# daniilidis-group/msckf_mono

Hardware: AMD Instinct MI355X
Metric: filter updates/sec (30-cam window, 200 feats) (higher is better)
Workload: dtype f32; 1 GPU; BASELINE.json configs[2]: synthetic 30-cam window / 200 feats, float, 64 batched trajectories per GPU; cam_window=30, tracks_per_update=200, trajectories_per_gpu=64, imu_per_update=10, parallelism=replicated trajectories, 64 per rank, noise=isotropic (f_u = f_v), sequences=1, gate_early_accept=False, streams=4

## Files before the change

include/msckf_hip.h:

```cpp
#ifndef MSCKF_HIP_H
#define MSCKF_HIP_H

#include <stdint.h>

#ifdef __cplusplus
extern "C" {
#endif

typedef struct msckf_hip_batch* msckf_hip_handle;

enum { MSCKF_HIP_F32 = 0, MSCKF_HIP_F64 = 1, MSCKF_HIP_F16H_F32P = 2 };

int msckf_hip_create(int B, int n_cap, int f_cap, int m_cap, int dtype, int device, msckf_hip_handle* out);
int msckf_hip_destroy(msckf_hip_handle h);
int msckf_hip_copy_state(msckf_hip_handle dst, msckf_hip_handle src);
const char* msckf_hip_last_error(void);

int msckf_hip_initialize(msckf_hip_handle h, int b, const double* cam12, const double* noise29,
                         const double* params8, const double* imu29);
int msckf_hip_initialize_full(msckf_hip_handle h, int b, const double* cam12, const double* uv2, const double* Q144,
                              const double* P0_225, const double* params8, const double* imu29);
int msckf_hip_propagate(msckf_hip_handle h, int b, const double* readings7, int K);
int msckf_hip_augment_state(msckf_hip_handle h, int b, int state_id, double time);
int msckf_hip_update(msckf_hip_handle h, int b, const double* meas2, const uint64_t* ids, int n);
// ... 10 lines not shown
int msckf_hip_get_pruned_states(msckf_hip_handle h, int b, double* cam7, double* time, int* state_ids,
                                int* last_correlated_ids, int cap);
int msckf_hip_get_cam_meta(msckf_hip_handle h, int b, double* time, int* n_tracked, int* last_correlated_ids, int cap);
int msckf_hip_get_tracked_feature_ids(msckf_hip_handle h, int b, int cam_index, uint64_t* ids, int cap);

int msckf_hip_get_covariance(msckf_hip_handle h, int b, double* P, int ld);
int msckf_hip_set_covariance(msckf_hip_handle h, int b, const double* P, int D);
int msckf_hip_set_imu_state(msckf_hip_handle h, int b, const double* imu29);
int msckf_hip_set_cam_pose(msckf_hip_handle h, int b, int slot, const double* cam7);
int msckf_hip_get_num_residualized(msckf_hip_handle h, int b, long long* n);
int msckf_hip_set_num_residualized(msckf_hip_handle h, int b, long long n);
int msckf_hip_last_stats(msckf_hip_handle h, int b, int* out7);
int msckf_hip_clear_error_flags(msckf_hip_handle h, int b);
int msckf_hip_get_error_flags(msckf_hip_handle h, int b, int* flags);
int msckf_hip_last_tracks(msckf_hip_handle h, int b, double* out8, int cap);
int msckf_hip_last_deltax(msckf_hip_handle h, int b, double* dx, int cap);
int msckf_hip_last_track_blocks(msckf_hip_handle h, int b, int* first, double* Hx, double* rw, double* Bh, int cap);

int msckf_hip_set_tracks(msckf_hip_handle h, int b, int F, const int* M, const int* slots, const double* obs2);
int msckf_hip_propagate_range(msckf_hip_handle h, int b0, int nb, const double* readings7, int K);
int msckf_hip_propagate_range_counts(msckf_hip_handle h, int b0, int nb, const double* readings7, const int* K);
int msckf_hip_augment_range(msckf_hip_handle h, int b0, int nb);
int msckf_hip_marginalize_range(msckf_hip_handle h, int b0, int nb);
int msckf_hip_drop_oldest_range(msckf_hip_handle h, int b0, int nb, int n_drop);
int msckf_hip_image_cycle_range(msckf_hip_handle h, int b0, int nb, const int* state_ids, const double* times,
                                const double* upd_meas2, const uint64_t* upd_ids, const int* upd_n,
                                const double* new_meas2, const uint64_t* new_ids, const int* new_n, int flags);

int msckf_hip_scenario_alloc(msckf_hip_handle h, int n_frames, int K);
int msckf_hip_scenario_set(msckf_hip_handle h, int frame, int b, const double* readings7 , int F,
                           const int* M, const int* slots, const double* obs2, int n_drop);
enum { MSCKF_HIP_CELL_SKIP = 1 };
int msckf_hip_scenario_set_cell(msckf_hip_handle h, int frame, int b, const double* readings7 , int k, int F,
                                const int* M, const int* slots, const double* obs2, int n_drop, int flags);
int msckf_hip_scenario_commit(msckf_hip_handle h);
int msckf_hip_run_frames(msckf_hip_handle h, int f0, int f1);
int msckf_hip_run_frames_streamed(msckf_hip_handle h, int f0, int f1);
int msckf_hip_scenario_pin(msckf_hip_handle h, int f0, int f1);
int msckf_hip_set_upload_ring(msckf_hip_handle h, int depth, int mode);
int msckf_hip_replay_alloc(msckf_hip_handle h, int n_seq, int n_frames, int K);
int msckf_hip_replay_set_cell(msckf_hip_handle h, int frame, int seq, const double* readings7 , int k, int F,
                              const int* M, const int* slots, const double* obs2, int n_drop, int flags);
int msckf_hip_replay_assign(msckf_hip_handle h, const int* seq_of, const uint64_t* seed, const double* sigma4);
int msckf_hip_replay_assign_q(msckf_hip_handle h, const int* seq_of, const uint64_t* seed, const double* Q144 ,
                              const double* scale , const double* sigma_uv );
int msckf_hip_replay_walk(msckf_hip_handle h, int f0, int f1, int b0, int nb, double* out);
int msckf_hip_replay_commit(msckf_hip_handle h);
int msckf_hip_run_frames_replay(msckf_hip_handle h, int f0, int f1);
int msckf_hip_replay_expand(msckf_hip_handle h, int frame, int b, double* rd , double* obs2, int cap_entries);
int msckf_hip_replay_expand_ints(msckf_hip_handle h, int frame, int b, int* ints, int* slots, int cap_entries);
int msckf_hip_sync(msckf_hip_handle h);
int msckf_hip_frame_log_enable(msckf_hip_handle h, int capacity_frames);
int msckf_hip_frame_log_reset(msckf_hip_handle h);
int msckf_hip_frame_log_count(msckf_hip_handle h);
int msckf_hip_frame_log_read(msckf_hip_handle h, int r0, int n, int b0, int nb, double* out);
int msckf_hip_frame_log_metrics(msckf_hip_handle h, int r0, int r1, const double* gt_p, double* out);
int msckf_hip_frame_log_metrics_ranges(msckf_hip_handle h, const int* r0, const int* r1, const double* gt_p, double* out);
int msckf_hip_map_log_enable(msckf_hip_handle h, int capacity_per_trajectory);
int msckf_hip_map_log_reset(msckf_hip_handle h);
int msckf_hip_map_log_frames(msckf_hip_handle h);
int msckf_hip_map_log_counts(msckf_hip_handle h, int b0, int nb, int* stored, int* found);
int msckf_hip_map_log_read(msckf_hip_handle h, int b, int r0, int n, double* out);
int msckf_hip_map_log_metrics(msckf_hip_handle h, int q0, int q1, const double* gt_xyz, const int* gt_off, double* out);
int msckf_hip_pruned_log_enable(msckf_hip_handle h, int capacity_per_trajectory);
int msckf_hip_pruned_log_reset(msckf_hip_handle h);
int msckf_hip_pruned_log_frames(msckf_hip_handle h);
int msckf_hip_pruned_log_counts(msckf_hip_handle h, int b0, int nb, int* stored, int* found);
int msckf_hip_pruned_log_read(msckf_hip_handle h, int b, int r0, int n, double* out, int* aug_ord);
int msckf_hip_pruned_log_metrics(msckf_hip_handle h, int q0, int q1, const double* gt_pose, int n_ord, double* out);
int msckf_hip_profile_enable(msckf_hip_handle h, int on);
int msckf_hip_profile_read(msckf_hip_handle h, double* ms8, int* count8);
int msckf_hip_profile_read_ex(msckf_hip_handle h, double* ms, int* count, int cap);
int msckf_hip_profile_event_overhead(msckf_hip_handle h, double* ms);
int msckf_hip_set_streams(msckf_hip_handle h, int n);
int msckf_hip_set_hw_queues(msckf_hip_handle h, int n);
int msckf_hip_parse_hw_queues(const char* text);
int msckf_hip_set_slices_exact(msckf_hip_handle h, int on);
int msckf_hip_get_effective_streams(msckf_hip_handle h, int streamed, int* out);
int msckf_hip_set_host_affinity(msckf_hip_handle h, const int* cpus, int n);
int msckf_hip_set_gate_early_accept(msckf_hip_handle h, int on);
int msckf_hip_set_compression(msckf_hip_handle h, int route);
int msckf_hip_set_covariance_update(msckf_hip_handle h, int form);
int msckf_hip_set_feature_overlap(msckf_hip_handle h, int on);
int msckf_hip_set_anisotropic_noise(msckf_hip_handle h, int mode, double tail_tol);
int msckf_hip_literal_info(msckf_hip_handle h, int b, int* out8);

#ifdef __cplusplus
}
#endif
#endif
```

msckf_mono_amd/capi.py:

```python
import ctypes as C
import os
import subprocess

import numpy as np

_HERE = os.path.dirname(os.path.abspath(__file__))
LIB_PATH = os.environ.get("MSCKF_HIP_LIB", os.path.join(_HERE, "libmsckf_hip.so"))
_LIB = None

F32, F64, F16H = 0, 1, 2
_dp = C.POINTER(C.c_double)
_ip = C.POINTER(C.c_int)
_up = C.POINTER(C.c_uint64)

SYMBOLS = [
    "msckf_hip_create", "msckf_hip_destroy", "msckf_hip_last_error", "msckf_hip_initialize", "msckf_hip_initialize_full", "msckf_hip_propagate",
    "msckf_hip_augment_state", "msckf_hip_update", "msckf_hip_add_features", "msckf_hip_marginalize",
    "msckf_hip_prune_empty_states", "msckf_hip_prune_redundant_states", "msckf_hip_finish",
    "msckf_hip_get_num_cam_states", "msckf_hip_get_imu_state", "msckf_hip_get_cam_states", "msckf_hip_get_map",
    "msckf_hip_get_pruned_state_ids", "msckf_hip_get_covariance", "msckf_hip_set_covariance", "msckf_hip_set_imu_state",
    "msckf_hip_set_cam_pose", "msckf_hip_get_num_residualized", "msckf_hip_set_num_residualized", "msckf_hip_last_stats",
    "msckf_hip_last_tracks", "msckf_hip_last_deltax", "msckf_hip_set_tracks", "msckf_hip_propagate_range",
    "msckf_hip_augment_range", "msckf_hip_marginalize_range", "msckf_hip_drop_oldest_range", "msckf_hip_scenario_alloc",
    "msckf_hip_scenario_set", "msckf_hip_scenario_commit", "msckf_hip_run_frames", "msckf_hip_run_frames_streamed", "msckf_hip_sync",
    "msckf_hip_profile_enable", "msckf_hip_profile_read", "msckf_hip_profile_read_ex", "msckf_hip_profile_event_overhead", "msckf_hip_set_streams", "msckf_hip_set_gate_early_accept",
    "msckf_hip_scenario_pin", "msckf_hip_set_upload_ring", "msckf_hip_clear_error_flags",
    "msckf_hip_set_compression", "msckf_hip_set_covariance_update", "msckf_hip_set_feature_overlap", "msckf_hip_get_pruned_states", "msckf_hip_get_cam_meta", "msckf_hip_get_tracked_feature_ids",
    "msckf_hip_set_anisotropic_noise", "msckf_hip_literal_info", "msckf_hip_get_error_flags", "msckf_hip_copy_state", "msckf_hip_set_host_affinity",
    "msckf_hip_image_cycle_range", "msckf_hip_get_effective_streams", "msckf_hip_set_hw_queues", "msckf_hip_parse_hw_queues", "msckf_hip_set_slices_exact",
    "msckf_hip_frame_log_enable", "msckf_hip_frame_log_reset", "msckf_hip_frame_log_count", "msckf_hip_frame_log_read", "msckf_hip_frame_log_metrics",
    "msckf_hip_scenario_set_cell", "msckf_hip_propagate_range_counts", "msckf_hip_frame_log_metrics_ranges",
    "msckf_hip_map_log_enable", "msckf_hip_map_log_reset", "msckf_hip_map_log_frames", "msckf_hip_map_log_counts", "msckf_hip_map_log_read", "msckf_hip_map_log_metrics",
    "msckf_hip_pruned_log_enable", "msckf_hip_pruned_log_reset", "msckf_hip_pruned_log_frames", "msckf_hip_pruned_log_counts", "msckf_hip_pruned_log_read", "msckf_hip_pruned_log_metrics",
    "msckf_hip_replay_alloc", "msckf_hip_replay_set_cell", "msckf_hip_replay_assign", "msckf_hip_replay_commit", "msckf_hip_run_frames_replay", "msckf_hip_replay_expand",
    "msckf_hip_replay_expand_ints", "msckf_hip_replay_assign_q", "msckf_hip_replay_walk", "msckf_hip_last_track_blocks",
]
CELL_SKIP = 1

FRAME_LOG_STRIDE = 48
FRAME_LOG_FIELDS = {
    "q": slice(0, 4), "b_g": slice(4, 7), "v": slice(7, 10), "b_a": slice(10, 13), "p": slice(13, 16),
    "P_II_diag": slice(16, 31), "P_pp": slice(31, 37),
    "n_cam": slice(37, 38), "n_tracks": slice(38, 39), "n_passed": slice(39, 40), "error_flags": slice(40, 41),
    "cam0": slice(41, 48),
}
FRAME_LOG_METRICS = ("n", "sum_sq_err", "max_err", "final_err", "sum_nees", "n_flagged")
MAP_LOG_STRIDE = 8
MAP_LOG_FIELDS = {"p": slice(0, 3), "gamma": slice(3, 4), "frame": slice(4, 5), "track": slice(5, 6), "flags": slice(6, 7), "M": slice(7, 8)}
MAP_FLAG_PASS, MAP_FLAG_INCLUDED, MAP_FLAG_BOUND = 1, 2, 4
MAP_LOG_METRICS = ("n", "n_matched", "sum_sq_err", "max_err", "n_gated", "sum_gamma", "sum_dof", "n_unmatched")
PRUNED_LOG_STRIDE = 32
PRUNED_LOG_FIELDS = {"q": slice(0, 4), "p": slice(4, 7), "frame": slice(7, 8), "cov": slice(8, 29),
                     "n_cam": slice(29, 30), "k": slice(30, 31), "pad": slice(31, 32)}
PRUNED_LOG_METRICS = ("n", "n_matched", "sum_sq_pos_err", "max_pos_err", "sum_sq_ang_err", "max_ang_err", "sum_nees", "n_nees", "n_bad_pivot", "n_unmatched")


def build():
    subprocess.check_call(["make", "-s", "-j8", "-C", os.path.join(_HERE, "csrc")])


def lib():
    global _LIB
    if _LIB is None:
        if not os.path.exists(LIB_PATH):
            raise RuntimeError("libmsckf_hip.so is not built (run __graft_entry__.build()); there is no CPU fallback")
        try:
            import torch
        except Exception:
            pass
        L = C.CDLL(LIB_PATH)
        L.msckf_hip_last_error.restype = C.c_char_p
        _LIB = L
    return _LIB


class HipError(RuntimeError):
    pass


def _chk(rc):
    if rc < 0:
        raise HipError("msckf_hip call failed (%d): %s" % (rc, lib().msckf_hip_last_error().decode()))
    return rc


def _d(a):
    a = np.ascontiguousarray(a, dtype=np.float64)
    return a, a.ctypes.data_as(_dp)


def _i(a):
    a = np.ascontiguousarray(a, dtype=np.int32)
    return a, a.ctypes.data_as(_ip)


def pack_config(cfg):
    cam = np.array([cfg["c_u"], cfg["c_v"], cfg["f_u"], cfg["f_v"], cfg.get("b", 0.0)] + list(cfg["q_CI"]) + list(cfg["p_C_I"]), dtype=np.float64)
    noise = np.array([cfg["u_var_prime"], cfg["v_var_prime"]] + list(cfg["Q_imu_diag"]) + list(cfg["P0_diag"]), dtype=np.float64)
    params = np.array([cfg["max_gn_cost_norm"], cfg.get("min_rcond", 3e-12), cfg["translation_threshold"],
                       cfg.get("redundancy_angle_thresh", 0.005), cfg.get("redundancy_distance_thresh", 0.05),
                       cfg["min_track_length"], cfg["max_track_length"], cfg["max_cam_states"]], dtype=np.float64)
    return cam, noise, params


def full_noise(cfg):
    if "Q_imu" not in cfg and "P0" not in cfg:
        return None
    Q = np.asarray(cfg["Q_imu"], dtype=np.float64) if "Q_imu" in cfg else np.diag(np.asarray(cfg["Q_imu_diag"], dtype=np.float64))
    P0 = np.asarray(cfg["P0"], dtype=np.float64) if "P0" in cfg else np.diag(np.asarray(cfg["P0_diag"], dtype=np.float64))
    if Q.shape != (12, 12) or P0.shape != (15, 15):
        raise ValueError("Q_imu must be 12 x 12 and P0 15 x 15")
    return Q, P0


class Batch:
    _replay_K = 0
    _replay_frames = 0

# ... 211 lines not shown
    def replay_set_cell(self, frame, seq, readings, M, slots, obs, n_drop, skip=False):
        r, pr = _d(np.asarray(readings, dtype=np.float64).reshape(-1, 7)); Ma, pM = _i(M); s, ps = _i(slots); o, po = _d(obs)
        _chk(self.L.msckf_hip_replay_set_cell(self.h, int(frame), int(seq), pr, r.shape[0], len(Ma), pM, ps, po, int(n_drop), CELL_SKIP if skip else 0))

    def replay_assign(self, seq_of, seeds, sigma4):
        q, pq = _i(seq_of)
        sd = np.ascontiguousarray([int(x) & 0xFFFFFFFFFFFFFFFF for x in seeds], dtype=np.uint64)
        sg = np.ascontiguousarray(np.broadcast_to(np.asarray(sigma4, dtype=np.float64), (self.B, 4)))
        if q.shape != (self.B,) or sd.shape != (self.B,):
            raise ValueError("seq_of and seeds must hold one value per trajectory")
        _chk(self.L.msckf_hip_replay_assign(self.h, pq, sd.ctypes.data_as(_up), sg.ctypes.data_as(_dp)))

    def replay_assign_q(self, seq_of, seeds, Q, scale, sigma_uv):
        q, pq = _i(seq_of)
        sd = np.ascontiguousarray([int(x) & 0xFFFFFFFFFFFFFFFF for x in seeds], dtype=np.uint64)
        if q.shape != (self.B,) or sd.shape != (self.B,):
            raise ValueError("seq_of and seeds must hold one value per trajectory")
        Qa = np.broadcast_to(np.asarray(Q, dtype=np.float64), (self.B, 12, 12))
        Qc = np.ascontiguousarray(np.swapaxes(Qa, 1, 2))
        sc_ = np.ascontiguousarray(np.broadcast_to(np.asarray(scale, dtype=np.float64), (self.B,)))
        uv = np.ascontiguousarray(np.broadcast_to(np.asarray(sigma_uv, dtype=np.float64), (self.B, 2)))
        _chk(self.L.msckf_hip_replay_assign_q(self.h, pq, sd.ctypes.data_as(_up), Qc.ctypes.data_as(_dp), sc_.ctypes.data_as(_dp), uv.ctypes.data_as(_dp)))

    def replay_walk(self, f0=0, f1=None, b0=0, nb=None):
        f1 = self._replay_frames + 1 if f1 is None else int(f1)
        nb = self.B - int(b0) if nb is None else int(nb)
        out = np.zeros((max(f1 - int(f0), 0), max(nb, 0), 6))
        _chk(self.L.msckf_hip_replay_walk(self.h, int(f0), f1, int(b0), nb, out.ctypes.data_as(_dp)))
        return out

    def replay_commit(self):
        _chk(self.L.msckf_hip_replay_commit(self.h))

    def run_frames_replay(self, f0, f1):
        _chk(self.L.msckf_hip_run_frames_replay(self.h, int(f0), int(f1)))

    def replay_expand(self, frame, b):
        cap = self.f_cap * self.m_cap
        rd = np.zeros((self._replay_K, 7)); obs = np.zeros((cap, 2)); ints = np.zeros(3 + 2 * self.f_cap, dtype=np.int32); slots = np.zeros(cap, dtype=np.int32)
        n = _chk(self.L.msckf_hip_replay_expand(self.h, int(frame), int(b), rd.ctypes.data_as(_dp), obs.ctypes.data_as(_dp), cap))
        _chk(self.L.msckf_hip_replay_expand_ints(self.h, int(frame), int(b), ints.ctypes.data_as(_ip), slots.ctypes.data_as(_ip), cap))
        return dict(rd=rd, obs=obs[:n], n=int(ints[0]), drop=int(ints[1]), k=int(ints[2]), M=ints[3:3 + self.f_cap].copy(),
                    off=ints[3 + self.f_cap:].copy(), slots=slots[:n])

    def scenario_pin(self, f0, f1):
        _chk(self.L.msckf_hip_scenario_pin(self.h, int(f0), int(f1)))

    def set_upload_ring(self, depth=6, mode=0):
        _chk(self.L.msckf_hip_set_upload_ring(self.h, int(depth), int(mode)))

    def clear_error_flags(self, b):
        _chk(self.L.msckf_hip_clear_error_flags(self.h, int(b)))

    def sync(self):
        _chk(self.L.msckf_hip_sync(self.h))

    def set_host_affinity(self, cpus):
        a = np.ascontiguousarray(list(cpus), dtype=np.int32)
        _chk(self.L.msckf_hip_set_host_affinity(self.h, a.ctypes.data_as(_ip), int(a.size)))

    def set_streams(self, n):
        _chk(self.L.msckf_hip_set_streams(self.h, int(n)))

    def set_hw_queues(self, n):
        _chk(self.L.msckf_hip_set_hw_queues(self.h, int(n)))

    def set_slices_exact(self, on):
        _chk(self.L.msckf_hip_set_slices_exact(self.h, 1 if on else 0))

    def effective_streams(self, streamed=False):
        n = C.c_int(0)
        _chk(self.L.msckf_hip_get_effective_streams(self.h, 1 if streamed else 0, C.byref(n)))
        return int(n.value)

    def set_compression(self, route):
        _chk(self.L.msckf_hip_set_compression(self.h, int(route)))

    def set_covariance_update(self, form):
        _chk(self.L.msckf_hip_set_covariance_update(self.h, int(form)))

    def set_feature_overlap(self, on):
        _chk(self.L.msckf_hip_set_feature_overlap(self.h, 1 if on else 0))

    def set_gate_early_accept(self, on):
        _chk(self.L.msckf_hip_set_gate_early_accept(self.h, 1 if on else 0))

    def set_anisotropic_noise(self, mode, tail_tol=-1.0):
        _chk(self.L.msckf_hip_set_anisotropic_noise(self.h, int(mode), C.c_double(float(tail_tol))))

    def literal_info(self, b):
        o = np.zeros(8, dtype=np.int32)
        _chk(self.L.msckf_hip_literal_info(self.h, int(b), o.ctypes.data_as(_ip)))
        return dict(zip(["m_rows", "kept_rows", "reflected", "skipped_by_tolerance", "route", "leading_rows_handed_through", "kept_handed_through_rows", "spare"], o.tolist()))

    def frame_log_enable(self, capacity_frames):
        _chk(self.L.msckf_hip_frame_log_enable(self.h, int(capacity_frames)))

    def frame_log_reset(self):
        _chk(self.L.msckf_hip_frame_log_reset(self.h))

    def frame_log_count(self):
        return _chk(self.L.msckf_hip_frame_log_count(self.h))

    def frame_log_read(self, r0=0, n=None, b0=0, nb=None):
        n = self.frame_log_count() - r0 if n is None else int(n)
        nb = self.B - b0 if nb is None else int(nb)
        o = np.zeros((max(n, 0), max(nb, 0), FRAME_LOG_STRIDE))
        _chk(self.L.msckf_hip_frame_log_read(self.h, int(r0), n, int(b0), nb, o.ctypes.data_as(_dp)))
        return o, {k: o[:, :, s] for k, s in FRAME_LOG_FIELDS.items()}

    def frame_log_metrics(self, r0, r1, gt_p):
        g = np.ascontiguousarray(gt_p, dtype=np.float64)
        if g.shape != (int(r1) - int(r0), self.B, 3):
            raise ValueError("gt_p must be [r1 - r0][B][3]")
        o = np.zeros((self.B, 6))
        _chk(self.L.msckf_hip_frame_log_metrics(self.h, int(r0), int(r1), g.ctypes.data_as(_dp), o.ctypes.data_as(_dp)))
        return o

    def frame_log_metrics_ranges(self, r0, r1, gt_p):
        a0, p0 = _i(r0); a1, p1 = _i(r1)
        if a0.shape != (self.B,) or a1.shape != (self.B,):
            raise ValueError("r0 and r1 must hold one record index per trajectory")
        g = np.ascontiguousarray(gt_p, dtype=np.float64)
        if g.shape != (int(a1.max()) - int(a0.min()), self.B, 3):
            raise ValueError("gt_p must be [max(r1) - min(r0)][B][3]")
        o = np.zeros((self.B, 6))
        _chk(self.L.msckf_hip_frame_log_metrics_ranges(self.h, p0, p1, g.ctypes.data_as(_dp), o.ctypes.data_as(_dp)))
        return o

    def _cursor_log_counts(self, prefix, b0, nb):
        nb = self.B - b0 if nb is None else int(nb)
        s = np.zeros(max(nb, 0), dtype=np.int32); f = np.zeros(max(nb, 0), dtype=np.int32)
        _chk(getattr(self.L, "msckf_hip_%s_log_counts" % prefix)(self.h, int(b0), nb, s.ctypes.data_as(_ip), f.ctypes.data_as(_ip)))
        return s, f

    def _cursor_log_read(self, prefix, stride, b, r0, n, aug=False):
        n = int(self._cursor_log_counts(prefix, b, 1)[0][0]) - r0 if n is None else int(n)
        o = np.zeros((max(n, 0), stride)); a = np.full(max(n, 1), -1, dtype=np.int32) if aug else None
        _chk(getattr(self.L, "msckf_hip_%s_log_read" % prefix)(self.h, int(b), int(r0), n, o.ctypes.data_as(_dp), *([a.ctypes.data_as(_ip)] if aug else [])))
        return o, a

    def map_log_enable(self, capacity_per_trajectory):
        _chk(self.L.msckf_hip_map_log_enable(self.h, int(capacity_per_trajectory)))

    def map_log_reset(self):
        _chk(self.L.msckf_hip_map_log_reset(self.h))

    def map_log_frames(self):
        return _chk(self.L.msckf_hip_map_log_frames(self.h))

    def map_log_counts(self, b0=0, nb=None):
        return self._cursor_log_counts("map", b0, nb)

    def map_log_read(self, b, r0=0, n=None):
        o = self._cursor_log_read("map", MAP_LOG_STRIDE, b, r0, n)[0]
        return o, {k: o[:, s] for k, s in MAP_LOG_FIELDS.items()}

    def map_log_metrics(self, q0, q1, gt=None):
        o = np.zeros((self.B, 8))
        if gt is None:
            _chk(self.L.msckf_hip_map_log_metrics(self.h, int(q0), int(q1), None, None, o.ctypes.data_as(_dp)))
            return o
        g = np.ascontiguousarray(gt[0], dtype=np.float64).reshape(-1, 3)
        off, po = _i(gt[1])
        if off.shape != ((int(q1) - int(q0)) * self.B + 1,) or (off.size and int(off[-1]) > len(g)):
            raise ValueError("gt_off must hold (q1 - q0) * B + 1 offsets into gt_xyz")
# ... 110 lines not shown
```

msckf_mono_amd/csrc/dev_common.h:

```cpp
#ifndef MSCKF_DEV_COMMON_H
#define MSCKF_DEV_COMMON_H

#include <hip/hip_runtime.h>
#include <hip/hip_fp16.h>

#include <cstdint>
#include <type_traits>

#include "update_routes.h"

namespace msckf {

constexpr int IMU_STRIDE = 32;
constexpr int CAM_STRIDE = 8;
constexpr int PRM_STRIDE = 48;
constexpr int DG_STRIDE = 28;
constexpr int RD_STRIDE = 7;
constexpr int QF_STRIDE = 80;
constexpr int QF_FLAG = 78;
__host__ __device__ constexpr int qf_index(int i, int j) { return i * (23 - i) / 2 + j; }

enum {
  IQ = 0, IBG = 4, IV = 7, IBA = 10, IP = 13, IG = 16, IQN = 19, IVN = 23, IPN = 26
};
// ... 292 lines not shown
template <class T> __device__ __forceinline__ T half_sum(T v) { return x16_sum(row16_sum(v)); }
__device__ __forceinline__ float half_max(float v) {
  v = row16_max(v);
  const auto r = __builtin_amdgcn_permlane16_swap(__float_as_uint(v), __float_as_uint(v), false, false);
  const float a = __uint_as_float(r[0]), c = __uint_as_float(r[1]);
  return a > c ? a : c;
}
__device__ __forceinline__ int half_min_i(int v) {
  v = row16_min(v);
  const auto r = __builtin_amdgcn_permlane16_swap((unsigned)v, (unsigned)v, false, false);
  return min((int)r[0], (int)r[1]);
}

__device__ __forceinline__ void wave_lds_sync() {
  __builtin_amdgcn_fence(__ATOMIC_RELEASE, "workgroup"); __builtin_amdgcn_wave_barrier(); __builtin_amdgcn_fence(__ATOMIC_ACQUIRE, "workgroup");
}

typedef float f32x4 __attribute__((ext_vector_type(4)));
typedef double f64x4 __attribute__((ext_vector_type(4)));
template <class T> struct Mfma16;
template <> struct Mfma16<double> {
  typedef f64x4 V;
  static __device__ __forceinline__ V mma(double a, double b, V c) { return __builtin_amdgcn_mfma_f64_16x16x4f64(a, b, c, 0, 0, 0); }
  static __device__ __forceinline__ int row(int lane, int r) { return (lane >> 4) + 4 * r; }
  static __device__ __forceinline__ int row_of_group(int g, int r) { return g + 4 * r; }
};
template <> struct Mfma16<float> {
  typedef f32x4 V;
  static __device__ __forceinline__ V mma(float a, float b, V c) { return __builtin_amdgcn_mfma_f32_16x16x4f32(a, b, c, 0, 0, 0); }
  static __device__ __forceinline__ int row(int lane, int r) { return 4 * (lane >> 4) + r; }
  static __device__ __forceinline__ int row_of_group(int g, int r) { return 4 * g + r; }
};

template <class S> __device__ __forceinline__ S fast_rsqrt(S x);
template <> __device__ __forceinline__ float fast_rsqrt<float>(float x) {
  const float r = __builtin_amdgcn_rsqf(x);
  return r * (1.5f - 0.5f * x * r * r);
}
template <> __device__ __forceinline__ double fast_rsqrt<double>(double x) {
  double r = __builtin_amdgcn_rsq(x);
  r = r + 0.5 * r * (1.0 - x * r * r);
  r = r + 0.5 * r * (1.0 - x * r * r);
  return r;
}

template <class S> __device__ __forceinline__ S fast_rcp(S x);
template <> __device__ __forceinline__ float fast_rcp<float>(float x) {
  const float r = __builtin_amdgcn_rcpf(x);
  return __builtin_fmaf(__builtin_fmaf(-x, r, 1.0f), r, r);
}
template <> __device__ __forceinline__ double fast_rcp<double>(double x) {
  double r = __builtin_amdgcn_rcp(x);
  r = __builtin_fma(__builtin_fma(-x, r, 1.0), r, r);
  r = __builtin_fma(__builtin_fma(-x, r, 1.0), r, r);
  return r;
}

template <class S> struct Lim;
template <> struct Lim<float> { static __device__ __forceinline__ float tiny() { return 1.17549435e-38f; } };
template <> struct Lim<double> { static __device__ __forceinline__ double tiny() { return 2.2250738585072014e-308; } };

__device__ __forceinline__ double lam_diag_term(const double* Dg, int n, int n_cap, int I, int J) {
  const int hi = I >= J ? I : J, lo = I >= J ? J : I;
  const bool isy = hi == n && lo < n, isd = hi < n && (hi / 6 == lo / 6);
  const int a6 = lo % 6, c6 = hi % 6;
  const int idx = isy ? 21 + a6 : (isd ? a6 * 6 - a6 * (a6 - 1) / 2 + (c6 - a6) : 0);
  const double dg = Dg[min(lo / 6, n_cap - 1) * DG_STRIDE + idx];
  return (isy || isd) ? dg : 0.0;
}
__device__ __forceinline__ double lam_hat(const double* Lam, const double* , int ldL, int n, int , int I, int J) {
  const int hi = I >= J ? I : J, lo = I >= J ? J : I;
  const bool ok = hi <= n && lo < n;
  const double lv = Lam[(long)min(hi, ldL - 1) * ldL + min(lo, ldL - 1)];
  return ok ? lv : 0.0;
}

constexpr int IMU_SKIP = -1;
template <class S> void launch_propagate(const Dev<S>& d, int b0, int nb, const S* readings, long rd_stride, int K, hipStream_t st, bool then_augment, int qroute, const int* cnt = nullptr);
template <class S> void launch_augment(const Dev<S>& d, int b0, int nb, hipStream_t st, const int* cnt = nullptr);
template <class S> void launch_prune(const Dev<S>& d, int b0, int nb, hipStream_t st, const int* drop = nullptr, int drop_const = -1);
template <class S> void launch_feature(const Dev<S>& d, int b0, int nb, hipStream_t st);
template <class S> void launch_select(const Dev<S>& d, int b0, int nb, hipStream_t st);
template <class S> void launch_select_diag(const Dev<S>& d, int b0, int nb, hipStream_t st);
template <class S> void launch_compress(const Dev<S>& d, int b0, int nb, hipStream_t st, int phase);
template <class S> void launch_gram(const Dev<S>& d, int b0, int nb, hipStream_t st, int phase);
template <class S> void launch_kalman(const Dev<S>& d, int b0, int nb, hipStream_t st);
template <class S> void launch_update_small(const Dev<S>& d, int b0, int nb, hipStream_t st, const routes::SmallRoute& r);
bool update_small_granted();
template <class S> void launch_literal(const Dev<S>& d, int b0, int nb, hipStream_t st, int part = 0);
template <class S> void launch_chol_gram(const Dev<S>& d, int b0, int nb, hipStream_t st, const routes::CompressRoute& r);
void launch_chol_gain(const Dev<float>& d, int b0, int nb, hipStream_t st, const routes::KalmanRoute& r);
template <class S> void launch_chol_gain_large(const Dev<S>& d, int b0, int nb, hipStream_t st, const routes::KalmanRoute& r);
template <class S> void launch_frame_log(const Dev<S>& d, int b0, int nb, hipStream_t st, const S* P, bool pending, S* rec);
template <class S> void launch_log_metrics(const S* log, int B, int r0, int r1, const int* r0b, const int* r1b, const double* gt, double* out, hipStream_t st);
template <class S> void launch_map_log(const Dev<S>& d, int b0, int nb, hipStream_t st, const int* n, const int* M, int ordinal, int cap, S* rec, int* found);
template <class S> void launch_map_metrics(const S* rec, const int* found, int cap, int B, int q0, int q1, const double* gt, const int* off, double* out, hipStream_t st);
template <class S> void launch_pruned_log(const Dev<S>& d, int b0, int nb, hipStream_t st, const int* drop, int ordinal, int cap, S* rec, int* found);
template <class S> void launch_pruned_metrics(const S* rec, const int* found, int cap, int B, int q0, int q1, const int* aug, const double* gt, int n_ord, double* out, hipStream_t st);
struct ReplaySeqIn { const double* rd; const int* n; const int* drop; const int* k; const int* M; const int* off; const int* slots; const double* obs; };
struct ReplayTrajIn { const int* seq_of; const uint64_t* seed; const double* sigma; const int* base; };
template <class S> struct ReplayOut { S* rd; int* n; int* drop; int* k; int* M; int* off; int* slots; S* obs; };
constexpr int REPLAY_CHUNK = 256;
constexpr int REPLAY_SCAN_CHUNK = 64;
struct ReplayModelIn { const double* L; const double* scale; const double* wstart; };
template <class S> void launch_replay_expand(const ReplaySeqIn& q, const ReplayTrajIn& t, const ReplayModelIn& m, const ReplayOut<S>& o, int f, int b0, int nb, int K, int f_cap, int max_entries, hipStream_t st);
void launch_replay_walk_scan(const double* rd, const int* k, const ReplayTrajIn& t, const ReplayModelIn& m, double* wstart, int frames, int S, int K, int B, hipStream_t st);
void feature_device_setup();
void qr_device_setup();
void kalman_device_setup();
void gram_device_setup();
void literal_device_setup();
bool literal_lds_available();
long lit_ws_doubles(int n6, int m_cap, int r_cap);

}
#endif
```

msckf_mono_amd/csrc/kernels_feature.hip:

```cpp
#include "chi2_table.h"
#include "dev_common.h"

namespace msckf {

__constant__ double c_chi2[99];
#ifdef MSCKF_ABLATE
__device__ int g_feat_dbg = 0;
#endif

template <class S> struct Pose { M3<S> R; V3<S> t; };

template <class S> __device__ __forceinline__ S lm_rcp(S x);
template <> __device__ __forceinline__ double lm_rcp<double>(double x) { return 1.0 / x; }
template <> __device__ __forceinline__ float lm_rcp<float>(float x) { const float r = __builtin_amdgcn_rcpf(x); return r * __builtin_fmaf(-x, r, 2.0f); }
template <class S> __device__ __forceinline__ S lm_sqrt(S x);
template <> __device__ __forceinline__ double lm_sqrt<double>(double x) { return sqrt(x); }
template <> __device__ __forceinline__ float lm_sqrt<float>(float x) { return __builtin_amdgcn_sqrtf(x); }

template <class S>
__device__ __forceinline__ S tri_cost(const Pose<S>& T, S a, S b, S rho, S zx, S zy) {
  const V3<S> h = mulv(T.R, mk3(a, b, S(1))) + (rho * T.t);
  if (sizeof(S) == 4) { const S iz = lm_rcp(h.z); const S dx = h.x * iz - zx, dy = h.y * iz - zy; return dx * dx + dy * dy; }
  const S dx = h.x / h.z - zx, dy = h.y / h.z - zy;
  return dx * dx + dy * dy;
}

template <class S>
__device__ __forceinline__ void ldlt3(const S A[6], S lam, const S b[3], S x[3]) {
  const S a00 = A[0] + lam, a01 = A[1], a02 = A[2], a11 = A[3] + lam, a12 = A[4], a22 = A[5] + lam;
  const S d0 = a00;
  S y0, y1, y2, l10, l20, l21;
  if (sizeof(S) == 4) {
    const S i0 = lm_rcp(d0);
    l10 = a01 * i0; l20 = a02 * i0;
    const S d1 = a11 - l10 * l10 * d0, i1 = lm_rcp(d1);
    l21 = (a12 - l20 * l10 * d0) * i1;
    const S d2 = a22 - l20 * l20 * d0 - l21 * l21 * d1;
    y0 = b[0]; y1 = b[1] - l10 * y0; y2 = b[2] - l20 * y0 - l21 * y1;
    y0 *= i0; y1 *= i1; y2 *= lm_rcp(d2);
  } else {
    l10 = a01 / d0; l20 = a02 / d0;
    const S d1 = a11 - l10 * l10 * d0;
    l21 = (a12 - l20 * l10 * d0) / d1;
    const S d2 = a22 - l20 * l20 * d0 - l21 * l21 * d1;
    y0 = b[0]; y1 = b[1] - l10 * y0; y2 = b[2] - l20 * y0 - l21 * y1;
    y0 /= d0; y1 /= d1; y2 /= d2;
  }
  x[2] = y2; x[1] = y1 - l21 * x[2]; x[0] = y0 - l10 * x[1] - l20 * x[2];
}

template <class T>
__device__ __forceinline__ void house3(T hf[2][3], int lane, T v[2][3], T Tm[3][3]) {
  T tau[3];
  const int row0 = 2 * lane;
#pragma unroll
  for (int k = 0; k < 3; ++k) {
    T t2 = 0;
#pragma unroll
    for (int s2 = 0; s2 < 2; ++s2) if (row0 + s2 > k) t2 += hf[s2][k] * hf[s2][k];
    t2 = wave_sum(t2);
    const T c0 = wave_bcast(hf[k & 1][k], k >> 1);
    T inv = 0;
    if (t2 <= Lim<T>::tiny()) { tau[k] = 0; }
    else {
      const T nn = c0 * c0 + t2, rs = fast_rsqrt(nn);
      T beta = nn * rs, ibeta = rs;
      if (c0 >= T(0)) { beta = -beta; ibeta = -ibeta; }
      inv = fast_rcp(c0 - beta);
      tau[k] = (beta - c0) * ibeta;
    }
#pragma unroll
    for (int s2 = 0; s2 < 2; ++s2) {
      const int row = row0 + s2;
      v[s2][k] = row > k ? hf[s2][k] * inv : (row == k ? T(1) : T(0));
    }
#pragma unroll
    for (int j = k + 1; j < 3; ++j) {
      T s = v[0][k] * hf[0][j] + v[1][k] * hf[1][j];
      s = wave_sum(s) * tau[k];
      hf[0][j] -= s * v[0][k];
      hf[1][j] -= s * v[1][k];
    }
  }
  const T d01 = wave_sum(v[0][0] * v[0][1] + v[1][0] * v[1][1]);
// ... 1175 lines not shown
      asm volatile("" : "+v"(lane_f));
      switch (nbr) {
        case 1: ok = gate_chol_dpp<1>(G, sC, lane_f, R2, sig2); break;
        case 2: ok = gate_chol_dpp<2>(G, sC, lane_f, R2, sig2); break;
        case 3: ok = gate_chol_dpp<3>(G, sC, lane_f, R2, sig2); break;
        case 4: ok = gate_chol_dpp<4>(G, sC, lane_f, R2, sig2); break;
        case 5: ok = gate_chol_dpp<5>(G, sC, lane_f, R2, sig2); break;
        case 6: ok = gate_chol_dpp<6>(G, sC, lane_f, R2, sig2); break;
        case 7: ok = gate_chol_dpp<7>(G, sC, lane_f, R2, sig2); break;
        default: ok = gate_chol_dpp<8>(G, sC, lane_f, R2, sig2); break;
      }
      const S gm = ok ? gate_gamma_from_corner<S>(sC) : S(0);
      if (g == s) { spd = ok; gamma = gm; }
      __syncthreads();
    }
  }
  FP_TICK(5);
  if (spd && gamma < thresh) status |= ST_GATE_PASS;

  if (has && gl == 0) {
    d.trk_status[tb] = status;
    d.trk_gamma[tb] = gamma;
    d.trk_first[tb] = slot_lo | (slot_hi << 8);
    S* opf = d.trk_pf + tb * 4;
    opf[0] = pf.x; opf[1] = pf.y; opf[2] = pf.z; opf[3] = 0;
  }

  {
#pragma unroll
    for (int i = 0; i < 2; ++i) {
      asm volatile("" : "+v"(r[i]));
#pragma unroll
      for (int k = 3; k < 6; ++k) asm volatile("" : "+v"(hx[i][k]));
    }
    const Lq q = normal_eq();
    double Bq[3][6];
    const double f0[3] = {-(double)hx[0][3], -(double)hx[0][4], -(double)hx[0][5]}, f1[3] = {-(double)hx[1][3], -(double)hx[1][4], -(double)hx[1][5]};
#pragma unroll
    for (int k = 0; k < 6; ++k) {
      const double h0 = (double)hx[0][k], h1 = (double)hx[1][k];
      const double g0 = f0[0] * h0 + f1[0] * h1, g1 = f0[1] * h0 + f1[1] * h1, g2 = f0[2] * h0 + f1[2] * h1;
      const double b0v = g0 * q.i00, b1v = (g1 - q.l10 * b0v) * q.i11;
      Bq[0][k] = b0v; Bq[1][k] = b1v; Bq[2][k] = (g2 - q.l20 * b0v - q.l21 * b1v) * q.i22;
    }
    int* sInv = reinterpret_cast<int*>(sG) + g * 64;
    sInv[gl] = -1; sInv[gl + GS] = -1;
    wave_lds_sync();
    if (act) sInv[slot] = gl;
    wave_lds_sync();
    double* oB = d.trk_B + tb * 3 * (long)d.ldR;
    signed char* oI = d.trk_inv + tb * d.n_cap;
    if (has) {
      for (int e = gl; e < d.n_cap; e += GS) oI[e] = (signed char)sInv[e];
      if (slot_hi - slot_lo + 1 != M) {
        const int c_n = 6 * (slot_hi - slot_lo + 1);
        for (int e = gl; e < 3 * c_n; e += GS) { const int qr = e / c_n, cc = e - qr * c_n; if (sInv[slot_lo + cc / 6] < 0) oB[(long)qr * d.ldR + 6 * slot_lo + cc] = 0.0; }
      }
    }
    if (act) {
      typedef float f4v __attribute__((ext_vector_type(4)));
      typedef double d2v __attribute__((ext_vector_type(2)));
      typedef float f2v __attribute__((ext_vector_type(2)));
      if (d.h16) { __half* oH = d.trk_Hx16 + (tb * m_cap) * 12; for (int i = 0; i < 2; ++i) for (int k = 0; k < 6; ++k) oH[gl * 12 + i * 6 + k] = __float2half_rn((float)hx[i][k]); }
      else {
        f4v* oHx = reinterpret_cast<f4v*>(d.trk_Hx + (tb * m_cap) * 12 + gl * 12);
        oHx[0] = f4v{hx[0][0], hx[0][1], hx[0][2], hx[0][3]}; oHx[1] = f4v{hx[0][4], hx[0][5], hx[1][0], hx[1][1]}; oHx[2] = f4v{hx[1][2], hx[1][3], hx[1][4], hx[1][5]};
      }
#pragma unroll
      for (int qr = 0; qr < 3; ++qr) {
        d2v* ob = reinterpret_cast<d2v*>(oB + (long)qr * d.ldR + 6 * slot);
        ob[0] = d2v{Bq[qr][0], Bq[qr][1]}; ob[1] = d2v{Bq[qr][2], Bq[qr][3]}; ob[2] = d2v{Bq[qr][4], Bq[qr][5]};
      }
      *reinterpret_cast<f2v*>(d.trk_rw + tb * 2 * m_cap + 2 * gl) = f2v{r[0], r[1]};
    }
    if (has && gl < 3) oB[(long)gl * d.ldR + 6 * ncam_now] = gl == 0 ? q.cq[0] : (gl == 1 ? q.cq[1] : q.cq[2]);
  }
  FP_TICK(6);
#ifdef MSCKF_ABLATE
  if ((fdbg & 0x100000) && lane == 0) atomicAdd(&g_featp_cycles[7], 1ull);
#endif
}

template <class S>
__device__ __forceinline__ void select_body(const Dev<S>& d, const int b0, const int nb, const int i, const int lane) {
  if (i >= nb) return;
  const int b = b0 + i;
  const int F = d.trk_n[(long)i * d.wl_stride_n];
  long long nres = d.n_resid[b];
  int* st = d.stats + (long)b * STAT_STRIDE;
  int mrej = 0, trej = 0, grej = 0, pass = 0;
  int* rs = d.row_start + (long)b * (d.f_cap + 1);
  int* order = d.trk_order + (long)b * d.f_cap;
  __shared__ int sCnt[64], sBase[64], sRows[64];
  sCnt[lane] = 0; sRows[lane] = 0;
  __syncthreads();
  if (!(nres <= 3 && d.mode == 0) && F <= 256) {
    __shared__ short sMrow[256];
    __shared__ short sOrd[256];
    int sv[4], Mv[4], fv[4];
    bool inc[4];
#pragma unroll
    for (int c = 0; c < 4; ++c) {
      const int t = 64 * c + lane, tc = min(t, max(F - 1, 0));
      const long tb = (long)b * d.f_cap + tc;
      sv[c] = d.trk_status[tb]; Mv[c] = d.trk_M[(long)i * d.wl_stride_f + tc]; fv[c] = d.trk_first[tb] & 63;
    }
#pragma unroll
    for (int c = 0; c < 4; ++c) {
      const int t = 64 * c + lane;
      const bool in = t < F;
      int sx = in ? sv[c] : 0;
      const int M = in ? Mv[c] : 0;
      bool m_rej = false, t_rej = false, g_rej = false, valid = false, incl = false;
      if (in) {
        if (M < 2 || !(sx & ST_MOTION_OK)) { m_rej = true; sx = (M < 2) ? 0 : (sx & ~(ST_TRI_VALID | ST_GATE_PASS)); }
        else if (sx & ST_TRI_VALID) valid = true;
        else { t_rej = true; sx &= ~ST_GATE_PASS; }
        if (valid) { if (sx & ST_GATE_PASS) { incl = true; sx |= ST_INCLUDED; } else g_rej = true; }
        d.trk_status[(long)b * d.f_cap + t] = sx;
        sMrow[t] = (short)(2 * M - 3);
      }
      inc[c] = incl;
      if (incl) { atomicAdd(&sCnt[fv[c]], 1); atomicAdd(&sRows[fv[c]], 2 * M - 3); }
      mrej += __popcll(__ballot(m_rej)); trej += __popcll(__ballot(t_rej)); grej += __popcll(__ballot(g_rej));
      pass += __popcll(__ballot(incl)); if (d.mode == 0) nres += __popcll(__ballot(valid));
    }
    __syncthreads();
    {
      const int c0 = sCnt[lane];
      int scan = c0;
#pragma unroll
      for (int o = 1; o < 64; o <<= 1) { const int up = __shfl_up(scan, o, 64); if (lane >= o) scan += up; }
      sBase[lane] = scan - c0;
    }
    __syncthreads();
    const int nbin = min(d.n_cap, 64);
#pragma unroll
    for (int c = 0; c < 4; ++c) {
      const int bin = inc[c] ? fv[c] : -1;
      int rank = 0, cnt = 0;
      for (int sbin = 0; sbin < nbin; ++sbin) {
        const unsigned long long m = __ballot(bin == sbin);
        if (bin == sbin) { rank = __popcll(m & ((1ull << lane) - 1ull)); cnt = __popcll(m); }
      }
      int pos = 0;
      if (inc[c]) { pos = sBase[bin] + rank; sOrd[pos] = (short)(64 * c + lane); order[pos] = 64 * c + lane; }
      __syncthreads();
      if (inc[c] && rank == 0) sBase[bin] += cnt;
      __syncthreads();
    }
    int rows = 0;
    for (int p0 = 0; p0 < pass; p0 += 64) {
      const int p = p0 + lane;
      const int r = p < pass ? (int)sMrow[sOrd[p]] : 0;
      int scan = r;
#pragma unroll
      for (int o = 1; o < 64; o <<= 1) { const int up = __shfl_up(scan, o, 64); if (lane >= o) scan += up; }
      if (p < pass) rs[p] = rows + scan - r;
      rows += __shfl(scan, 63, 64);
    }
    if (lane == 0) {
      rs[pass] = rows;
      d.n_resid[b] = nres;
      st[STAT_NTRACKS] = F; st[STAT_MOTION_REJ] = mrej; st[STAT_TRI_REJ] = trej; st[STAT_GATE_REJ] = grej;
      st[STAT_PASSED] = pass; st[STAT_MROWS] = rows; st[STAT_RROWS] = rows > 0 ? 6 * d.ncam[b] : 0;
    }
    return;
  }
  if (nres <= 3 && d.mode == 0) {
    if (lane == 0) {
      for (int t = 0; t < F; ++t) {
        const long tb = (long)b * d.f_cap + t;
        int s = d.trk_status[tb];
        const int M = d.trk_M[(long)i * d.wl_stride_f + t];
        bool valid = false;
        if (M < 2) { if (nres > 3) mrej++; else trej++; s = 0; }
        else if (nres > 3 && !(s & ST_MOTION_OK)) { mrej++; s &= ~(ST_TRI_VALID | ST_GATE_PASS); }
        else {
          if (nres <= 3) s |= ST_MOTION_SKIPPED;
          if (s & ST_TRI_VALID) { valid = true; nres++; } else { trej++; s &= ~ST_GATE_PASS; }
        }
        if (valid) {
          if (s & ST_GATE_PASS) { s |= ST_INCLUDED; pass++; const int f0 = d.trk_first[tb] & 63; sCnt[f0]++; sRows[f0] += 2 * M - 3; }
          else grej++;
        }
        d.trk_status[tb] = s;
      }
    }
    mrej = __shfl(mrej, 0, 64); trej = __shfl(trej, 0, 64); grej = __shfl(grej, 0, 64); pass = __shfl(pass, 0, 64);
    nres = __shfl((int)nres, 0, 64);
  } else {
    for (int t0 = 0; t0 < F; t0 += 64) {
      const int t = t0 + lane;
      const bool in = t < F;
      const long tb = (long)b * d.f_cap + t;
      int s = in ? d.trk_status[tb] : 0;
      const int M = in ? d.trk_M[(long)i * d.wl_stride_f + t] : 0;
      bool m_rej = false, t_rej = false, g_rej = false, valid = false, incl = false;
      if (in) {
        if (M < 2 || !(s & ST_MOTION_OK)) { m_rej = true; s = (M < 2) ? 0 : (s & ~(ST_TRI_VALID | ST_GATE_PASS)); }
        else if (s & ST_TRI_VALID) valid = true;
        else { t_rej = true; s &= ~ST_GATE_PASS; }
        if (valid) { if (s & ST_GATE_PASS) { incl = true; s |= ST_INCLUDED; } else g_rej = true; }
        d.trk_status[tb] = s;
      }
      if (incl) { const int f0 = d.trk_first[tb] & 63; atomicAdd(&sCnt[f0], 1); atomicAdd(&sRows[f0], 2 * M - 3); }
      mrej += __popcll(__ballot(m_rej)); trej += __popcll(__ballot(t_rej)); grej += __popcll(__ballot(g_rej));
      pass += __popcll(__ballot(incl)); if (d.mode == 0) nres += __popcll(__ballot(valid));
    }
  }
  __syncthreads();
  {
    const int c = sCnt[lane];
    int scan = c;
#pragma unroll
    for (int o = 1; o < 64; o <<= 1) { const int up = __shfl_up(scan, o, 64); if (lane >= o) scan += up; }
    sBase[lane] = scan - c;
  }
  __syncthreads();
  for (int t0 = 0; t0 < F; t0 += 64) {
    const int t = t0 + lane;
    const long tb = (long)b * d.f_cap + t;
    const bool incl = (t < F) && (d.trk_status[tb] & ST_INCLUDED);
    const int bin = incl ? (d.trk_first[tb] & 63) : -1;
    int pos = -1;
    for (int sbin = 0; sbin < d.n_cap && sbin < 64; ++sbin) {
      const unsigned long long m = __ballot(bin == sbin);
      if (bin == sbin) pos = sBase[sbin] + __popcll(m & ((1ull << lane) - 1ull));
      __syncthreads();
      if (lane == 0) sBase[sbin] += __popcll(m);
      __syncthreads();
    }
    if (incl) order[pos] = t;
  }
  __syncthreads();
  int rows = 0;
  for (int p0 = 0; p0 < pass; p0 += 64) {
    const int p = p0 + lane;
    int r = 0;
    if (p < pass) { const int t = order[p]; r = 2 * d.trk_M[(long)i * d.wl_stride_f + t] - 3; }
    int scan = r;
#pragma unroll
    for (int o = 1; o < 64; o <<= 1) { const int up = __shfl_up(scan, o, 64); if (lane >= o) scan += up; }
    if (p < pass) rs[p] = rows + scan - r;
    rows += __shfl(scan, 63, 64);
  }
  if (lane == 0) {
    rs[pass] = rows;
    d.n_resid[b] = nres;
    st[STAT_NTRACKS] = F; st[STAT_MOTION_REJ] = mrej; st[STAT_TRI_REJ] = trej; st[STAT_GATE_REJ] = grej;
    st[STAT_PASSED] = pass; st[STAT_MROWS] = rows; st[STAT_RROWS] = rows > 0 ? 6 * d.ncam[b] : 0;
  }
}

template <class S>
__global__ __launch_bounds__(64) void k_select(Dev<S> d, int b0, int nb) { select_body<S>(d, b0, nb, (int)blockIdx.x, (int)threadIdx.x); }

template <class S>
__global__ __launch_bounds__(256) void k_select_diag(Dev<S> d, int b0, int nb, int ndiag) {
  const int tid = threadIdx.x, lane = tid & 63, w = tid >> 6, i = blockIdx.y;
  if ((int)blockIdx.x == ndiag) { if (tid < 64) select_body<S>(d, b0, nb, i, tid); return; }
  const int b = b0 + i;
  const int N = d.ncam[b], F = d.trk_n[(long)i * d.wl_stride_n];
  const int s = 4 * (int)blockIdx.x + w;
  if (s >= N) return;
  const int f_cap = d.f_cap, m_cap = d.m_cap;
  const int* stt = d.trk_status + (long)b * f_cap;
  const int* Mv = d.trk_M + (long)i * d.wl_stride_f;
  constexpr int ALL = ST_MOTION_OK | ST_TRI_VALID | ST_GATE_PASS;
  int tcut = 0;
  if (d.mode == 0 && F > 0) {
    int need = 4 - d.nres_upd[b];
    if (need > 0) {
      tcut = F;
      for (int t0 = 0; t0 < F && need > 0; t0 += 64) {
        const int t = t0 + lane;
        const bool v = t < F && Mv[t] >= 2 && (stt[t] & ST_TRI_VALID);
        unsigned long long m = __ballot(v);
        const int c = __popcll(m);
        if (c < need) { need -= c; continue; }
        int pos = 0;
        for (int k = 0; k < need; ++k) { pos = __builtin_ctzll(m); m &= m - 1; }
        tcut = t0 + pos + 1; need = 0;
      }
    }
  }
  double acc[27];
#pragma unroll
  for (int e = 0; e < 27; ++e) acc[e] = 0.0;
  for (int t = lane; t < F; t += 64) {
    const long tb = (long)b * f_cap + t;
    const int sx = stt[t], M = Mv[t];
    const int oi = d.trk_inv[tb * d.n_cap + s];
    const int need_bits = t < tcut ? (ST_TRI_VALID | ST_GATE_PASS) : ALL;
    if (M < 2 || (sx & need_bits) != need_bits || oi < 0) continue;
    const long h0i = (tb * m_cap + oi) * 12;
    const S* rw = d.trk_rw + tb * 2 * m_cap + 2 * oi;
    double h0[6], h1[6];
#pragma unroll
    for (int k = 0; k < 6; ++k) { h0[k] = (double)ld_hx(d, h0i + k); h1[k] = (double)ld_hx(d, h0i + 6 + k); }
    const double r0 = (double)rw[0], r1 = (double)rw[1];
    int e = 0;
#pragma unroll
    for (int a = 0; a < 6; ++a)
#pragma unroll
      for (int c = a; c < 6; ++c) acc[e++] += h0[a] * h0[c] + h1[a] * h1[c];
#pragma unroll
    for (int a = 0; a < 6; ++a) acc[21 + a] += h0[a] * r0 + h1[a] * r1;
  }
  double* out = d.Dg + ((long)b * d.n_cap + s) * DG_STRIDE;
#pragma unroll
  for (int e = 0; e < 27; ++e) {
    const double v = wave_sum(acc[e]);
    if (lane == 0) out[e] = v;
  }
}

void feature_device_setup() {
  (void)hipMemcpyToSymbol(HIP_SYMBOL(c_chi2), kChi2Q05, sizeof(double) * 99);
  (void)hipFuncSetAttribute(reinterpret_cast<const void*>(k_feature<float, false>), hipFuncAttributeMaxDynamicSharedMemorySize, 160 * 1024);
  (void)hipFuncSetAttribute(reinterpret_cast<const void*>(k_feature<double, false>), hipFuncAttributeMaxDynamicSharedMemorySize, 160 * 1024);
  (void)hipFuncSetAttribute(reinterpret_cast<const void*>(k_feature<float, true>), hipFuncAttributeMaxDynamicSharedMemorySize, 160 * 1024);
  (void)hipFuncSetAttribute(reinterpret_cast<const void*>(k_feature<double, true>), hipFuncAttributeMaxDynamicSharedMemorySize, 160 * 1024);
  (void)hipFuncSetAttribute(reinterpret_cast<const void*>(k_feature_pair), hipFuncAttributeMaxDynamicSharedMemorySize, 160 * 1024);
}

template <class S>
void launch_feature(const Dev<S>& d, int b0, int nb, hipStream_t st) {
  if (nb <= 0) return;
  const dim3 grid(xcd_grid(nb, d.f_cap));
  const routes::FeatureRoute r = routes::feature_route(sizeof(S), d.f_cap, d.m_cap, nb, d.feat_pair, d.compress);
  for (int i = 0; i < r.n; ++i) {
    const routes::FeatureLaunch& l = r.l[i];
    if (l.pair) {
      if constexpr (sizeof(S) == 4) {
        const routes::PairResidency res = routes::feature_pair_residency(l.lm);
        hipLaunchKernelGGL(k_feature_pair, dim3(xcd_grid(nb, l.items)), dim3(64), res.lds_bytes, st, d, b0, nb, l.lm, l.m_lo, l.m_hi, res.s_cap, l.items, l.single);
      }
      continue;
    }
    const size_t lds = routes::feature_lds_bytes(l.lm, sizeof(S), l.staged != 0);
    if (l.long_form) hipLaunchKernelGGL((k_feature<S, true>), grid, dim3(64), lds, st, d, b0, nb, l.lm, l.m_lo, l.m_hi, l.staged);
    else hipLaunchKernelGGL((k_feature<S, false>), grid, dim3(64), lds, st, d, b0, nb, l.lm, l.m_lo, l.m_hi, l.staged);
  }
}
#ifdef MSCKF_ABLATE
void feat_debug_set(int val) { (void)hipMemcpyToSymbol(HIP_SYMBOL(g_feat_dbg), &val, sizeof(int)); }
void featp_cycles_read(unsigned long long* out8, int reset) {
  (void)hipMemcpyFromSymbol(out8, HIP_SYMBOL(g_featp_cycles), sizeof(unsigned long long) * 8);
  if (reset) { unsigned long long z[8] = {0}; (void)hipMemcpyToSymbol(HIP_SYMBOL(g_featp_cycles), z, sizeof(z)); }
}
#endif

template <class S>
void launch_select(const Dev<S>& d, int b0, int nb, hipStream_t st) {
  if (nb <= 0) return;
  hipLaunchKernelGGL(k_select<S>, dim3(nb), dim3(64), 0, st, d, b0, nb);
}
template <class S>
void launch_select_diag(const Dev<S>& d, int b0, int nb, hipStream_t st) {
  if (nb <= 0) return;
  const int ndiag = (d.n_cap + 3) / 4;
  hipLaunchKernelGGL(k_select_diag<S>, dim3(ndiag + 1, nb), dim3(256), 0, st, d, b0, nb, ndiag);
}

template void launch_feature<float>(const Dev<float>&, int, int, hipStream_t);
template void launch_feature<double>(const Dev<double>&, int, int, hipStream_t);
template void launch_select<float>(const Dev<float>&, int, int, hipStream_t);
template void launch_select<double>(const Dev<double>&, int, int, hipStream_t);
template void launch_select_diag<float>(const Dev<float>&, int, int, hipStream_t);
template void launch_select_diag<double>(const Dev<double>&, int, int, hipStream_t);

}
```

msckf_mono_amd/csrc/kernels_state.hip:

```cpp
#include "dev_common.h"

namespace msckf {

template <class S>
__device__ __forceinline__ void mm15(S* C, const S* A, const S* B, int lane) {
  for (int e = lane; e < 225; e += 64) {
    const int i = e / 15, j = e % 15;
    S s = 0;
#pragma unroll
    for (int k = 0; k < 15; ++k) s += A[i * 15 + k] * B[k * 15 + j];
    C[e] = s;
  }
}
template <class S>
__device__ __forceinline__ void mm15_abt(S* C, const S* A, const S* B, int lane) {
  for (int e = lane; e < 225; e += 64) {
    const int i = e / 15, j = e % 15;
    S s = 0;
#pragma unroll
    for (int k = 0; k < 15; ++k) s += A[i * 15 + k] * B[j * 15 + k];
    C[e] = s;
  }
}

constexpr int PG = 16;
constexpr int SST = 20;

template <class S>
__device__ __forceinline__ void imu_rk(const S* st, V3<S> g, V3<S> om, V3<S> ac, S dT, S* out) {
  const Q4<S> q = ldq(st);
  const V3<S> bg = ld3(st + 4), v = ld3(st + 7), ba = ld3(st + 10), p = ld3(st + 13);
  const V3<S> wh = om - bg, ah = ac - ba;
  const M3<S> C = q2rot(q);
  S y0[4] = {-q.x, -q.y, -q.z, q.w};
  auto omul = [&](const S* y, S* o) {
    o[0] = S(0.5) * (wh.z * y[1] - wh.y * y[2] + wh.x * y[3]);
    o[1] = S(0.5) * (-wh.z * y[0] + wh.x * y[2] + wh.y * y[3]);
    o[2] = S(0.5) * (wh.y * y[0] - wh.x * y[1] + wh.z * y[3]);
    o[3] = S(0.5) * (-wh.x * y[0] - wh.y * y[1] - wh.z * y[2]);
  };
  S k0[4], k1[4], k2[4], k3[4], k4[4], k5[4], t[4];
  omul(y0, k0);
  for (int i = 0; i < 4; ++i) t[i] = y0[i] + (k0[i] / S(4)) * dT;
  omul(t, k1);
  for (int i = 0; i < 4; ++i) t[i] = y0[i] + (k0[i] / S(8) + k1[i] / S(8)) * dT;
  omul(t, k2);
  for (int i = 0; i < 4; ++i) t[i] = y0[i] + (-k1[i] / S(2) + k2[i]) * dT;
  omul(t, k3);
  for (int i = 0; i < 4; ++i) t[i] = y0[i] + (k0[i] * S(3) / S(16) + k3[i] * S(9) / S(16)) * dT;
  omul(t, k4);
  for (int i = 0; i < 4; ++i)
    t[i] = y0[i] + (-k0[i] * S(3) / S(7) + k1[i] * S(2) / S(7) + k2[i] * S(12) / S(7) - k3[i] * S(12) / S(7) + k4[i] * S(8) / S(7)) * dT;
  omul(t, k5);
  S yt[4];
  for (int i = 0; i < 4; ++i) yt[i] = y0[i] + (S(7) * k0[i] + S(32) * k2[i] + S(12) * k3[i] + S(32) * k4[i] + S(7) * k5[i]) * dT / S(90);
  Q4<S> qn; qn.w = yt[3]; qn.x = -yt[0]; qn.y = -yt[1]; qn.z = -yt[2];
  qn = qnormalized(qn);
  stq(out, qn);
  st3(out + 4, bg);
  st3(out + 7, v + (dT * (multv(C, ah) + g)));
  st3(out + 10, ba);
  st3(out + 13, p + (dT * v));
}

#ifdef MSCKF_ABLATE
__device__ unsigned long long g_prop_cycles[8];
#define PR_TICK(slot) do { if (tid == 0) { const long long t_ = clock64(); pcyc[slot] += t_ - ptl; ptl = t_; } } while (0)
void prop_cycles_read(unsigned long long* out8, int reset) {
  (void)hipMemcpyFromSymbol(out8, HIP_SYMBOL(g_prop_cycles), sizeof(unsigned long long) * 8);
  if (reset) { unsigned long long z[8] = {0}; (void)hipMemcpyToSymbol(HIP_SYMBOL(g_prop_cycles), z, sizeof(z)); }
}
#else
#define PR_TICK(slot) do {} while (0)
#endif

template <class S>
__device__ __forceinline__ void augment_body(const Dev<S>& d, int b, int tid, S* sJP) {
  const int n = d.ncam[b];
  if (n >= d.n_cap) { if (tid == 0) atomicOr(&d.stats[(long)b * STAT_STRIDE + STAT_ERR], STAT_ERR_NCAP); return; }
  const int D = 15 + 6 * n, ld = d.ld;
  const S* imu = d.imu + (long)b * IMU_STRIDE;
  const S* prm = d.prm + (long)b * PRM_STRIDE;
  S* P = d.P + (long)b * ld * ld;
  const Q4<S> q = ldq(imu + IQ), qci = ldq(prm + PRM_QCI);
  const V3<S> pci = ld3(prm + PRM_PCI);
  const V3<S> lever = qrotate(qinverse(q), pci);
  const M3<S> Jtt = q2rot(qci), Jpt = skew3(lever);
  if (tid == 0) {
    S* cs = d.cam + ((long)b * d.n_cap + n) * CAM_STRIDE;
    stq(cs, qnormalized(qmul(qci, q)));
    st3(cs + 4, ld3(imu + IP) + lever);
  }
  for (int c = tid; c < D; c += 256) {
    const S* pc = P + (long)c * ld;
    const V3<S> th = mk3(pc[0], pc[1], pc[2]);
    const V3<S> a = mulv(Jtt, th), bb = mulv(Jpt, th);
    const S jp[6] = {a.x, a.y, a.z, bb.x + pc[12], bb.y + pc[13], bb.z + pc[14]};
#pragma unroll
    for (int i = 0; i < 6; ++i) { sJP[i * ld + c] = jp[i]; P[(long)c * ld + D + i] = jp[i]; P[(long)(D + i) * ld + c] = jp[i]; }
  }
  __syncthreads();
  if (tid < 36) {
    const int i = tid / 6, j = tid % 6;
    auto corner = [&](int r, int cc) {
      const S* jp = sJP + r * ld;
      if (cc < 3) return jp[0] * Jtt.m[cc][0] + jp[1] * Jtt.m[cc][1] + jp[2] * Jtt.m[cc][2];
      const int c3 = cc - 3;
      return jp[0] * Jpt.m[c3][0] + jp[1] * Jpt.m[c3][1] + jp[2] * Jpt.m[c3][2] + jp[12 + c3];
    };
    P[(long)(D + j) * ld + D + i] = (corner(i, j) + corner(j, i)) / S(2);
  }
  if (tid == 0) d.ncam[b] = n + 1;
}

template <class S>
__global__ __launch_bounds__(256) void k_augment(Dev<S> d, int b0, const int* cnt) {
  const int b = b0 + blockIdx.x, tid = threadIdx.x;
  if (cnt && cnt[blockIdx.x] < 0) return;
  __builtin_amdgcn_s_setprio(3);
  extern __shared__ __attribute__((aligned(16))) unsigned char smem_raw[];
  augment_body<S>(d, b, tid, reinterpret_cast<S*>(smem_raw));
}

template <class S, bool AUGMENT, int QM>
__global__ __launch_bounds__(256) void k_propagate(Dev<S> d, int b0, const S* readings, long rd_stride, int K, const int* cnt) {
  const int b = b0 + blockIdx.x, tid = threadIdx.x, lane = tid & 63, w = tid >> 6;
  if (cnt) K = cnt[blockIdx.x];
  constexpr bool FULLQ = QM == 2;
  if (QM != 0 && (d.qf[(long)b * QF_STRIDE + QF_FLAG] != S(0)) != FULLQ) return;
  __builtin_amdgcn_s_setprio(3);
#ifdef MSCKF_ABLATE
  long long pcyc[8] = {0, 0, 0, 0, 0, 0, 0, 0}, ptl = clock64();
#endif
  __shared__ S sState[(PG + 1) * SST];
  __shared__ S sPhi[PG * 225];
  constexpr int QT = FULLQ ? 145 : 32;
  __shared__ S sQt[PG * QT];
  __shared__ S sTot[225];
  __shared__ S sPii[225];
  __shared__ S sNull[12];
  __shared__ S sG[4];
  __shared__ S sRd[PG * RD_STRIDE];
  __shared__ S sQ[FULLQ ? 144 : 12];
  __shared__ S sRk[PG * 16];
  __shared__ S sDv[PG * 3];
  S* imu = d.imu + (long)b * IMU_STRIDE;
  const S* prm = d.prm + (long)b * PRM_STRIDE;
  S* P = d.P + (long)b * d.ld * d.ld;
  const int ld = d.ld;
  const int ncams = d.ncam_defer ? d.ncam_upd[b] - 1 : d.ncam[b];
  if (d.ncam_defer && tid == 0) d.ncam[b] = ncams;
  const int n = 6 * ncams;
  const S* rd = readings + (long)(b - b0) * rd_stride;
  constexpr int PIC_T = 6;
  S pic[PIC_T][4];
  {
    const int g = lane >> 4, c = lane & 15;
#pragma unroll
    for (int t = 0; t < PIC_T; ++t) {
      const int col = (w + 4 * t) * 16 + c;
#pragma unroll
      for (int kk = 0; kk < 4; ++kk) { const int k = Mfma16<S>::row_of_group(g, kk); pic[t][kk] = P[(long)(15 + min(col, d.n6cap - 1)) * ld + min(k, 14)]; }
    }
  }
  if (K <= 0) {
    if (AUGMENT && K == 0) {
      __syncthreads();
      extern __shared__ __attribute__((aligned(16))) unsigned char smem_aug0[];
      augment_body<S>(d, b, tid, reinterpret_cast<S*>(smem_aug0));
    }
    return;
  }
  if (tid < 16) sState[tid] = imu[tid];
  if (tid < 3) sG[tid] = imu[IG + tid];
  if (!FULLQ) { if (tid >= 64 && tid < 64 + 12) sQ[tid - 64] = prm[PRM_Q + tid - 64]; }
  else if (tid >= 64 && tid < 64 + 144) {
    const int i = (tid - 64) / 12, j = (tid - 64) % 12;
    sQ[tid - 64] = d.qf[(long)b * QF_STRIDE + (i <= j ? qf_index(i, j) : qf_index(j, i))];
  }
  if (tid >= 32 && tid < 32 + 10) sNull[tid - 32] = imu[IQN + (tid - 32)];
  for (int e = tid; e < 225; e += 256) {
    const int i = e / 15, j = e % 15;
    sPii[e] = P[(long)j * ld + i];
  }
  for (int e = tid; e < min(PG, K) * RD_STRIDE; e += 256) sRd[e] = rd[e];
  __syncthreads();
  typename Mfma16<S>::V Mreg = {0, 0, 0, 0};
  {
    const int g = lane >> 4, c = lane & 15;
#pragma unroll
    for (int r = 0; r < 4; ++r) {
      const int i = Mfma16<S>::row_of_group(g, r);
      if (i < 15 && c < 15) Mreg[r] = w == 0 ? sPii[i * 15 + c] : (i == c ? S(1) : S(0));
    }
  }
  for (int k0 = 0; k0 < K; k0 += PG) {
    const int G = min(PG, K - k0);
    if (k0 > 0) { for (int e = tid; e < G * RD_STRIDE; e += 256) sRd[e] = rd[(long)k0 * RD_STRIDE + e]; __syncthreads(); }
    PR_TICK(0);
    const V3<S> g = mk3(sG[0], sG[1], sG[2]);
    if (tid < 4 * G) {
      const int s = tid >> 2, c = tid & 3;
      const S* r = sRd + s * RD_STRIDE;
      const S dT = r[6];
      const V3<S> wh = ld3(r) - mk3(sState[4], sState[5], sState[6]);
      auto omul = [&](const S* y, S* o) {
        o[0] = S(0.5) * (wh.z * y[1] - wh.y * y[2] + wh.x * y[3]);
        o[1] = S(0.5) * (-wh.z * y[0] + wh.x * y[2] + wh.y * y[3]);
        o[2] = S(0.5) * (wh.y * y[0] - wh.x * y[1] + wh.z * y[3]);
        o[3] = S(0.5) * (-wh.x * y[0] - wh.y * y[1] - wh.z * y[2]);
// ... 164 lines not shown
    __syncthreads();
    PR_TICK(2);
    {
      typedef Mfma16<S> MF;
      const int g = lane >> 4, c = lane & 15;
      if (w < 2) {
        const S* qt = sQt;
        int qidx[4];
#pragma unroll
        for (int r = 0; r < 4; ++r) {
          const int i = MF::row_of_group(g, r), bi = i / 3;
          if (FULLQ) qidx[r] = (i < 12 && c < 12) ? i * 12 + c : 144;
          else qidx[r] = (bi != c / 3 || bi >= 4) ? 31 : (bi == 2 ? 15 + (i - 6) * 3 + (c - 6) : (i == c ? i : 31));
        }
        if (w == 0) {
#pragma unroll
          for (int r = 0; r < 4; ++r) Mreg[r] += qt[qidx[r]];
        }
        for (int s = 0; s < G; ++s) {
          const S* Ph = sPhi + s * 225;
          S aPhi[4];
#pragma unroll
          for (int kk = 0; kk < 4; ++kk) { const int k = MF::row_of_group(g, kk); aPhi[kk] = (k < 15 && c < 15) ? Ph[c * 15 + k] : S(0); }
          typename MF::V zero = {0, 0, 0, 0};
          if (w == 0) {
            typename MF::V Y = zero, Pn = zero, Pt = zero;
#pragma unroll
            for (int kk = 0; kk < 4; ++kk) Y = MF::mma(Mreg[kk], aPhi[kk], Y);
#pragma unroll
            for (int kk = 0; kk < 4; ++kk) { Pn = MF::mma(aPhi[kk], Y[kk], Pn); Pt = MF::mma(Y[kk], aPhi[kk], Pt); }
            qt += QT;
#pragma unroll
            for (int r = 0; r < 4; ++r) Mreg[r] = (Pn[r] + Pt[r]) / S(2) + (s + 1 < G ? qt[qidx[r]] : S(0));
          } else {
            typename MF::V Tn = zero;
#pragma unroll
            for (int kk = 0; kk < 4; ++kk) Tn = MF::mma(aPhi[kk], Mreg[kk], Tn);
            Mreg = Tn;
          }
        }
      }
    }
    __syncthreads();
    if (tid < 16) sState[tid] = sState[G * SST + tid];
    __syncthreads();
    PR_TICK(3);
  }
  if (w < 2) {
    const int g = lane >> 4, c = lane & 15;
    S* dst = w == 0 ? sPii : sTot;
#pragma unroll
    for (int r = 0; r < 4; ++r) { const int i = Mfma16<S>::row_of_group(g, r); if (i < 15 && c < 15) dst[i * 15 + c] = Mreg[r]; }
  }
  __syncthreads();
  if (tid < 16) imu[tid] = sState[tid];
  if (tid < 4) imu[IQN + tid] = sState[tid];
  if (tid >= 4 && tid < 7) imu[IVN + tid - 4] = sState[7 + tid - 4];
  if (tid >= 8 && tid < 11) imu[IPN + tid - 8] = sState[13 + tid - 8];
  for (int e = tid; e < 225; e += 256) { const int i = e / 15, j = e % 15; P[(long)j * ld + i] = sPii[e]; }
  {
    const int g = lane >> 4, c = lane & 15;
    S aT[4];
#pragma unroll
    for (int kk = 0; kk < 4; ++kk) { const int k = Mfma16<S>::row_of_group(g, kk); aT[kk] = (k < 15 && c < 15) ? sTot[c * 15 + k] : S(0); }
#pragma unroll
    for (int t = 0; t < PIC_T; ++t) {
      const int col = (w + 4 * t) * 16 + c;
      if ((w + 4 * t) * 16 >= n) break;
      typename Mfma16<S>::V o = {0, 0, 0, 0};
#pragma unroll
      for (int kk = 0; kk < 4; ++kk) o = Mfma16<S>::mma(aT[kk], (col < n && Mfma16<S>::row_of_group(g, kk) < 15) ? pic[t][kk] : S(0), o);
      if (col < n) {
#pragma unroll
        for (int r = 0; r < 4; ++r) {
          const int i = Mfma16<S>::row_of_group(g, r);
          if (i < 15) { P[(long)(15 + col) * ld + i] = o[r]; P[(long)i * ld + 15 + col] = o[r]; }
        }
      }
    }
  }
#ifdef MSCKF_ABLATE
  __syncthreads();
  PR_TICK(4);
  if (tid == 0 && blockIdx.x == 0) { for (int q = 0; q < 5; ++q) atomicAdd(&g_prop_cycles[q], (unsigned long long)pcyc[q]); atomicAdd(&g_prop_cycles[5], 1ull); }
#endif
  if (AUGMENT) {
    __syncthreads();
    extern __shared__ __attribute__((aligned(16))) unsigned char smem_aug[];
    augment_body<S>(d, b, tid, reinterpret_cast<S*>(smem_aug));
  }
}

template <class S, int RMAX, int CMAX>
__global__ __launch_bounds__(1024) void k_prune_inplace(Dev<S> d, int b0, const int* drop, int drop_const, int use_keep) {
  const int b = b0 + blockIdx.y, tid = threadIdx.x;
  const int n = d.ncam[b];
  int nk, nd = 0;
  if (use_keep) nk = d.nkeep[b];
  else { nd = drop ? drop[blockIdx.y] : drop_const; nd = nd < 0 ? 0 : (nd > n ? n : nd); nk = n - nd; }
  const int* keep = d.keep + (long)b * d.n_cap;
  prune_bookkeeping<S>(d, b, tid, n, nk, nd, use_keep);
  if (nk >= n) return;
  const int Dn = 15 + 6 * nk, ld = d.ld;
  S* P = d.P + (long)b * ld * ld;
  __shared__ int sSrc[256 * RMAX];
  for (int i = tid; i < Dn; i += 1024) sSrc[i] = i < 15 ? i : 15 + 6 * (use_keep ? keep[(i - 15) / 6] : nd + (i - 15) / 6) + (i - 15) % 6;
  __syncthreads();
  const int ri = tid & 255, cg = tid >> 8;
  for (int j0 = 0; j0 < Dn; j0 += 4 * CMAX) {
    S v[CMAX][RMAX];
#pragma unroll
    for (int c = 0; c < CMAX; ++c) {
      const int j = j0 + cg + 4 * c;
      if (j < Dn) {
        const S* src = P + (long)sSrc[j] * ld;
#pragma unroll
        for (int r = 0; r < RMAX; ++r) { const int i = ri + r * 256; v[c][r] = i < Dn ? src[sSrc[i]] : S(0); }
      }
    }
    asm volatile("s_waitcnt vmcnt(0)" ::: "memory");
    __syncthreads();
#pragma unroll
    for (int c = 0; c < CMAX; ++c) {
      const int j = j0 + cg + 4 * c;
      if (j < Dn) {
        S* dst = P + (long)j * ld;
#pragma unroll
        for (int r = 0; r < RMAX; ++r) { const int i = ri + r * 256; if (i < Dn) dst[i] = v[c][r]; }
      }
    }
  }
  if (tid == 0) d.ncam[b] = nk;
}

template <class S, int QM>
static void launch_propagate_q(const Dev<S>& d, int b0, int nb, const S* readings, long rd_stride, int K, hipStream_t st, bool then_augment, const int* cnt) {
  if (then_augment) hipLaunchKernelGGL((k_propagate<S, true, QM>), dim3(nb), dim3(256), (size_t)6 * d.ld * sizeof(S), st, d, b0, readings, rd_stride, K, cnt);
  else hipLaunchKernelGGL((k_propagate<S, false, QM>), dim3(nb), dim3(256), 0, st, d, b0, readings, rd_stride, K, cnt);
}
template <class S>
void launch_propagate(const Dev<S>& d, int b0, int nb, const S* readings, long rd_stride, int K, hipStream_t st, bool then_augment, int qroute, const int* cnt) {
  if (nb <= 0) return;
  if (K <= 0 && !cnt) { if (then_augment) launch_augment<S>(d, b0, nb, st); return; }
  if (qroute == 0) { launch_propagate_q<S, 0>(d, b0, nb, readings, rd_stride, K, st, then_augment, cnt); return; }
  if (qroute == 1) launch_propagate_q<S, 1>(d, b0, nb, readings, rd_stride, K, st, then_augment, cnt);
  launch_propagate_q<S, 2>(d, b0, nb, readings, rd_stride, K, st, then_augment, cnt);
}
template <class S>
void launch_augment(const Dev<S>& d, int b0, int nb, hipStream_t st, const int* cnt) {
  if (nb <= 0) return;
  hipLaunchKernelGGL(k_augment<S>, dim3(nb), dim3(256), (size_t)6 * d.ld * sizeof(S), st, d, b0, cnt);
}
template <class S>
void launch_prune(const Dev<S>& d, int b0, int nb, hipStream_t st, const int* drop, int drop_const) {
  if (nb <= 0) return;
  const int use_keep = (!drop && drop_const < 0) ? 1 : 0;
  const dim3 grid(1, nb);
  if (d.ld <= 256) hipLaunchKernelGGL((k_prune_inplace<S, 1, 16>), grid, dim3(1024), 0, st, d, b0, drop, drop_const, use_keep);
  else hipLaunchKernelGGL((k_prune_inplace<S, 2, 12>), grid, dim3(1024), 0, st, d, b0, drop, drop_const, use_keep);
}

template void launch_propagate<float>(const Dev<float>&, int, int, const float*, long, int, hipStream_t, bool, int, const int*);
template void launch_propagate<double>(const Dev<double>&, int, int, const double*, long, int, hipStream_t, bool, int, const int*);
template void launch_augment<float>(const Dev<float>&, int, int, hipStream_t, const int*);
template void launch_augment<double>(const Dev<double>&, int, int, hipStream_t, const int*);
template void launch_prune<float>(const Dev<float>&, int, int, hipStream_t, const int*, int);
template void launch_prune<double>(const Dev<double>&, int, int, hipStream_t, const int*, int);

}
```

msckf_mono_amd/csrc/msckf_hip.hip:

```cpp
#include <hip/hip_runtime.h>

#include <algorithm>
#include <atomic>
#include <cerrno>
#include <chrono>
#include <cmath>
#include <condition_variable>
#include <cstdint>
#include <cstdio>
#include <cstdlib>
#include <cstring>
#include <dlfcn.h>
#include <functional>
#include <mutex>
#include <string>
#include <thread>
#include <utility>
#include <vector>
#include <pthread.h>
#include <sched.h>

#include "../../include/msckf_hip.h"
#include "dev_common.h"
#include "host_lists.h"
#include "input_layouts.h"
#include "replay_plan.h"
#include "settings.h"
#include "slice_policy.h"

namespace {
using namespace msckf;
using namespace msckf_lists;
using msckf_settings::Settings;
namespace inputs = msckf_inputs;
static_assert(inputs::RD_ROW == RD_STRIDE && inputs::NO_IMAGE == IMU_SKIP, "input_layouts.h restates the reading's stride and the skipped cell's count");
static_assert(TRK_MOTION_OK == ST_MOTION_OK && TRK_TRI_VALID == ST_TRI_VALID && TRK_MOTION_SKIPPED == ST_MOTION_SKIPPED, "host_lists.h reads the feature kernel's status bits");

struct Roctx {
  int (*push)(const char*) = nullptr; int (*pop)() = nullptr;
  Roctx() {
    const char* e = getenv("MSCKF_HIP_ROCTX");
    if (!e || !atoi(e)) return;
    void* h = dlopen("librocprofiler-sdk-roctx.so", RTLD_NOW | RTLD_GLOBAL);
    if (!h) h = dlopen("libroctx64.so", RTLD_NOW | RTLD_GLOBAL);
    if (!h) return;
    push = reinterpret_cast<int (*)(const char*)>(dlsym(h, "roctxRangePushA"));
    pop = reinterpret_cast<int (*)()>(dlsym(h, "roctxRangePop"));
    if (!push || !pop) { push = nullptr; pop = nullptr; }
  }
};
const Roctx& roctx() { static Roctx r; return r; }
struct StageRange {
  bool on;
  explicit StageRange(const char* name) : on(roctx().push != nullptr) { if (on) roctx().push(name); }
  ~StageRange() { if (on) roctx().pop(); }
};

thread_local std::string g_err;
int fail(int code, const std::string& msg) { g_err = msg; return code; }

#define HIPCHK(expr)                                                                         \
  do {                                                                                       \
    hipError_t e_ = (expr);                                                                  \
    if (e_ != hipSuccess) return fail(-EIO, std::string(#expr) + ": " + hipGetErrorString(e_)); \
  } while (0)

constexpr int NSTAGE = 13;

struct Workers {
  std::vector<std::thread> th;
  std::mutex m;
  std::condition_variable cv, cv_done;
  std::function<void(int)> job;
  unsigned long gen = 0;
  int active = 0, pending = 0;
  bool stop = false;
  std::vector<int> cpus;
  static void pin_self(int cpu, cpu_set_t* orig, bool* have_orig) {
    if (cpu < 0) {
      if (*have_orig) (void)pthread_setaffinity_np(pthread_self(), sizeof(*orig), orig);
      return;
    }
    if (!*have_orig) { if (pthread_getaffinity_np(pthread_self(), sizeof(*orig), orig) == 0) *have_orig = true; }
    cpu_set_t set; CPU_ZERO(&set); CPU_SET(cpu, &set);
    (void)pthread_setaffinity_np(pthread_self(), sizeof(set), &set);
  }
  void loop(int idx) {
    unsigned long seen = 0;
    int pinned = -2;
    cpu_set_t orig; bool have_orig = false;
    for (;;) {
      std::function<void(int)> f;
      {
        std::unique_lock<std::mutex> lk(m);
        cv.wait(lk, [&] { return stop || gen != seen; });
        if (stop) return;
        seen = gen;
        if (idx >= active) continue;
        f = job;
        const int want = idx + 1 < (int)cpus.size() ? cpus[idx + 1] : -1;
        if (want != pinned) { pin_self(want, &orig, &have_orig); pinned = want; }
      }
      f(idx);
      { std::lock_guard<std::mutex> lk(m); if (--pending == 0) cv_done.notify_all(); }
    }
  }
  void start(int n, std::function<void(int)> f) {
    while ((int)th.size() < n) { const int idx = (int)th.size(); th.emplace_back([this, idx] { loop(idx); }); }
    { std::lock_guard<std::mutex> lk(m); job = std::move(f); active = n; pending = n; ++gen; }
    cv.notify_all();
  }
  void wait() { std::unique_lock<std::mutex> lk(m); cv_done.wait(lk, [&] { return pending == 0; }); }
  ~Workers() {
    { std::lock_guard<std::mutex> lk(m); stop = true; }
    cv.notify_all();
    for (auto& t : th) t.join();
  }
};

struct BatchCore {
  int B = 0, n_cap = 0, f_cap = 0, m_cap = 0, dtype = 0, device = 0;
  bool h16 = false;
  size_t esz = 0;
  std::vector<HostTraj> traj;
  hipStream_t st = nullptr;
  static constexpr int MAXS = 8;
  hipStream_t stx[MAXS] = {nullptr};
  hipEvent_t ev_fork = nullptr, ev_join[MAXS] = {nullptr};
  std::vector<void*> allocs;
  static constexpr int NSTG = 8;
  unsigned char* h_stage[NSTG] = {nullptr}; size_t h_stage_bytes[NSTG] = {0}; hipEvent_t ev_stage[NSTG] = {nullptr}; bool stage_busy[NSTG] = {false};
  int stage_cur = 0;
  std::vector<int> h_ncam;
  hipStream_t sty[MAXS] = {nullptr}; hipEvent_t ev_fa[MAXS] = {nullptr}, ev_fb[MAXS] = {nullptr};
  Settings settings;
  int small_limit = 0;
  bool info_form = false;
  std::vector<double> h_uv;
  std::vector<char> h_imu_ok;
  std::vector<char> h_lit;
  std::vector<char> h_qfull;
  int qroute(int b0, int nb) const {
    int n = 0;
    for (int b = b0; b < b0 + nb; ++b) n += h_qfull[b] ? 1 : 0;
    return n == 0 ? 0 : (n == nb ? 2 : 1);
  }
  int n_lit = 0;
  int* dv_ncam = nullptr; long long* dv_nres = nullptr; int* dv_stats = nullptr;
  int rd_cap = 0;
  void* h_rb = nullptr;
  inputs::SingleBlock wl_blk; int* wl_i = nullptr;
  inputs::ScenarioStore sc;
  bool committed = false;
  unsigned char* sc_dev[inputs::N_SECTIONS] = {nullptr}; size_t sc_total = 0;
  std::vector<void*> sc_allocs;
  static constexpr int RING_MAX = 8;
  hipStream_t stc = nullptr; hipEvent_t ev_up[RING_MAX] = {nullptr}; hipEvent_t ev_use[RING_MAX][MAXS] = {{nullptr}};
  unsigned char* sg_blk[RING_MAX] = {nullptr}; size_t sg_bytes = 0;
  struct PinFrame { unsigned char* p = nullptr; size_t bytes = 0; int chunk = -1; };
  struct PinChunk { void* p = nullptr; int live = 0; };
  std::vector<PinFrame> pinf; std::vector<PinChunk> pin_chunks;
  void unpin_frame(int f) {
    const int c = pinf[f].chunk;
    if (c >= 0 && c < (int)pin_chunks.size() && pin_chunks[c].p && --pin_chunks[c].live == 0) {
      if (stc) (void)hipStreamSynchronize(stc);
      (void)hipHostFree(pin_chunks[c].p);
      pin_chunks[c].p = nullptr;
    }
    pinf[f] = PinFrame();
  }
  void unpin_host() {
    for (auto& q : pin_chunks) if (q.p) hipHostFree(q.p);
    pin_chunks.clear();
    for (auto& pf : pinf) pf = PinFrame();
  }
  msckf_replay::Plan rp;
  unsigned char* rp_dev[inputs::N_SECTIONS] = {nullptr}; std::vector<int> rp_maxcell;
  int* rp_seq_of = nullptr; uint64_t* rp_seed = nullptr; double* rp_sigma = nullptr; int* rp_base = nullptr; size_t rp_base_count = 0;
  bool rp_uploaded = false;
  double* rp_L = nullptr; double* rp_scale = nullptr; double* rp_wstart = nullptr; size_t rp_wstart_count = 0;
  unsigned char* rp_blk[MAXS] = {nullptr}; size_t rp_blk_bytes = 0;
  unsigned char* rp_scratch = nullptr; size_t rp_scratch_bytes = 0;
  std::vector<int> rp_cells[MAXS];
  Workers workers;
  void* log_buf = nullptr; int log_cap = 0, log_n = 0, log_base = 0;
  struct CursorLog {
    int stride; const char* name; const char* api;
    void* buf = nullptr; int* found = nullptr; int cap = 0, ord = 0, base = 0;
    int ordinal(int f, int f0) const { return base + (f - f0); }
  };
  CursorLog map{MAP_STRIDE, "map log", "msckf_hip_map_log"};
  CursorLog prn{PRN_STRIDE, "pruned-state log", "msckf_hip_pruned_log"};
  PrunedFifo prn_list;
  bool prof = false;
  std::vector<std::pair<hipEvent_t, hipEvent_t>> ev_pool[NSTAGE];
  size_t ev_used[NSTAGE] = {0};
  double prof_ms[NSTAGE] = {0}; int prof_cnt[NSTAGE] = {0};

  template <class T> int dalloc(T** p, size_t count, size_t elem = sizeof(T)) {
    void* q = nullptr;
    HIPCHK(hipMalloc(&q, std::max<size_t>(count, 1) * elem));
    HIPCHK(hipMemsetAsync(q, 0, std::max<size_t>(count, 1) * elem, st));
    allocs.push_back(q);
    *p = (T*)q;
    return 0;
  }
  int create() {
    { std::string err; if (!msckf_settings::settings_from_env(settings, err)) return fail(-EINVAL, err); }
    HIPCHK(hipSetDevice(device));
    feature_device_setup(); qr_device_setup(); kalman_device_setup(); gram_device_setup(); literal_device_setup();
    HIPCHK(hipGetLastError());
    HIPCHK(hipStreamCreateWithFlags(&st, hipStreamNonBlocking));
    for (int i = 0; i < NSTG; ++i) HIPCHK(hipEventCreateWithFlags(&ev_stage[i], hipEventDisableTiming));
    stx[0] = st;
    for (int i = 1; i < MAXS; ++i) HIPCHK(hipStreamCreateWithFlags(&stx[i], hipStreamNonBlocking));
    HIPCHK(hipEventCreateWithFlags(&ev_fork, hipEventDisableTiming));
    for (int i = 1; i < MAXS; ++i) HIPCHK(hipEventCreateWithFlags(&ev_join[i], hipEventDisableTiming));
    for (int i = 0; i < MAXS; ++i) {
// ... 641 lines not shown
    stage_begin(12, st);
    launch_replay_walk_scan(reinterpret_cast<const double*>(rp_dev[SEC_RD]), reinterpret_cast<const int*>(rp_dev[SEC_K]), ReplayTrajIn{rp_seq_of, rp_seed, rp_sigma, rp_base},
                            replay_model(0), rp_wstart, rp.frames(), rp.S, rp.K(), B, st);
    stage_end(12, st);
    HIPCHK(hipGetLastError());
    rp.walk_planned = true;
    return 0;
  }
  ReplayModelIn replay_model(int f) const {
    if (rp.model != msckf_replay::MODEL_Q) return ReplayModelIn{nullptr, nullptr, nullptr};
    return ReplayModelIn{rp_L, rp_scale, rp_wstart + (size_t)f * B * msckf_replay::WALK_ROW};
  }
  int replay_walk(int f0, int f1, int b0, int nb, double* out) {
    if (int rc = guard()) return rc;
    if (int rc = refuse(rp.walk_refusal(f0, f1, b0, nb))) return rc;
    if (int rc = enter()) return rc;
    if (int rc = replay_upload_plan()) return rc;
    if (int rc = replay_walk_table()) return rc;
    constexpr int W = msckf_replay::WALK_ROW;
    std::vector<double> rows((size_t)(f1 - f0) * B * W);
    if (!rows.empty()) HIPCHK(hipMemcpyAsync(rows.data(), rp_wstart + (size_t)f0 * B * W, rows.size() * sizeof(double), hipMemcpyDeviceToHost, st));
    HIPCHK(hipStreamSynchronize(st));
    for (int f = 0; f < f1 - f0; ++f) std::copy(rows.begin() + ((size_t)f * B + b0) * W, rows.begin() + ((size_t)f * B + b0 + nb) * W, out + (size_t)f * nb * W);
    return 0;
  }
  int replay_blocks(int nh) {
    const size_t need = rp.block_bytes(esz);
    if (need > rp_blk_bytes) {
      HIPCHK(hipStreamSynchronize(st));
      for (auto& p : rp_blk) dfree(p);
      rp_blk_bytes = need;
    }
    for (int i = 0; i < nh; ++i) if (!rp_blk[i]) HIPCHK(hipMalloc((void**)&rp_blk[i], rp_blk_bytes));
    return 0;
  }
  int run_frames_replay(int f0, int f1) {
    if (int rc = guard()) return rc;
    if (int rc = refuse(rp.run_refusal(f0, f1))) return rc;
    if (int rc = enter()) return rc;
    if (int rc = replay_upload_plan()) return rc;
    if (int rc = replay_walk_table()) return rc;
    const int nh = n_slices(false);
    if (int rc = replay_blocks(nh)) return rc;
    if (int rc = reserve_logs(f0, f1)) return rc;
    for (int i = 0; i < nh; ++i) rp_cells[i].assign((size_t)3 * B, 0);
    const int rc = fork_slices(nh);
    if (rc) return rc;
    int slice_rc[MAXS] = {0};
    auto enqueue = [&](int hh) {
      Slice s = begin_slice(hh, nh);
      for (int f = f0; f < f1; ++f) enqueue_frame(s, f, f0, f1, IN_REPLAY);
      slice_rc[hh] = (int)hipGetLastError();
    };
    if (nh == 1) enqueue(0);
    else {
      workers.start(nh - 1, [&](int idx) { enqueue(idx + 1); });
      enqueue(0);
      workers.wait();
    }
    return finish_slices(nh, slice_rc, f0, f1);
  }
  static constexpr int IN_RESIDENT = -1, IN_REPLAY = -2;
  struct FrameCells { const int* k; const int* drop; const int* maxslot; };
  FrameCells frame_cells(int f, int staged, int hh, int b0, int nb) {
    using namespace inputs;
    if (staged != IN_REPLAY) {
      const size_t cell0 = (size_t)f * B;
      return FrameCells{sc.ints(SEC_K) + cell0, sc.ints(SEC_DROP) + cell0, sc.maxslot.data() + cell0};
    }
    int* c = rp_cells[hh].data();
    for (int b = b0; b < b0 + nb; ++b) {
      const size_t cell = rp.cell_of(f, b);
      c[b] = rp.seq.ints(SEC_K)[cell]; c[B + b] = rp.seq.ints(SEC_DROP)[cell]; c[2 * B + b] = rp.seq.maxslot[cell];
    }
    return FrameCells{c, c + B, c + 2 * B};
  }
  int sync() {
    if (int rc = enter()) return rc;
    HIPCHK(hipStreamSynchronize(st));
    return 0;
  }
  int store(int Settings::* field, int v) { settings.*field = v; apply_settings(); return 0; }
  int set_feature_overlap(int on) { return store(&Settings::overlap_feature, on ? 1 : 0); }
  int set_compression(int route) {
    if (route < -1 || route > 3) return fail(-EINVAL, "route: -1 default, 0 Householder TSQR, 1..3 information form (blocked matrix-core Cholesky; 1 and 2 named retired factorizations)");
    if (route >= 1 && !info_form) return fail(-ENOTSUP, "information form not available for this window size (6 n_cap + 1 > 384 or f_cap > 1024)");
    return store(&Settings::compress_route, route);
  }
  int set_gate_early(int on) { return store(&Settings::gate_early, on ? 1 : 0); }
  int set_cov_update(int form) {
    if (form < 0 || form > 2) return fail(-EINVAL, "form: 0 square-root gain (P - W W^T), 1 Joseph, 2 square-root gain with the register-resident solve");
    return store(&Settings::cov_update, form);
  }
  int set_host_affinity(const int* cpus, int n) {
    std::lock_guard<std::mutex> lk(workers.m);
    workers.cpus.assign(cpus, cpus + std::max(n, 0));
    return 0;
  }
  int set_streams(int n) {
    if (n < 1 || n > MAXS) return fail(-EINVAL, "1 to 8 streams");
    return store(&Settings::nstreams, n);
  }
  int prof_enable(int on) {
    prof = on != 0;
    for (int s = 0; s < NSTAGE; ++s) { ev_used[s] = 0; prof_ms[s] = 0; prof_cnt[s] = 0; }
    return 0;
  }
  int prof_event_overhead(double* ms) {
    if (int rc = enter()) return rc;
    hipEvent_t a, b2;
    HIPCHK(hipEventCreate(&a)); HIPCHK(hipEventCreate(&b2));
    HIPCHK(hipStreamSynchronize(st));
    double tot = 0; const int reps = 64;
    for (int i = 0; i < reps; ++i) {
      HIPCHK(hipEventRecord(a, st)); HIPCHK(hipEventRecord(b2, st));
      HIPCHK(hipEventSynchronize(b2));
      float t = 0; HIPCHK(hipEventElapsedTime(&t, a, b2));
      tot += t;
    }
    hipEventDestroy(a); hipEventDestroy(b2);
    *ms = tot / reps;
    return 0;
  }
  int prof_read(double* ms, int* cnt, int cap) {
    if (int rc = enter()) return rc;
    HIPCHK(hipStreamSynchronize(st));
    for (int s = 0; s < NSTAGE; ++s) {
      for (size_t i = 0; i < ev_used[s]; ++i) {
        float t = 0;
        HIPCHK(hipEventElapsedTime(&t, ev_pool[s][i].first, ev_pool[s][i].second));
        prof_ms[s] += t; prof_cnt[s]++;
      }
      ev_used[s] = 0;
      if (s < cap) { ms[s] = prof_ms[s]; cnt[s] = prof_cnt[s]; }
    }
    return 0;
  }

  virtual int alloc() = 0;
  virtual int init_core(int b, const double* cam, const double* noise, const double* q78, const double* P0, const double* params, const double* imu) = 0;
  virtual int init_full(int b, const double* cam, const double* uv2, const double* Q144, const double* P0_225, const double* params, const double* imu) = 0;
  virtual void mirror_advance(int b, const double* rd, int K) = 0;
  virtual int propagate_device(const inputs::Readings& in, int b0, bool then_augment = false) = 0;
  virtual int augment(int b0, int nb) = 0;
  virtual int set_tracks(int b, int F, const int* M, const int* slots, const double* obs) = 0;
  virtual int marginalize(int b0, int nb, int mode = 0) = 0;
  virtual int set_tracks_range(int b0, int nb, const std::vector<WorkList>& wl) = 0;
  virtual int cams_range(int b0, int nb, double* poses7) = 0;
  virtual int feature_only_range(int b0, int nb, int* status, double* pf3, bool launch) = 0;
  virtual int set_given_range(int b0, int nb, const double* pf3) = 0;
  virtual int prune_keep_range(int b0, int nb, const std::vector<std::vector<int>>& keep) = 0;
  virtual int drop_oldest(int b0, int nb, int n) = 0;
  virtual int get_imu(int b, double* o) = 0;
  virtual int set_imu(int b, const double* in) = 0;
  virtual int get_cams(int b, double* o, int cap, int* n) = 0;
  virtual int get_cams_known(int b, double* o, int n) = 0;
  virtual int set_cam(int b, int slot, const double* in) = 0;
  virtual int get_cov(int b, double* P, int ldo) = 0;
  virtual int set_cov(int b, const double* P, int D) = 0;
  virtual int track_info(int b, double* out, int cap) = 0;
  virtual int track_blocks(int b, int* first, double* Hx, double* rw, double* Bh, int cap) = 0;
  virtual int deltax(int b, double* out, int cap) = 0;
  virtual int scen_set(int f, int b, const double* rd, int k, int F, const int* M, const int* slots, const double* obs, int n_drop, int flags) = 0;
  virtual void enqueue_frame(Slice& s, int f, int f0, int f1, int staged) = 0;
  virtual int replay_expand(int f, int b, double* rd, double* obs, int* ints, int* slots, int cap_entries) = 0;
  virtual void commit_buffer_parity(int f0, int f1) = 0;
// ... 260 lines not shown
  }
  void mirror_advance(int b, const double* rd, int K) override {
    for (int k = 0; k < K; ++k) host_rk(h_imu.data() + (size_t)b * IMU_STRIDE, rd + (size_t)k * RD_STRIDE);
  }
  int propagate_device(const inputs::Readings& in, int b0, bool then_augment) override {
    const int nb = in.nb;
    for (int k0 = 0; k0 < in.kmax; k0 += rd_cap) {
      const int kk = in.rows(k0, rd_cap);
      unsigned char* raw = nullptr;
      int rc = stage_acquire(in.staged_bytes(kk, sizeof(S)), &raw);
      if (rc) return rc;
      S* tmp = reinterpret_cast<S*>(raw); int* hc = reinterpret_cast<int*>(raw + in.counts_at(kk, sizeof(S)));
      in.pack(tmp, hc, k0, kk, rd_cap);
      HIPCHK(hipMemcpyAsync(d_rd, tmp, in.scalars(kk) * sizeof(S), hipMemcpyHostToDevice, st));
      if (in.Kb) HIPCHK(hipMemcpyAsync(d_cnt, hc, nb * sizeof(int), hipMemcpyHostToDevice, st));
      rc = stage_release();
      if (rc) return rc;
      if (in.Kb) launch_propagate<S>(d, b0, nb, d_rd, (long)kk * RD_STRIDE, kk, st, false, qroute(b0, nb), d_cnt);
      else launch_propagate<S>(d, b0, nb, d_rd, (long)kk * RD_STRIDE, kk, st, then_augment && k0 + kk >= in.K, qroute(b0, nb));
      HIPCHK(hipGetLastError());
    }
    return 0;
  }
  int augment(int b0, int nb) override {
    if (int rc = guard()) return rc;
    if (chk_range(b0, nb)) return fail(-EINVAL, "trajectory range out of bounds");
    HIPCHK(hipSetDevice(device));
    if (pend_b >= 0 && pend_b == b0 && nb == 1 && !pend_rd.empty()) {
      const int rc = flush_pending(true);
      if (rc) return rc;
    } else {
      if (int rc = enter()) return rc;
      launch_augment<S>(d, b0, nb, st);
    }
    for (int b = b0; b < b0 + nb; ++b) if (h_ncam[b] < n_cap) h_ncam[b]++;
    HIPCHK(hipGetLastError());
    return 0;
  }
  int set_tracks(int b, int F, const int* M, const int* slots, const double* obs) override {
    if (chk(b)) return fail(-EINVAL, "trajectory index out of range");
    int rc = check_worklist(F, M, slots);
    if (rc) return rc;
    if (int rc = enter()) return rc;
    const size_t nI = wl_blk.ints(F), nO = wl_blk.scalars(F);
    unsigned char* raw = nullptr;
    rc = stage_acquire(wl_blk.staged_bytes(nI, nO, sizeof(S)), &raw);
    if (rc) return rc;
    int* hI = reinterpret_cast<int*>(raw); S* hO = reinterpret_cast<S*>(raw + wl_blk.coords_at(nI));
    wl_blk.pack(hI, hO, F, M, slots, obs);
    HIPCHK(hipMemcpyAsync(wl_i + (size_t)b * wl_blk.ib, hI, (F ? nI : (size_t)wl_blk.M_AT) * sizeof(int), hipMemcpyHostToDevice, st));
    if (F) HIPCHK(hipMemcpyAsync(wl_obs + (size_t)b * wl_blk.ib * 2, hO, nO * sizeof(S), hipMemcpyHostToDevice, st));
    rc = stage_release();
    if (rc) return rc;
    traj[b].wl_F = F;
    return 0;
  }
  int set_tracks_range(int b0, int nb, const std::vector<WorkList>& wl) override {
    if (chk_range(b0, nb) || (int)wl.size() != nb) return fail(-EINVAL, "trajectory range out of bounds");
    for (int i = 0; i < nb; ++i) { const int rc = check_worklist((int)wl[i].M.size(), wl[i].M.data(), wl[i].slots.data()); if (rc) return rc; }
    if (int rc = enter()) return rc;
    const size_t nI = (size_t)nb * wl_blk.ib, nO = (size_t)nb * wl_blk.ib * 2;
    unsigned char* raw = nullptr;
    int rc = stage_acquire(wl_blk.staged_bytes(nI, nO, sizeof(S)), &raw);
    if (rc) return rc;
    int* hI = reinterpret_cast<int*>(raw); S* hO = reinterpret_cast<S*>(raw + wl_blk.coords_at(nI));
    parallel_for(nb, [&](int i) {
      wl_blk.pack(hI + (size_t)i * wl_blk.ib, hO + (size_t)i * wl_blk.ib * 2, (int)wl[i].M.size(), wl[i].M.data(), wl[i].slots.data(), wl[i].obs.data());
      return 0;
    });
    HIPCHK(hipMemcpyAsync(wl_i + (size_t)b0 * wl_blk.ib, hI, nI * sizeof(int), hipMemcpyHostToDevice, st));
    HIPCHK(hipMemcpyAsync(wl_obs + (size_t)b0 * wl_blk.ib * 2, hO, nO * sizeof(S), hipMemcpyHostToDevice, st));
    rc = stage_release();
    if (rc) return rc;
    for (int i = 0; i < nb; ++i) traj[b0 + i].wl_F = (int)wl[i].M.size();
    return 0;
  }
  bool fuse_frame(int f, int f1) const { return settings.fuse_prune && !prof && !settings.overlap_feature && d.joseph == 0 && f + 1 < f1 && !prn.buf; }
  void commit_buffer_parity(int f0, int f1) override {
    int flips = 0;
    for (int f = f0; f < f1; ++f) flips += fuse_frame(f, f1) ? 1 : 0;
    if (flips & 1) std::swap(d.P, P_spare);
  }
  int update_compress() const { return routes::effective_compress(d.compress, settings.compress_route, n_lit); }
  void launch_update(const Dev<S>& vin, int b0, int nb, hipStream_t q, bool feature_done = false, int ncam_ahead = 0, const int* cell_k = nullptr) {
    invalidate_imu(b0, nb);
    Dev<S> v = vin;
    v.compress = update_compress();
    if (!feature_done) { stage_begin(2, q); launch_feature<S>(v, b0, nb, q); stage_end(2, q); }
    const routes::CompressRoute cr = routes::compress_route(v.compress, d.ldR, d.Mp != nullptr, d.lam_part > 0, d.gram_parts);
    stage_begin(7, q); if (cr.select_diag) launch_select_diag<S>(v, b0, nb, q); else launch_select<S>(v, b0, nb, q); stage_end(7, q);
    const routes::SmallRoute sr = routes::small_route(nb, [&](int i) { return routes::window_cols(h_ncam[b0 + i], ncam_ahead, cell_k && cell_k[i] == IMU_SKIP, n_cap); },
                                                      small_limit, v.compress, n_lit, d.joseph, f_cap, sizeof(S), update_small_granted());
    if (sr.kind != routes::CHAIN_ONLY) {
      v.small_split = sr.small_split;
      stage_begin(5, q); launch_update_small<S>(v, b0, nb, q, sr); stage_end(5, q);
      if (sr.kind == routes::SMALL_ONLY) return;
    }
    if (cr.info) {
      stage_begin(3, q);
      launch_gram<S>(v, b0, nb, q, 3);
      stage_end(3, q);
      if (n_lit > 0) {
        if (prof) for (int part = 1; part <= 3; ++part) { stage_begin(7 + part, q); launch_literal<S>(v, b0, nb, q, part); stage_end(7 + part, q); }
        else launch_literal<S>(v, b0, nb, q);
      }
      stage_begin(4, q); launch_gram<S>(v, b0, nb, q, 2); stage_end(4, q);
    } else {
      stage_begin(3, q); launch_compress<S>(v, b0, nb, q, 1); stage_end(3, q);
      stage_begin(4, q); launch_compress<S>(v, b0, nb, q, 2); stage_end(4, q);
    }
    stage_begin(5, q); launch_kalman<S>(v, b0, nb, q); stage_end(5, q);
  }
  int marginalize(int b0, int nb, int mode) override {
    if (int rc = guard()) return rc;
    if (int rc = enter_range(b0, nb)) return rc;
    use_single_worklists();
    Dev<S> v = view(b0);
    v.mode = mode;
    launch_update(v, b0, nb, st);
    HIPCHK(hipGetLastError());
    return 0;
  }
  int cams_range(int b0, int nb, double* poses7) override {
    if (int rc = guard()) return rc;
    if (int rc = enter_range(b0, nb)) return rc;
    const size_t per = (size_t)n_cap * CAM_STRIDE;
    std::vector<S> tmp(per * nb);
    if (const int rc = read_back(tmp.data(), d.cam + (size_t)b0 * per, tmp.size() * sizeof(S))) return rc;
    for (int i = 0; i < nb; ++i)
      for (int c = 0; c < n_cap; ++c)
        for (int k = 0; k < 7; ++k) poses7[((size_t)i * n_cap + c) * 7 + k] = (double)tmp[(size_t)i * per + (size_t)c * CAM_STRIDE + k];
    return 0;
  }
  int feature_only_range(int b0, int nb, int* status, double* pf3, bool launch) override {
    if (int rc = guard()) return rc;
    if (int rc = enter_range(b0, nb)) return rc;
    if (launch) { use_single_worklists(); launch_feature<S>(view(b0), b0, nb, st); HIPCHK(hipGetLastError()); }
    std::vector<int> stt((size_t)nb * f_cap); std::vector<S> pf((size_t)nb * f_cap * 4);
    HIPCHK(hipMemcpyAsync(stt.data(), d.trk_status + (size_t)b0 * f_cap, stt.size() * sizeof(int), hipMemcpyDeviceToHost, st));
    HIPCHK(hipMemcpyAsync(pf.data(), d.trk_pf + (size_t)b0 * f_cap * 4, pf.size() * sizeof(S), hipMemcpyDeviceToHost, st));
    HIPCHK(hipStreamSynchronize(st));
    for (size_t t = 0; t < stt.size(); ++t) { status[t] = stt[t]; for (int k = 0; k < 3; ++k) pf3[3 * t + k] = (double)pf[4 * t + k]; }
    return 0;
  }
  int set_given_range(int b0, int nb, const double* pf3) override {
    if (int rc = enter_range(b0, nb)) return rc;
    const size_t cnt = (size_t)nb * f_cap * 4;
    unsigned char* raw = nullptr;
    int rc = stage_acquire(cnt * sizeof(S), &raw);
    if (rc) return rc;
    S* tmp = reinterpret_cast<S*>(raw);
    for (size_t t = 0; t < (size_t)nb * f_cap; ++t) { for (int k = 0; k < 3; ++k) tmp[4 * t + k] = (S)pf3[3 * t + k]; tmp[4 * t + 3] = S(0); }
    HIPCHK(hipMemcpyAsync(d_pfin + (size_t)b0 * f_cap * 4, tmp, cnt * sizeof(S), hipMemcpyHostToDevice, st));
    return stage_release();
  }
  int prune_keep_range(int b0, int nb, const std::vector<std::vector<int>>& keep) override {
    if (int rc = guard()) return rc;
    if (chk_range(b0, nb) || (int)keep.size() != nb) return fail(-EINVAL, "trajectory range out of bounds");
    if (int rc = enter()) return rc;
    const size_t nI = (size_t)nb * n_cap + nb;
    unsigned char* raw = nullptr;
    int rc = stage_acquire(nI * sizeof(int), &raw);
    if (rc) return rc;
    int* hk = reinterpret_cast<int*>(raw); int* hn = hk + (size_t)nb * n_cap;
    std::memset(hk, 0, nI * sizeof(int));
    for (int i = 0; i < nb; ++i) {
      const int nk = (int)keep[i].size();
      if (nk > n_cap) return fail(-EINVAL, "keep list longer than n_cap");
      hn[i] = nk;
      for (int k = 0; k < nk; ++k) hk[(size_t)i * n_cap + k] = keep[i][k];
    }
    HIPCHK(hipMemcpyAsync(d.keep + (size_t)b0 * n_cap, hk, (size_t)nb * n_cap * sizeof(int), hipMemcpyHostToDevice, st));
    HIPCHK(hipMemcpyAsync(d.nkeep + b0, hn, nb * sizeof(int), hipMemcpyHostToDevice, st));
// ... 28 lines not shown
    if (int rc = enter_traj(b)) return rc;
    S tmp[IMU_STRIDE] = {0};
    for (int i = 0; i < 29; ++i) tmp[i] = (S)in[i];
    if (const int rc = write_dev(d.imu + (size_t)b * IMU_STRIDE, tmp, sizeof(tmp))) return rc;
    std::copy(tmp, tmp + IMU_STRIDE, h_imu.begin() + (size_t)b * IMU_STRIDE); h_imu_ok[b] = 1;
    return 0;
  }
  int get_cams(int b, double* o, int cap, int* nout) override {
    if (int rc = guard()) return rc;
    int n = 0;
    int rc = get_ncam(b, &n);
    if (rc) return rc;
    *nout = n;
    if (n > cap) return fail(-E2BIG, "output buffer too small");
    std::vector<S> tmp((size_t)std::max(n, 1) * CAM_STRIDE);
    if (n) HIPCHK(hipMemcpyAsync(tmp.data(), d.cam + (size_t)b * n_cap * CAM_STRIDE, (size_t)n * CAM_STRIDE * sizeof(S), hipMemcpyDeviceToHost, st));
    HIPCHK(hipStreamSynchronize(st));
    for (int i = 0; i < n; ++i) for (int k = 0; k < 7; ++k) o[7 * i + k] = (double)tmp[(size_t)i * CAM_STRIDE + k];
    return 0;
  }
  int get_cams_known(int b, double* o, int n) override {
    if (int rc = guard()) return rc;
    if (chk(b) || n < 0 || n > n_cap) return fail(-EINVAL, "index out of range");
    if (int rc = enter()) return rc;
    S* tmp = static_cast<S*>(h_rb); S* tim = tmp + (size_t)n_cap * CAM_STRIDE;
    if (n) HIPCHK(hipMemcpyAsync(tmp, d.cam + (size_t)b * n_cap * CAM_STRIDE, (size_t)n * CAM_STRIDE * sizeof(S), hipMemcpyDeviceToHost, st));
    const bool want_imu = !h_imu_ok[b];
    if (want_imu) HIPCHK(hipMemcpyAsync(tim, d.imu + (size_t)b * IMU_STRIDE, IMU_STRIDE * sizeof(S), hipMemcpyDeviceToHost, st));
    HIPCHK(hipStreamSynchronize(st));
    if (want_imu) { std::copy(tim, tim + IMU_STRIDE, h_imu.begin() + (size_t)b * IMU_STRIDE); h_imu_ok[b] = 1; }
    for (int i = 0; i < n; ++i) for (int k = 0; k < 7; ++k) o[7 * i + k] = (double)tmp[(size_t)i * CAM_STRIDE + k];
    return 0;
  }
  int set_cam(int b, int slot, const double* in) override {
    if (chk(b) || slot < 0 || slot >= n_cap) return fail(-EINVAL, "index out of range");
    if (int rc = enter()) return rc;
    S tmp[CAM_STRIDE] = {0};
    for (int k = 0; k < 7; ++k) tmp[k] = (S)in[k];
    return write_dev(d.cam + ((size_t)b * n_cap + slot) * CAM_STRIDE, tmp, sizeof(tmp));
  }
  int get_cov(int b, double* P, int ldo) override {
    if (int rc = guard()) return rc;
    int n = 0;
    int rc = get_ncam(b, &n);
    if (rc) return rc;
    const int D = 15 + 6 * n;
    if (ldo < D) return fail(-EINVAL, "ld smaller than D");
    std::vector<S> tmp((size_t)d.ld * d.ld);
    if (const int rc = read_back(tmp.data(), d.P + (size_t)b * d.ld * d.ld, tmp.size() * sizeof(S))) return rc;
    for (int j = 0; j < D; ++j) for (int i = 0; i < D; ++i) P[(size_t)j * ldo + i] = (double)tmp[(size_t)j * d.ld + i];
    return 0;
  }
  int set_cov(int b, const double* P, int D) override {
    if (chk(b)) return fail(-EINVAL, "trajectory index out of range");
    if (D < 15 || (D - 15) % 6 || (D - 15) / 6 > n_cap) return fail(-EINVAL, "bad covariance dimension");
    if (int rc = enter()) return rc;
    std::vector<S> tmp((size_t)d.ld * d.ld, S(0));
    for (int j = 0; j < D; ++j) for (int i = 0; i < D; ++i) tmp[(size_t)j * d.ld + i] = (S)P[(size_t)j * D + i];
    const int n = (D - 15) / 6;
    HIPCHK(hipMemcpyAsync(d.P + (size_t)b * d.ld * d.ld, tmp.data(), tmp.size() * sizeof(S), hipMemcpyHostToDevice, st));
    HIPCHK(hipMemcpyAsync(d.ncam + b, &n, sizeof(int), hipMemcpyHostToDevice, st));
    HIPCHK(hipStreamSynchronize(st));
    h_ncam[b] = n;
    return 0;
  }
  int copy_from(BatchCore* src) override {
    if (int rc = guard()) return rc;
    Batch<S>* o = dynamic_cast<Batch<S>*>(src);
    if (!o || o->B != B || o->n_cap != n_cap || o->f_cap != f_cap || o->m_cap != m_cap || o->h16 != h16 || (d.lit.W2 && !d.lit.X && o->settings.lit_route == 1))
      return fail(-EINVAL, "copy_state: handles differ in shape or dtype");
    if (o->poisoned) return fail(-EIO, "copy_state: the source handle is unusable after a failed run_frames call (its filter states are undefined)");
    { const int rcf = o->flush_pending(); if (rcf) return rcf; }
    for (int b = 0; b < o->B; ++b) { const int rcm = resolve_map(o, b); if (rcm) return rcm; }
    if (int rc = enter()) return rc;
    HIPCHK(hipStreamSynchronize(o->st));
    const size_t Bz = B, pl = (size_t)d.ld * d.ld;
    auto cp = [&](void* dst, const void* sp, size_t bytes) { return hipMemcpyAsync(dst, sp, bytes, hipMemcpyDeviceToDevice, st); };
    HIPCHK(cp(d.imu, o->d.imu, Bz * IMU_STRIDE * sizeof(S))); HIPCHK(cp(d.cam, o->d.cam, Bz * n_cap * CAM_STRIDE * sizeof(S)));
    HIPCHK(cp(d.prm, o->d.prm, Bz * PRM_STRIDE * sizeof(S))); HIPCHK(cp(d.P, o->d.P, Bz * pl * sizeof(S)));
    HIPCHK(cp(d.qf, o->d.qf, Bz * QF_STRIDE * sizeof(S)));
    HIPCHK(cp(d.ncam, o->d.ncam, Bz * sizeof(int))); HIPCHK(cp(d.n_resid, o->d.n_resid, Bz * sizeof(long long)));
    HIPCHK(cp(d.stats, o->d.stats, Bz * STAT_STRIDE * sizeof(int))); HIPCHK(cp(d.ncam_upd, o->d.ncam_upd, Bz * sizeof(int)));
    traj = o->traj; h_ncam = o->h_ncam; h_uv = o->h_uv; h_imu = o->h_imu; h_imu_ok = o->h_imu_ok; h_qfull = o->h_qfull;
    settings.take_over(o->settings);
    prn_list.forget(h_ncam);
    HIPCHK(hipStreamSynchronize(st));
    std::fill(h_lit.begin(), h_lit.end(), 0); n_lit = 0;
    return set_aniso(settings.aniso_mode, settings.lit_tol);
  }
  int track_info(int b, double* out, int cap) override {
    if (int rc = enter_traj(b)) return rc;
    int tmp[STAT_STRIDE];
    if (const int rc = read_back(tmp, d.stats + (size_t)b * STAT_STRIDE, sizeof(tmp))) return rc;
    const int F = tmp[STAT_NTRACKS];
    if (F > cap) return fail(-E2BIG, "output buffer too small");
    std::vector<int> stt(std::max(F, 1)); std::vector<S> gm(std::max(F, 1)), pf((size_t)std::max(F, 1) * 4);
    if (F) {
      HIPCHK(hipMemcpyAsync(stt.data(), d.trk_status + (size_t)b * f_cap, F * sizeof(int), hipMemcpyDeviceToHost, st));
      HIPCHK(hipMemcpyAsync(gm.data(), d.trk_gamma + (size_t)b * f_cap, F * sizeof(S), hipMemcpyDeviceToHost, st));
      HIPCHK(hipMemcpyAsync(pf.data(), d.trk_pf + (size_t)b * f_cap * 4, (size_t)F * 4 * sizeof(S), hipMemcpyDeviceToHost, st));
      HIPCHK(hipStreamSynchronize(st));
    }
    for (int t = 0; t < F; ++t) {
      double* o = out + 8 * t;
      const bool skipped = stt[t] & ST_MOTION_SKIPPED;
      o[0] = (skipped || (stt[t] & ST_MOTION_OK)) ? 1 : 0;
      o[1] = (stt[t] & ST_TRI_VALID) ? 1 : 0; o[2] = (stt[t] & ST_GATE_PASS) ? 1 : 0; o[3] = (stt[t] & ST_INCLUDED) ? 1 : 0;
      o[4] = (double)gm[t]; o[5] = (double)pf[4 * t]; o[6] = (double)pf[4 * t + 1]; o[7] = (double)pf[4 * t + 2];
    }
    return F;
  }
  int track_blocks(int b, int* first, double* Hx, double* rw, double* Bh, int cap) override {
    if (int rc = enter_traj(b)) return rc;
    if (!d.trk_B || !d.trk_Hx || !d.trk_rw) return fail(-ENOTSUP, "the per-track blocks exist on the information-form route with an f32 / f64 Jacobian only");
    int tmp[STAT_STRIDE];
    if (const int rc = read_back(tmp, d.stats + (size_t)b * STAT_STRIDE, sizeof(tmp))) return rc;
    const int F = tmp[STAT_NTRACKS];
    if (F > cap) return fail(-E2BIG, "output buffer too small");
    if (!F) return 0;
    const size_t tb = (size_t)b * f_cap, nh = (size_t)F * m_cap * 12, nr = (size_t)F * 2 * m_cap, ldR = (size_t)d.ldR, nB = (size_t)F * 3 * ldR, nc = 6 * (size_t)n_cap + 1;
    std::vector<S> hx(nh), r(nr); std::vector<double> bb(nB);
    HIPCHK(hipMemcpyAsync(first, d.trk_first + tb, F * sizeof(int), hipMemcpyDeviceToHost, st));
    HIPCHK(hipMemcpyAsync(hx.data(), d.trk_Hx + tb * m_cap * 12, nh * sizeof(S), hipMemcpyDeviceToHost, st));
    HIPCHK(hipMemcpyAsync(r.data(), d.trk_rw + tb * 2 * m_cap, nr * sizeof(S), hipMemcpyDeviceToHost, st));
    HIPCHK(hipMemcpyAsync(bb.data(), d.trk_B + tb * 3 * ldR, nB * sizeof(double), hipMemcpyDeviceToHost, st));
    HIPCHK(hipStreamSynchronize(st));
    for (size_t i = 0; i < nh; ++i) Hx[i] = (double)hx[i];
    for (size_t i = 0; i < nr; ++i) rw[i] = (double)r[i];
    for (size_t q = 0; q < (size_t)F * 3; ++q) for (size_t c = 0; c < nc; ++c) Bh[q * nc + c] = bb[q * ldR + c];
    return F;
  }
  int deltax(int b, double* out, int cap) override {
    int n = 0;
    int rc = get_ncam(b, &n);
    if (rc) return rc;
    const int D = 15 + 6 * n;
    if (D > cap) return fail(-E2BIG, "output buffer too small");
    std::vector<S> tmp(D);
    if (const int rc = read_back(tmp.data(), d.dx + (size_t)b * d.ld, D * sizeof(S))) return rc;
    for (int i = 0; i < D; ++i) out[i] = (double)tmp[i];
    return D;
  }
  int scen_set(int f, int b, const double* rd, int k, int F, const int* M, const int* slots, const double* obs, int n_drop, int flags) override {
    if (f < 0 || f >= sc.frames || chk(b)) return fail(-EINVAL, "scenario cell out of range");
    { const int rc = check_worklist(F, M, slots); if (rc) return rc; }
    if (n_drop < 0) return fail(-EINVAL, "negative n_drop");
    if (const char* why = cell_refusal(k, sc.lay.K, F, n_drop, flags)) return fail(-EINVAL, why);
    if (k > 0 && !rd) return fail(-EINVAL, "null readings for a cell with samples");
    sc.set_cell<S>(f, b, rd, k, (flags & CELL_SKIP) != 0, F, M, slots, obs, n_drop);
    committed = false;
    unpin_frame(f);
    return 0;
  }
  using FrameIn = inputs::FrameIn<S>;
  FrameIn resident_frame(int f, int b0) const {
    return inputs::frame_in<S>(sc.lay, b0, [&](int s) { return sc_dev[s] + sc.lay.resident_at(s, f, sc.fr_base[f]); });
  }
  FrameIn staged_frame(int f, int k, int b0) const {
    return inputs::frame_in<S>(sc.lay, b0, [&](int s) { return sg_blk[k] + sc.lay.block_at(s, sc.entries(f)); });
  }
  ReplaySeqIn replay_seq(int f) const {
    using namespace inputs;
    const ScenarioStore& q = rp.seq;
    auto at = [&](int s) { return rp_dev[s] + q.lay.resident_at(s, f, q.fr_base[f]); };
    auto i = [&](int s) { return reinterpret_cast<const int*>(at(s)); };
    return ReplaySeqIn{reinterpret_cast<const double*>(at(SEC_RD)), i(SEC_N), i(SEC_DROP), i(SEC_K), i(SEC_M), i(SEC_OFF), i(SEC_SLOTS), reinterpret_cast<const double*>(at(SEC_OBS))};
  }
  ReplayTrajIn replay_traj(int f) const { return ReplayTrajIn{rp_seq_of, rp_seed, rp_sigma, rp_base + (size_t)f * B}; }
  ReplayOut<S> replay_out(unsigned char* blk, int f) const {
    using namespace inputs;
    const FrameLayout L = rp.out_layout(sizeof(S));
    auto at = [&](int s) { return blk + L.block_at(s, rp.nf[f]); };
    auto i = [&](int s) { return reinterpret_cast<int*>(at(s)); };
    return ReplayOut<S>{reinterpret_cast<S*>(at(SEC_RD)), i(SEC_N), i(SEC_DROP), i(SEC_K), i(SEC_M), i(SEC_OFF), i(SEC_SLOTS), reinterpret_cast<S*>(at(SEC_OBS))};
  }
  FrameIn replay_frame(int f, int hh, int b0) const {
    const inputs::FrameLayout L = rp.out_layout(sizeof(S));
    return inputs::frame_in<S>(L, b0, [&](int s) { return rp_blk[hh] + L.block_at(s, rp.nf[f]); });
  }
  int replay_expand(int f, int b, double* rd, double* obs, int* ints, int* slots, int cap_entries) override {
    using namespace inputs;
    if (int rc = guard()) return rc;
    if (int rc = refuse(rp.expand_refusal(f, b))) return rc;
    if (int rc = enter()) return rc;
    if (int rc = replay_upload_plan()) return rc;
    if (int rc = replay_walk_table()) return rc;
    const int K = rp.K(), E = (int)rp.entries(rp.seq_of[b], f);
    if (E > cap_entries) return fail(-E2BIG, "output buffer too small for the cell's entries");
    const size_t need = rp.block_bytes(sizeof(S));
    if (need > rp_scratch_bytes) {
      HIPCHK(hipStreamSynchronize(st));
      dfree(rp_scratch); rp_scratch_bytes = 0;
      HIPCHK(hipMalloc((void**)&rp_scratch, need));
      rp_scratch_bytes = need;
    }
    const ReplayOut<S> o = replay_out(rp_scratch, f);
    launch_replay_expand<S>(replay_seq(f), replay_traj(f), replay_model(f), o, f, b, 1, K, f_cap, rp_maxcell[f], st);
    HIPCHK(hipGetLastError());
    const size_t base = (size_t)rp.base[(size_t)f * B + b];
    std::vector<S> hr((size_t)K * RD_STRIDE), ho((size_t)2 * std::max(E, 1));
    std::vector<int> hi((size_t)3 + 2 * f_cap), hs(std::max(E, 1));
    HIPCHK(hipMemcpyAsync(hr.data(), o.rd + (size_t)b * K * RD_STRIDE, hr.size() * sizeof(S), hipMemcpyDeviceToHost, st));
    if (E) HIPCHK(hipMemcpyAsync(ho.data(), o.obs + 2 * base, (size_t)2 * E * sizeof(S), hipMemcpyDeviceToHost, st));
    if (E) HIPCHK(hipMemcpyAsync(hs.data(), o.slots + base, (size_t)E * sizeof(int), hipMemcpyDeviceToHost, st));
    HIPCHK(hipMemcpyAsync(&hi[0], o.n + b, sizeof(int), hipMemcpyDeviceToHost, st));
    HIPCHK(hipMemcpyAsync(&hi[1], o.drop + b, sizeof(int), hipMemcpyDeviceToHost, st));
    HIPCHK(hipMemcpyAsync(&hi[2], o.k + b, sizeof(int), hipMemcpyDeviceToHost, st));
    HIPCHK(hipMemcpyAsync(&hi[3], o.M + (size_t)b * f_cap, (size_t)f_cap * sizeof(int), hipMemcpyDeviceToHost, st));
    HIPCHK(hipMemcpyAsync(&hi[3 + f_cap], o.off + (size_t)b * f_cap, (size_t)f_cap * sizeof(int), hipMemcpyDeviceToHost, st));
    HIPCHK(hipStreamSynchronize(st));
    if (rd) for (size_t i = 0; i < hr.size(); ++i) rd[i] = (double)hr[i];
    if (obs) for (int i = 0; i < 2 * E; ++i) obs[i] = (double)ho[i];
    if (ints) std::copy(hi.begin(), hi.end(), ints);
    if (slots) std::copy(hs.begin(), hs.begin() + E, slots);
    return E;
  }
  void enqueue_frame(Slice& s, int f, int f0, int f1, int staged) override {
    const int b0 = s.b0, nb = s.nb, hh = s.hh;
    const bool replay = staged == IN_REPLAY;
    const FrameIn in = replay ? replay_frame(f, hh, b0) : staged == IN_RESIDENT ? resident_frame(f, b0) : staged_frame(f, staged, b0);
    const bool may_overlap = staged == IN_RESIDENT;
    hipStream_t q = s.q;
    const FrameCells cells = frame_cells(f, staged, hh, b0, nb);
    const int* cell_k = cells.k; const int* cell_drop = cells.drop;
    const int K = replay ? rp.K() : sc.lay.K;
    if (replay) { stage_begin(11, q); launch_replay_expand<S>(replay_seq(f), replay_traj(f), replay_model(f), replay_out(rp_blk[hh], f), f, b0, nb, K, f_cap, rp_maxcell[f], q); stage_end(11, q); }
    Dev<S> v = d;
    v.P = s.flipped ? P_spare : d.P; v.ncam_defer = s.pending ? 1 : 0;
    const bool fuse = fuse_frame(f, f1);
    v.trk_n = in.n; v.trk_M = in.M; v.trk_off = in.off; v.trk_slots = in.slots; v.trk_obs = in.obs;
    v.wl_stride_n = 1; v.wl_stride_f = f_cap; v.wl_stride_o = 0;
    bool early = may_overlap && settings.overlap_feature && !prof && f > f0;
    for (int b = b0; b < b0 + nb && early; ++b) {
      const int n_after = std::min(h_ncam[b] + 1, n_cap);
      early = h_ncam[b] < n_cap && cells.maxslot[b] <= n_after - 2 && cell_k[b] != IMU_SKIP;
    }
    if (early) {
      (void)hipEventRecord(ev_fa[hh], q);
      (void)hipStreamWaitEvent(sty[hh], ev_fa[hh], 0);
      Dev<S> v2 = v; v2.ncam_bias = 1;
      v2.compress = update_compress();
      launch_feature<S>(v2, b0, nb, sty[hh]);
      (void)hipEventRecord(ev_fb[hh], sty[hh]);
    }
    {
      StageRange r("imu_prop+msckf_augment_state");
      stage_begin(0, q); launch_propagate<S>(v, b0, nb, in.rd, (long)K * RD_STRIDE, K, q, !prof, qroute(b0, nb), in.k); stage_end(0, q);
      if (prof) { stage_begin(1, q); launch_augment<S>(v, b0, nb, q, in.k); stage_end(1, q); }
    }
    if (early) (void)hipStreamWaitEvent(q, ev_fb[hh], 0);
    v.ncam_defer = 0;
    if (fuse) { v.Pout = s.flipped ? d.P : P_spare; v.fuse_drop = in.drop; }
    { StageRange r(fuse ? "msckf_marginalize+msckf_prune_empty_states" : "msckf_marginalize"); launch_update(v, b0, nb, q, early, 1, cell_k + b0); }
    if (fuse) s.flipped = !s.flipped;
    else {
      if (prn.buf) launch_pruned_log<S>(v, b0, nb, q, in.drop, prn.ordinal(f, f0), prn.cap, static_cast<S*>(prn.buf), prn.found);
      StageRange r("msckf_prune_empty_states");
      stage_begin(6, q);
      launch_prune<S>(v, b0, nb, q, in.drop, 0);
      stage_end(6, q);
    }
    s.pending = fuse;
    if (log_buf) launch_frame_log<S>(d, b0, nb, q, s.flipped ? P_spare : d.P, s.pending, static_cast<S*>(log_buf) + (size_t)(log_base + (f - f0)) * B * LOG_STRIDE);
    if (map.buf) launch_map_log<S>(d, b0, nb, q, in.n, in.M, map.ordinal(f, f0), map.cap, static_cast<S*>(map.buf), map.found);
    for (int b = b0; b < b0 + nb; ++b) {
      const bool augmented = h_ncam[b] < n_cap && cell_k[b] != IMU_SKIP;
      if (augmented) h_ncam[b]++;
      const int nd = std::max(0, std::min(cell_drop[b], h_ncam[b]));
      h_ncam[b] -= nd;
      if (prn.buf) prn_list.mirror(b, augmented, nd, prn.ordinal(f, f0), prn.cap);
    }
  }
  int frame_log_read(int r0, int n, int b0, int nb, double* out) override {
    if (int rc = guard()) return rc;
    if (r0 < 0 || n < 0 || (long)r0 + n > log_n) return fail(-EINVAL, "record range beyond the records written (msckf_hip_frame_log_count)");
    if (int rc = enter_range(b0, nb)) return rc;
    const size_t row = (size_t)nb * LOG_STRIDE;
    std::vector<S> tmp(std::max<size_t>(row * n, 1));
    if (n && nb)
      HIPCHK(hipMemcpy2DAsync(tmp.data(), row * sizeof(S), static_cast<const S*>(log_buf) + ((size_t)r0 * B + b0) * LOG_STRIDE, (size_t)B * LOG_STRIDE * sizeof(S),
                              row * sizeof(S), (size_t)n, hipMemcpyDeviceToHost, st));
    HIPCHK(hipStreamSynchronize(st));
    for (size_t i = 0; i < row * n; ++i) out[i] = (double)tmp[i];
    return 0;
  }
  int frame_log_metrics(int r0, int r1, const double* gt_p, double* out, const int* r0b, const int* r1b) override {
    if (int rc = guard()) return rc;
    if (r0 < 0 || r1 < r0 || r1 > log_n) return fail(-EINVAL, "record range beyond the records written (msckf_hip_frame_log_count)");
    if (int rc = enter()) return rc;
    std::vector<int> rb;
    if (r0b) { rb.assign(r0b, r0b + B); rb.insert(rb.end(), r1b, r1b + B); }
    return log_metrics_call("frame_log_metrics", gt_p, (size_t)(r1 - r0) * B * 3, rb.data(), rb.size(), out, (size_t)B * 6, [&](const double* dg, double* dout, const int* dr) {
      launch_log_metrics<S>(static_cast<const S*>(log_buf), B, r0, r1, r0b ? dr : nullptr, r0b ? dr + B : nullptr, dg, dout, st);
    });
  }
  int cursor_log_copy(const CursorLog& g, int b, int r0, int n, double* out) {
    if (!n) return 0;
    std::vector<S> tmp((size_t)n * g.stride);
    if (const int rc = read_back(tmp.data(), static_cast<const S*>(g.buf) + ((size_t)b * g.cap + r0) * g.stride, tmp.size() * sizeof(S))) return rc;
    for (size_t i = 0; i < tmp.size(); ++i) out[i] = (double)tmp[i];
    return 0;
  }
  int cursor_log_read(CursorLog& g, int b, int r0, int n, double* out) {
    if (int rc = cursor_log_check_range(g, b, r0, n)) return rc;
    return cursor_log_copy(g, b, r0, n, out);
  }
  int map_log_read(int b, int r0, int n, double* out) override { return cursor_log_read(map, b, r0, n, out); }
  int map_log_metrics(int q0, int q1, const double* gt_xyz, const int* gt_off, double* out) override {
    if (int rc = guard()) return rc;
    if (int rc = map_log_check_gt(q0, q1, gt_xyz, gt_off)) return rc;
    if (int rc = enter()) return rc;
    const size_t cells = (size_t)(q1 - q0) * B, noff = gt_off ? cells + 1 : 0, ng = gt_off ? (size_t)gt_off[cells] * 3 : 0;
    return log_metrics_call("map_log_metrics", gt_xyz, ng, gt_off, noff, out, (size_t)B * 8, [&](const double* dg, double* dout, const int* doff) {
      launch_map_metrics<S>(static_cast<const S*>(map.buf), map.found, map.cap, B, q0, q1, gt_off ? dg : nullptr, gt_off ? doff : nullptr, dout, st);
    });
  }
  int pruned_log_read(int b, int r0, int n, double* out, int* aug_ord) override {
    if (int rc = cursor_log_check_range(prn, b, r0, n)) return rc;
    if (!n) return 0;
    const std::vector<int>& aug = prn_list.aug[b];
    if ((int)aug.size() < r0 + n) return fail(-EIO, "pruned-state log: fewer augment ordinals on the host than records on the device");
    if (int rc = cursor_log_copy(prn, b, r0, n, out)) return rc;
    if (aug_ord) std::copy(aug.begin() + r0, aug.begin() + r0 + n, aug_ord);
    return 0;
  }
  int pruned_log_metrics(int q0, int q1, const double* gt_pose, int n_ord, double* out) override {
    if (int rc = guard()) return rc;
    if (int rc = cursor_log_check_ordinals(prn, q0, q1)) return rc;
    if (n_ord < 0 || (n_ord > 0 && !gt_pose)) return fail(-EINVAL, "gt_pose: n_ord poses per trajectory, n_ord >= 0, null only with n_ord == 0");
    if (int rc = enter()) return rc;
    std::vector<int> aug((size_t)B * prn.cap, -1);
    for (int b = 0; b < B; ++b) std::copy(prn_list.aug[b].begin(), prn_list.aug[b].end(), aug.begin() + (size_t)b * prn.cap);
    return log_metrics_call("pruned_log_metrics", gt_pose, (size_t)n_ord * B * 7, aug.data(), aug.size(), out, (size_t)B * 10, [&](const double* dg, double* dout, const int* daug) {
      launch_pruned_metrics<S>(static_cast<const S*>(prn.buf), prn.found, prn.cap, B, q0, q1, daug, dg, n_ord, dout, st);
    });
  }
// ... 439 lines not shown
  if (b < 0 || b >= H(h)->B) return fail(-EINVAL, "trajectory index out of range");
  const auto& cams = H(h)->traj[b].cams;
  if ((int)cams.size() > cap) return fail(-E2BIG, "output buffer too small");
  for (size_t i = 0; i < cams.size(); ++i) {
    if (time) time[i] = cams[i].time;
    if (n_tracked) n_tracked[i] = (int)cams[i].tracked.size();
    if (last_correlated_ids) last_correlated_ids[i] = cams[i].last_correlated_id;
  }
  return (int)cams.size();
}
int msckf_hip_get_tracked_feature_ids(msckf_hip_handle h, int b, int cam_index, uint64_t* ids, int cap) {
  if (b < 0 || b >= H(h)->B) return fail(-EINVAL, "trajectory index out of range");
  const auto& cams = H(h)->traj[b].cams;
  if (cam_index < 0 || cam_index >= (int)cams.size()) return fail(-EINVAL, "camera index out of range");
  const auto& tr = cams[(size_t)cam_index].tracked;
  if ((int)tr.size() > cap) return fail(-E2BIG, "output buffer too small");
  std::copy(tr.begin(), tr.end(), ids);
  return (int)tr.size();
}
int msckf_hip_get_covariance(msckf_hip_handle h, int b, double* P, int ld) { return H(h)->get_cov(b, P, ld); }
int msckf_hip_set_covariance(msckf_hip_handle h, int b, const double* P, int D) { return H(h)->set_cov(b, P, D); }
int msckf_hip_set_imu_state(msckf_hip_handle h, int b, const double* imu29) { return H(h)->set_imu(b, imu29); }
int msckf_hip_set_cam_pose(msckf_hip_handle h, int b, int slot, const double* cam7) { return H(h)->set_cam(b, slot, cam7); }
int msckf_hip_get_num_residualized(msckf_hip_handle h, int b, long long* n) { return H(h)->get_nres(b, n); }
int msckf_hip_set_num_residualized(msckf_hip_handle h, int b, long long n) { return H(h)->set_nres(b, n); }
int msckf_hip_last_stats(msckf_hip_handle h, int b, int* out7) { return H(h)->stats(b, out7); }
int msckf_hip_clear_error_flags(msckf_hip_handle h, int b) { if (!h) return fail(-EINVAL, "null handle"); return H(h)->clear_errors(b); }
int msckf_hip_last_tracks(msckf_hip_handle h, int b, double* out8, int cap) { return H(h)->track_info(b, out8, cap); }
int msckf_hip_last_deltax(msckf_hip_handle h, int b, double* dx, int cap) { return H(h)->deltax(b, dx, cap); }
int msckf_hip_last_track_blocks(msckf_hip_handle h, int b, int* first, double* Hx, double* rw, double* Bh, int cap) { return H(h)->track_blocks(b, first, Hx, rw, Bh, cap); }

int msckf_hip_set_tracks(msckf_hip_handle h, int b, int F, const int* M, const int* slots, const double* obs2) { return H(h)->set_tracks(b, F, M, slots, obs2); }
int msckf_hip_propagate_range(msckf_hip_handle h, int b0, int nb, const double* readings7, int K) { return H(h)->propagate(b0, nb, readings7, K); }
int msckf_hip_propagate_range_counts(msckf_hip_handle h, int b0, int nb, const double* readings7, const int* K) {
  if (!h || (nb > 0 && !K)) return fail(-EINVAL, "null argument");
  return H(h)->propagate_counts(b0, nb, readings7, K);
}
int msckf_hip_augment_range(msckf_hip_handle h, int b0, int nb) { return H(h)->augment(b0, nb); }
int msckf_hip_marginalize_range(msckf_hip_handle h, int b0, int nb) { return H(h)->marginalize(b0, nb, 0); }
int msckf_hip_drop_oldest_range(msckf_hip_handle h, int b0, int nb, int n_drop) { return H(h)->drop_oldest(b0, nb, n_drop); }

int msckf_hip_scenario_alloc(msckf_hip_handle h, int n_frames, int K) { return H(h)->scen_alloc(n_frames, K); }
int msckf_hip_scenario_set(msckf_hip_handle h, int frame, int b, const double* readings7, int F, const int* M, const int* slots, const double* obs2, int n_drop) {
  if (!h) return fail(-EINVAL, "null handle");
  return H(h)->scen_set(frame, b, readings7, H(h)->sc.lay.K, F, M, slots, obs2, n_drop, 0);
}
static_assert(MSCKF_HIP_CELL_SKIP == CELL_SKIP, "host_lists.h states the cell rule with the header's flag bit");
int msckf_hip_scenario_set_cell(msckf_hip_handle h, int frame, int b, const double* readings7, int k, int F, const int* M, const int* slots, const double* obs2, int n_drop, int flags) {
  if (!h) return fail(-EINVAL, "null handle");
  return H(h)->scen_set(frame, b, readings7, k, F, M, slots, obs2, n_drop, flags);
}
int msckf_hip_scenario_commit(msckf_hip_handle h) { return H(h)->scen_commit(); }
int msckf_hip_run_frames(msckf_hip_handle h, int f0, int f1) { return H(h)->run_frames(f0, f1); }
int msckf_hip_run_frames_streamed(msckf_hip_handle h, int f0, int f1) { return H(h)->run_frames_streamed(f0, f1); }
int msckf_hip_replay_alloc(msckf_hip_handle h, int n_seq, int n_frames, int K) { if (!h) return fail(-EINVAL, "null handle"); return H(h)->replay_alloc(n_seq, n_frames, K); }
int msckf_hip_replay_set_cell(msckf_hip_handle h, int frame, int seq, const double* readings7, int k, int F, const int* M, const int* slots, const double* obs2, int n_drop, int flags) {
  if (!h) return fail(-EINVAL, "null handle");
  return H(h)->replay_set_cell(frame, seq, readings7, k, F, M, slots, obs2, n_drop, flags);
}
int msckf_hip_replay_assign(msckf_hip_handle h, const int* seq_of, const uint64_t* seed, const double* sigma4) { if (!h || !seq_of || !seed || !sigma4) return fail(-EINVAL, "null argument"); return H(h)->replay_assign(seq_of, seed, sigma4); }
int msckf_hip_replay_assign_q(msckf_hip_handle h, const int* seq_of, const uint64_t* seed, const double* Q144, const double* scale, const double* sigma_uv) {
  if (!h || !seq_of || !seed || !Q144 || !scale || !sigma_uv) return fail(-EINVAL, "null argument");
  return H(h)->replay_assign_q(seq_of, seed, Q144, scale, sigma_uv);
}
int msckf_hip_replay_walk(msckf_hip_handle h, int f0, int f1, int b0, int nb, double* out) { if (!h || !out) return fail(-EINVAL, "null argument"); return H(h)->replay_walk(f0, f1, b0, nb, out); }
int msckf_hip_replay_commit(msckf_hip_handle h) { if (!h) return fail(-EINVAL, "null handle"); return H(h)->replay_commit(); }
int msckf_hip_run_frames_replay(msckf_hip_handle h, int f0, int f1) { if (!h) return fail(-EINVAL, "null handle"); return H(h)->run_frames_replay(f0, f1); }
int msckf_hip_replay_expand(msckf_hip_handle h, int frame, int b, double* rd, double* obs2, int cap_entries) { if (!h || !rd || !obs2) return fail(-EINVAL, "null argument"); return H(h)->replay_expand(frame, b, rd, obs2, nullptr, nullptr, cap_entries); }
int msckf_hip_replay_expand_ints(msckf_hip_handle h, int frame, int b, int* ints, int* slots, int cap_entries) { if (!h || !ints || !slots) return fail(-EINVAL, "null argument"); return H(h)->replay_expand(frame, b, nullptr, nullptr, ints, slots, cap_entries); }
int msckf_hip_sync(msckf_hip_handle h) { return H(h)->sync(); }
int msckf_hip_profile_enable(msckf_hip_handle h, int on) { return H(h)->prof_enable(on); }
int msckf_hip_profile_read(msckf_hip_handle h, double* ms7, int* count7) { return H(h)->prof_read(ms7, count7, 8); }
int msckf_hip_profile_read_ex(msckf_hip_handle h, double* ms, int* count, int cap) { if (!h || !ms || !count || cap < 8) return fail(-EINVAL, "bad arguments"); for (int s = NSTAGE; s < cap; ++s) { ms[s] = 0; count[s] = 0; } return H(h)->prof_read(ms, count, cap); }
int msckf_hip_profile_event_overhead(msckf_hip_handle h, double* ms) { if (!h || !ms) return fail(-EINVAL, "null argument"); return H(h)->prof_event_overhead(ms); }
int msckf_hip_set_host_affinity(msckf_hip_handle h, const int* cpus, int n) { if (!h || (n > 0 && !cpus)) return fail(-EINVAL, "null argument"); return H(h)->set_host_affinity(cpus, n); }
int msckf_hip_set_streams(msckf_hip_handle h, int n) { return H(h)->set_streams(n); }
int msckf_hip_get_effective_streams(msckf_hip_handle h, int streamed, int* out) { if (!h || !out) return fail(-EINVAL, "null argument"); *out = H(h)->n_slices(streamed != 0); return 0; }
int msckf_hip_parse_hw_queues(const char* text) { return msckf::slices::parse_hw_queue_budget(text); }
int msckf_hip_set_hw_queues(msckf_hip_handle h, int n) { if (!h) return fail(-EINVAL, "null handle"); return H(h)->set_hw_queues(n); }
int msckf_hip_set_slices_exact(msckf_hip_handle h, int on) { if (!h) return fail(-EINVAL, "null handle"); H(h)->slices_exact = on != 0; return 0; }
int msckf_hip_scenario_pin(msckf_hip_handle h, int f0, int f1) { if (!h) return fail(-EINVAL, "null handle"); return H(h)->scen_pin(f0, f1); }
int msckf_hip_set_upload_ring(msckf_hip_handle h, int depth, int mode) { if (!h) return fail(-EINVAL, "null handle"); return H(h)->set_upload_ring(depth, mode); }
int msckf_hip_set_feature_overlap(msckf_hip_handle h, int on) { if (!h) return fail(-EINVAL, "null handle"); return H(h)->set_feature_overlap(on); }
int msckf_hip_set_covariance_update(msckf_hip_handle h, int form) { if (!h) return fail(-EINVAL, "null handle"); return H(h)->set_cov_update(form); }
int msckf_hip_set_compression(msckf_hip_handle h, int route) { if (!h) return fail(-EINVAL, "null handle"); return H(h)->set_compression(route); }
int msckf_hip_set_gate_early_accept(msckf_hip_handle h, int on) { if (!h) return fail(-EINVAL, "null handle"); return H(h)->set_gate_early(on); }
int msckf_hip_set_anisotropic_noise(msckf_hip_handle h, int mode, double tail_tol) { if (!h) return fail(-EINVAL, "null handle"); return H(h)->set_aniso(mode, tail_tol); }
int msckf_hip_copy_state(msckf_hip_handle dst, msckf_hip_handle src) { if (!dst || !src) return fail(-EINVAL, "null handle"); return H(dst)->copy_from(H(src)); }
int msckf_hip_get_error_flags(msckf_hip_handle h, int b, int* flags) { if (!h || !flags) return fail(-EINVAL, "null argument"); return H(h)->error_flags(b, flags); }
int msckf_hip_frame_log_enable(msckf_hip_handle h, int capacity_frames) { if (!h) return fail(-EINVAL, "null handle"); return H(h)->frame_log_enable(capacity_frames); }
int msckf_hip_frame_log_reset(msckf_hip_handle h) { if (!h) return fail(-EINVAL, "null handle"); return H(h)->frame_log_reset(); }
int msckf_hip_frame_log_count(msckf_hip_handle h) { if (!h) return fail(-EINVAL, "null handle"); return H(h)->frame_log_count(); }
int msckf_hip_frame_log_read(msckf_hip_handle h, int r0, int n, int b0, int nb, double* out) { if (!h || !out) return fail(-EINVAL, "null argument"); return H(h)->frame_log_read(r0, n, b0, nb, out); }
int msckf_hip_frame_log_metrics(msckf_hip_handle h, int r0, int r1, const double* gt_p, double* out) { if (!h || !gt_p || !out) return fail(-EINVAL, "null argument"); return H(h)->frame_log_metrics(r0, r1, gt_p, out); }
int msckf_hip_frame_log_metrics_ranges(msckf_hip_handle h, const int* r0, const int* r1, const double* gt_p, double* out) { if (!h || !r0 || !r1 || !gt_p || !out) return fail(-EINVAL, "null argument"); return H(h)->frame_log_metrics_ranges(r0, r1, gt_p, out); }
int msckf_hip_map_log_enable(msckf_hip_handle h, int capacity_per_trajectory) { if (!h) return fail(-EINVAL, "null handle"); return H(h)->map_log_enable(capacity_per_trajectory); }
int msckf_hip_map_log_reset(msckf_hip_handle h) { if (!h) return fail(-EINVAL, "null handle"); return H(h)->map_log_reset(); }
int msckf_hip_map_log_frames(msckf_hip_handle h) { if (!h) return fail(-EINVAL, "null handle"); return H(h)->map_log_frames(); }
int msckf_hip_map_log_counts(msckf_hip_handle h, int b0, int nb, int* stored, int* found) { if (!h || !stored || !found) return fail(-EINVAL, "null argument"); return H(h)->map_log_counts(b0, nb, stored, found); }
int msckf_hip_map_log_read(msckf_hip_handle h, int b, int r0, int n, double* out) { if (!h || !out) return fail(-EINVAL, "null argument"); return H(h)->map_log_read(b, r0, n, out); }
int msckf_hip_map_log_metrics(msckf_hip_handle h, int q0, int q1, const double* gt_xyz, const int* gt_off, double* out) { if (!h || !out) return fail(-EINVAL, "null argument"); return H(h)->map_log_metrics(q0, q1, gt_xyz, gt_off, out); }
int msckf_hip_pruned_log_enable(msckf_hip_handle h, int capacity_per_trajectory) { if (!h) return fail(-EINVAL, "null handle"); return H(h)->pruned_log_enable(capacity_per_trajectory); }
int msckf_hip_pruned_log_reset(msckf_hip_handle h) { if (!h) return fail(-EINVAL, "null handle"); return H(h)->pruned_log_reset(); }
int msckf_hip_pruned_log_frames(msckf_hip_handle h) { if (!h) return fail(-EINVAL, "null handle"); return H(h)->pruned_log_frames(); }
int msckf_hip_pruned_log_counts(msckf_hip_handle h, int b0, int nb, int* stored, int* found) { if (!h || !stored || !found) return fail(-EINVAL, "null argument"); return H(h)->pruned_log_counts(b0, nb, stored, found); }
int msckf_hip_pruned_log_read(msckf_hip_handle h, int b, int r0, int n, double* out, int* aug_ord) { if (!h || !out || !aug_ord) return fail(-EINVAL, "null argument"); return H(h)->pruned_log_read(b, r0, n, out, aug_ord); }
int msckf_hip_pruned_log_metrics(msckf_hip_handle h, int q0, int q1, const double* gt_pose, int n_ord, double* out) { if (!h || !out) return fail(-EINVAL, "null argument"); return H(h)->pruned_log_metrics(q0, q1, gt_pose, n_ord, out); }
int msckf_hip_literal_info(msckf_hip_handle h, int b, int* out8) { if (!h || !out8) return fail(-EINVAL, "null argument"); return H(h)->lit_info(b, out8); }

}
```

msckf_mono_amd/csrc/settings.h:

```cpp
#ifndef MSCKF_SETTINGS_H
#define MSCKF_SETTINGS_H

#include <cstdlib>
#include <string>

namespace msckf_settings {

struct Settings {
  int nstreams = 1;
  int fuse_prune = 1;
  int overlap_feature = 0;
  int compress_route = -1;
  int small_update = 84;
  int gain_parts = 0;
  int fused_s = 2;
  int feat_pair = 1;
  int cov_update = 0;
  int gate_early = 0;
  int aniso_mode = 0;
  double lit_tol = -1;
  int lit_route = 0;
  int lit_serial = 0;
  int lit_timers = 0;
  int ring = 6, up_mode = 0;
  int test_fail_upload = -1;
  inline void take_over(const Settings& o);
};

enum { KEPT = 0, COPIED = 1 };
enum { NUMBER = 0, FLAG = 1 };
struct SettingRow {
  const char* env;
  int Settings::* field = nullptr;
  double Settings::* dfield = nullptr;
  int copied = KEPT, flag = NUMBER;
  const int* allowed = nullptr; int n_allowed = 0; const char* refusal = nullptr;
};
inline constexpr int GAIN_PARTS_ALLOWED[] = {0, 2, 4};
inline constexpr SettingRow SETTINGS_TABLE[] = {
    {nullptr, &Settings::nstreams, nullptr, COPIED},
    {"MSCKF_HIP_FUSE_PRUNE", &Settings::fuse_prune, nullptr, COPIED, FLAG},
    {nullptr, &Settings::overlap_feature, nullptr, COPIED},
    {nullptr, &Settings::compress_route, nullptr, COPIED},
    {"MSCKF_HIP_SMALL_UPDATE", &Settings::small_update, nullptr, COPIED},
    {"MSCKF_HIP_GAIN_PARTS", &Settings::gain_parts, nullptr, COPIED, NUMBER, GAIN_PARTS_ALLOWED, 3, "MSCKF_HIP_GAIN_PARTS must be 0, 2 or 4"},
    {"MSCKF_HIP_FUSED_S", &Settings::fused_s, nullptr, COPIED},
    {"MSCKF_HIP_FEATURE_PAIR", &Settings::feat_pair, nullptr, COPIED},
    {nullptr, &Settings::cov_update, nullptr, COPIED},
    {nullptr, &Settings::gate_early, nullptr, COPIED},
    {nullptr, &Settings::aniso_mode, nullptr, COPIED},
    {nullptr, nullptr, &Settings::lit_tol, COPIED},
    {"MSCKF_HIP_LITERAL_ROUTE", &Settings::lit_route, nullptr, COPIED},
    {"MSCKF_HIP_LITERAL_SERIAL", &Settings::lit_serial, nullptr, COPIED},
    {"MSCKF_HIP_LITERAL_TIMERS", &Settings::lit_timers, nullptr, KEPT, FLAG},
    {nullptr, &Settings::ring, nullptr, KEPT},
    {nullptr, &Settings::up_mode, nullptr, KEPT},
    {"MSCKF_HIP_TEST_FAIL_UPLOAD", &Settings::test_fail_upload, nullptr, KEPT},
    {"MSCKF_HIP_ROCTX"},
    {"MSCKF_HIP_HOST_THREADS"},
    {"MSCKF_HIP_CYCLE_TIMERS"},
};

inline void Settings::take_over(const Settings& o) {
  for (const SettingRow& r : SETTINGS_TABLE) {
    if (r.copied != COPIED) continue;
    if (r.field) this->*r.field = o.*r.field;
    if (r.dfield) this->*r.dfield = o.*r.dfield;
  }
}

inline bool settings_from_env(Settings& s, std::string& err) {
  for (const SettingRow& r : SETTINGS_TABLE) {
    const char* e = (r.env && r.field) ? getenv(r.env) : nullptr;
    if (!e) continue;
    const int v = r.flag == FLAG ? atoi(e) != 0 : atoi(e);
    bool ok = r.n_allowed == 0;
    for (int i = 0; i < r.n_allowed; ++i) ok = ok || v == r.allowed[i];
    if (!ok) { err = r.refusal; return false; }
    s.*r.field = v;
  }
  return true;
}

}
#endif
```

Measured before the change: 218,300 updates/s.

## Fuse feature selection/diagonal Gram into propagate kernel via feature-first frame order

Adds a feature-first frame order in which the select/diag-Gram work for the update runs as extra blocks inside the propagate kernel (a HEAD variant with a 2D grid), so it is no longer a separate launch after propagation. The select and diag bodies move into a shared header so both kernels can call them, and they use an update_ncam helper to read the camera count valid before augmentation. A host-side gate refuses the route for doubles, non-diag routes, the first frame, profiling, a full window, skipped frames, or when tracks already reference the newest slot. This cuts launch count and serialization per frame, at the cost of extra complexity and a larger grid for the propagate kernel.

```diff
diff --git a/include/msckf_hip.h b/include/msckf_hip.h
--- a/include/msckf_hip.h
+++ b/include/msckf_hip.h
@@ -116,6 +116,8 @@
 int msckf_hip_set_compression(msckf_hip_handle h, int route);
 int msckf_hip_set_covariance_update(msckf_hip_handle h, int form);
 int msckf_hip_set_feature_overlap(msckf_hip_handle h, int on);
+int msckf_hip_set_frame_order(msckf_hip_handle h, int order);
+int msckf_hip_get_frame_order_count(msckf_hip_handle h, long long* count);
 int msckf_hip_set_anisotropic_noise(msckf_hip_handle h, int mode, double tail_tol);
 int msckf_hip_literal_info(msckf_hip_handle h, int b, int* out8);
 
diff --git a/msckf_mono_amd/capi.py b/msckf_mono_amd/capi.py
--- a/msckf_mono_amd/capi.py
+++ b/msckf_mono_amd/capi.py
@@ -34,6 +34,7 @@
     "msckf_hip_pruned_log_enable", "msckf_hip_pruned_log_reset", "msckf_hip_pruned_log_frames", "msckf_hip_pruned_log_counts", "msckf_hip_pruned_log_read", "msckf_hip_pruned_log_metrics",
     "msckf_hip_replay_alloc", "msckf_hip_replay_set_cell", "msckf_hip_replay_assign", "msckf_hip_replay_commit", "msckf_hip_run_frames_replay", "msckf_hip_replay_expand",
     "msckf_hip_replay_expand_ints", "msckf_hip_replay_assign_q", "msckf_hip_replay_walk", "msckf_hip_last_track_blocks",
+    "msckf_hip_set_frame_order", "msckf_hip_get_frame_order_count",
 ]
 CELL_SKIP = 1
 
@@ -411,6 +412,14 @@
     def set_feature_overlap(self, on):
         _chk(self.L.msckf_hip_set_feature_overlap(self.h, 1 if on else 0))
 
+    def set_frame_order(self, order):
+        _chk(self.L.msckf_hip_set_frame_order(self.h, int(order)))
+
+    def frame_order_count(self):
+        n = C.c_longlong(0)
+        _chk(self.L.msckf_hip_get_frame_order_count(self.h, C.byref(n)))
+        return n.value
+
     def set_gate_early_accept(self, on):
         _chk(self.L.msckf_hip_set_gate_early_accept(self.h, 1 if on else 0))
 
diff --git a/msckf_mono_amd/csrc/dev_common.h b/msckf_mono_amd/csrc/dev_common.h
--- a/msckf_mono_amd/csrc/dev_common.h
+++ b/msckf_mono_amd/csrc/dev_common.h
@@ -398,6 +398,7 @@
 template <class S> void launch_feature(const Dev<S>& d, int b0, int nb, hipStream_t st);
 template <class S> void launch_select(const Dev<S>& d, int b0, int nb, hipStream_t st);
 template <class S> void launch_select_diag(const Dev<S>& d, int b0, int nb, hipStream_t st);
+template <class S> void launch_frame_head(const Dev<S>& d, int b0, int nb, const S* readings, long rd_stride, int K, hipStream_t st, int qroute, const int* cnt);
 template <class S> void launch_compress(const Dev<S>& d, int b0, int nb, hipStream_t st, int phase);
 template <class S> void launch_gram(const Dev<S>& d, int b0, int nb, hipStream_t st, int phase);
 template <class S> void launch_kalman(const Dev<S>& d, int b0, int nb, hipStream_t st);
diff --git a/msckf_mono_amd/csrc/frame_order.h b/msckf_mono_amd/csrc/frame_order.h
--- /dev/null
+++ b/msckf_mono_amd/csrc/frame_order.h
@@ -0,0 +1,57 @@
+#ifndef MSCKF_FRAME_ORDER_H
+#define MSCKF_FRAME_ORDER_H
+
+#include <cstddef>
+
+namespace msckf {
+namespace routes {
+
+enum FrameOrderRefusal {
+  FO_TAKEN = 0,
+  FO_SETTING,
+  FO_SCALAR,
+  FO_ROUTE,
+  FO_FIRST_FRAME,
+  FO_PROFILE,
+  FO_WINDOW_FULL,
+  FO_SKIPPED,
+  FO_NEWEST_SEEN
+};
+inline const char* frame_order_text(FrameOrderRefusal r) {
+  switch (r) {
+    case FO_TAKEN: return "feature_first";
+    case FO_SETTING: return "setting";
+    case FO_SCALAR: return "double";
+    case FO_ROUTE: return "route";
+    case FO_FIRST_FRAME: return "first_frame";
+    case FO_PROFILE: return "profile";
+    case FO_WINDOW_FULL: return "window_full";
+    case FO_SKIPPED: return "skipped";
+    case FO_NEWEST_SEEN: return "newest_seen";
+  }
+  return "?";
+}
+
+inline FrameOrderRefusal feature_ahead(int nb, const int* ncam, const int* maxslot, const int* k, int skip_mark, int n_cap, bool first_frame, bool prof) {
+  if (first_frame) return FO_FIRST_FRAME;
+  if (prof) return FO_PROFILE;
+  for (int i = 0; i < nb; ++i) {
+    if (ncam[i] >= n_cap) return FO_WINDOW_FULL;
+    if (k[i] == skip_mark) return FO_SKIPPED;
+    const int n_after = ncam[i] + 1;
+    if (maxslot[i] > n_after - 2) return FO_NEWEST_SEEN;
+  }
+  return FO_TAKEN;
+}
+
+inline FrameOrderRefusal frame_order(int setting, int overlap_feature, size_t scalar, bool select_diag, int qroute,
+                                     int nb, const int* ncam, const int* maxslot, const int* k, int skip_mark, int n_cap, bool first_frame, bool prof) {
+  if (!setting || overlap_feature) return FO_SETTING;
+  if (scalar != 4) return FO_SCALAR;
+  if (!select_diag || qroute == 1) return FO_ROUTE;
+  return feature_ahead(nb, ncam, maxslot, k, skip_mark, n_cap, first_frame, prof);
+}
+
+}
+}
+#endif
diff --git a/msckf_mono_amd/csrc/kernels_feature.hip b/msckf_mono_amd/csrc/kernels_feature.hip
--- a/msckf_mono_amd/csrc/kernels_feature.hip
+++ b/msckf_mono_amd/csrc/kernels_feature.hip
@@ -1,5 +1,6 @@
 #include "chi2_table.h"
 #include "dev_common.h"
+#include "select_diag.h"
 
 namespace msckf {
 
@@ -1341,239 +1342,8 @@
 }
 
 template <class S>
-__device__ __forceinline__ void select_body(const Dev<S>& d, const int b0, const int nb, const int i, const int lane) {
-  if (i >= nb) return;
-  const int b = b0 + i;
-  const int F = d.trk_n[(long)i * d.wl_stride_n];
-  long long nres = d.n_resid[b];
-  int* st = d.stats + (long)b * STAT_STRIDE;
-  int mrej = 0, trej = 0, grej = 0, pass = 0;
-  int* rs = d.row_start + (long)b * (d.f_cap + 1);
-  int* order = d.trk_order + (long)b * d.f_cap;
-  __shared__ int sCnt[64], sBase[64], sRows[64];
-  sCnt[lane] = 0; sRows[lane] = 0;
-  __syncthreads();
-  if (!(nres <= 3 && d.mode == 0) && F <= 256) {
-    __shared__ short sMrow[256];
-    __shared__ short sOrd[256];
-    int sv[4], Mv[4], fv[4];
-    bool inc[4];
-#pragma unroll
-    for (int c = 0; c < 4; ++c) {
-      const int t = 64 * c + lane, tc = min(t, max(F - 1, 0));
-      const long tb = (long)b * d.f_cap + tc;
-      sv[c] = d.trk_status[tb]; Mv[c] = d.trk_M[(long)i * d.wl_stride_f + tc]; fv[c] = d.trk_first[tb] & 63;
-    }
-#pragma unroll
-    for (int c = 0; c < 4; ++c) {
-      const int t = 64 * c + lane;
-      const bool in = t < F;
-      int sx = in ? sv[c] : 0;
-      const int M = in ? Mv[c] : 0;
-      bool m_rej = false, t_rej = false, g_rej = false, valid = false, incl = false;
-      if (in) {
-        if (M < 2 || !(sx & ST_MOTION_OK)) { m_rej = true; sx = (M < 2) ? 0 : (sx & ~(ST_TRI_VALID | ST_GATE_PASS)); }
-        else if (sx & ST_TRI_VALID) valid = true;
-        else { t_rej = true; sx &= ~ST_GATE_PASS; }
-        if (valid) { if (sx & ST_GATE_PASS) { incl = true; sx |= ST_INCLUDED; } else g_rej = true; }
-        d.trk_status[(long)b * d.f_cap + t] = sx;
-        sMrow[t] = (short)(2 * M - 3);
-      }
-      inc[c] = incl;
-      if (incl) { atomicAdd(&sCnt[fv[c]], 1); atomicAdd(&sRows[fv[c]], 2 * M - 3); }
-      mrej += __popcll(__ballot(m_rej)); trej += __popcll(__ballot(t_rej)); grej += __popcll(__ballot(g_rej));
-      pass += __popcll(__ballot(incl)); if (d.mode == 0) nres += __popcll(__ballot(valid));
-    }
-    __syncthreads();
-    {
-      const int c0 = sCnt[lane];
-      int scan = c0;
-#pragma unroll
-      for (int o = 1; o < 64; o <<= 1) { const int up = __shfl_up(scan, o, 64); if (lane >= o) scan += up; }
-      sBase[lane] = scan - c0;
-    }
-    __syncthreads();
-    const int nbin = min(d.n_cap, 64);
-#pragma unroll
-    for (int c = 0; c < 4; ++c) {
-      const int bin = inc[c] ? fv[c] : -1;
-      int rank = 0, cnt = 0;
-      for (int sbin = 0; sbin < nbin; ++sbin) {
-        const unsigned long long m = __ballot(bin == sbin);
-        if (bin == sbin) { rank = __popcll(m & ((1ull << lane) - 1ull)); cnt = __popcll(m); }
-      }
-      int pos = 0;
-      if (inc[c]) { pos = sBase[bin] + rank; sOrd[pos] = (short)(64 * c + lane); order[pos] = 64 * c + lane; }
-      __syncthreads();
-      if (inc[c] && rank == 0) sBase[bin] += cnt;
-      __syncthreads();
-    }
-    int rows = 0;
-    for (int p0 = 0; p0 < pass; p0 += 64) {
-      const int p = p0 + lane;
-      const int r = p < pass ? (int)sMrow[sOrd[p]] : 0;
-      int scan = r;
-#pragma unroll
-      for (int o = 1; o < 64; o <<= 1) { const int up = __shfl_up(scan, o, 64); if (lane >= o) scan += up; }
-      if (p < pass) rs[p] = rows + scan - r;
-      rows += __shfl(scan, 63, 64);
-    }
-    if (lane == 0) {
-      rs[pass] = rows;
-      d.n_resid[b] = nres;
-      st[STAT_NTRACKS] = F; st[STAT_MOTION_REJ] = mrej; st[STAT_TRI_REJ] = trej; st[STAT_GATE_REJ] = grej;
-      st[STAT_PASSED] = pass; st[STAT_MROWS] = rows; st[STAT_RROWS] = rows > 0 ? 6 * d.ncam[b] : 0;
-    }
-    return;
-  }
-  if (nres <= 3 && d.mode == 0) {
-    if (lane == 0) {
-      for (int t = 0; t < F; ++t) {
-        const long tb = (long)b * d.f_cap + t;
-        int s = d.trk_status[tb];
-        const int M = d.trk_M[(long)i * d.wl_stride_f + t];
-        bool valid = false;
-        if (M < 2) { if (nres > 3) mrej++; else trej++; s = 0; }
-        else if (nres > 3 && !(s & ST_MOTION_OK)) { mrej++; s &= ~(ST_TRI_VALID | ST_GATE_PASS); }
-        else {
-          if (nres <= 3) s |= ST_MOTION_SKIPPED;
-          if (s & ST_TRI_VALID) { valid = true; nres++; } else { trej++; s &= ~ST_GATE_PASS; }
-        }
-        if (valid) {
-          if (s & ST_GATE_PASS) { s |= ST_INCLUDED; pass++; const int f0 = d.trk_first[tb] & 63; sCnt[f0]++; sRows[f0] += 2 * M - 3; }
-          else grej++;
-        }
-        d.trk_status[tb] = s;
-      }
-    }
-    mrej = __shfl(mrej, 0, 64); trej = __shfl(trej, 0, 64); grej = __shfl(grej, 0, 64); pass = __shfl(pass, 0, 64);
-    nres = __shfl((int)nres, 0, 64);
-  } else {
-    for (int t0 = 0; t0 < F; t0 += 64) {
-      const int t = t0 + lane;
-      const bool in = t < F;
-      const long tb = (long)b * d.f_cap + t;
-      int s = in ? d.trk_status[tb] : 0;
-      const int M = in ? d.trk_M[(long)i * d.wl_stride_f + t] : 0;
-      bool m_rej = false, t_rej = false, g_rej = false, valid = false, incl = false;
-      if (in) {
-        if (M < 2 || !(s & ST_MOTION_OK)) { m_rej = true; s = (M < 2) ? 0 : (s & ~(ST_TRI_VALID | ST_GATE_PASS)); }
-        else if (s & ST_TRI_VALID) valid = true;
-        else { t_rej = true; s &= ~ST_GATE_PASS; }
-        if (valid) { if (s & ST_GATE_PASS) { incl = true; s |= ST_INCLUDED; } else g_rej = true; }
-        d.trk_status[tb] = s;
-      }
-      if (incl) { const int f0 = d.trk_first[tb] & 63; atomicAdd(&sCnt[f0], 1); atomicAdd(&sRows[f0], 2 * M - 3); }
-      mrej += __popcll(__ballot(m_rej)); trej += __popcll(__ballot(t_rej)); grej += __popcll(__ballot(g_rej));
-      pass += __popcll(__ballot(incl)); if (d.mode == 0) nres += __popcll(__ballot(valid));
-    }
-  }
-  __syncthreads();
-  {
-    const int c = sCnt[lane];
-    int scan = c;
-#pragma unroll
-    for (int o = 1; o < 64; o <<= 1) { const int up = __shfl_up(scan, o, 64); if (lane >= o) scan += up; }
-    sBase[lane] = scan - c;
-  }
-  __syncthreads();
-  for (int t0 = 0; t0 < F; t0 += 64) {
-    const int t = t0 + lane;
-    const long tb = (long)b * d.f_cap + t;
-    const bool incl = (t < F) && (d.trk_status[tb] & ST_INCLUDED);
-    const int bin = incl ? (d.trk_first[tb] & 63) : -1;
-    int pos = -1;
-    for (int sbin = 0; sbin < d.n_cap && sbin < 64; ++sbin) {
-      const unsigned long long m = __ballot(bin == sbin);
-      if (bin == sbin) pos = sBase[sbin] + __popcll(m & ((1ull << lane) - 1ull));
-      __syncthreads();
-      if (lane == 0) sBase[sbin] += __popcll(m);
-      __syncthreads();
-    }
-    if (incl) order[pos] = t;
-  }
-  __syncthreads();
-  int rows = 0;
-  for (int p0 = 0; p0 < pass; p0 += 64) {
-    const int p = p0 + lane;
-    int r = 0;
-    if (p < pass) { const int t = order[p]; r = 2 * d.trk_M[(long)i * d.wl_stride_f + t] - 3; }
-    int scan = r;
-#pragma unroll
-    for (int o = 1; o < 64; o <<= 1) { const int up = __shfl_up(scan, o, 64); if (lane >= o) scan += up; }
-    if (p < pass) rs[p] = rows + scan - r;
-    rows += __shfl(scan, 63, 64);
-  }
-  if (lane == 0) {
-    rs[pass] = rows;
-    d.n_resid[b] = nres;
-    st[STAT_NTRACKS] = F; st[STAT_MOTION_REJ] = mrej; st[STAT_TRI_REJ] = trej; st[STAT_GATE_REJ] = grej;
-    st[STAT_PASSED] = pass; st[STAT_MROWS] = rows; st[STAT_RROWS] = rows > 0 ? 6 * d.ncam[b] : 0;
-  }
-}
-
-template <class S>
 __global__ __launch_bounds__(64) void k_select(Dev<S> d, int b0, int nb) { select_body<S>(d, b0, nb, (int)blockIdx.x, (int)threadIdx.x); }
 
-template <class S>
-__global__ __launch_bounds__(256) void k_select_diag(Dev<S> d, int b0, int nb, int ndiag) {
-  const int tid = threadIdx.x, lane = tid & 63, w = tid >> 6, i = blockIdx.y;
-  if ((int)blockIdx.x == ndiag) { if (tid < 64) select_body<S>(d, b0, nb, i, tid); return; }
-  const int b = b0 + i;
-  const int N = d.ncam[b], F = d.trk_n[(long)i * d.wl_stride_n];
-  const int s = 4 * (int)blockIdx.x + w;
-  if (s >= N) return;
-  const int f_cap = d.f_cap, m_cap = d.m_cap;
-  const int* stt = d.trk_status + (long)b * f_cap;
-  const int* Mv = d.trk_M + (long)i * d.wl_stride_f;
-  constexpr int ALL = ST_MOTION_OK | ST_TRI_VALID | ST_GATE_PASS;
-  int tcut = 0;
-  if (d.mode == 0 && F > 0) {
-    int need = 4 - d.nres_upd[b];
-    if (need > 0) {
-      tcut = F;
-      for (int t0 = 0; t0 < F && need > 0; t0 += 64) {
-        const int t = t0 + lane;
-        const bool v = t < F && Mv[t] >= 2 && (stt[t] & ST_TRI_VALID);
-        unsigned long long m = __ballot(v);
-        const int c = __popcll(m);
-        if (c < need) { need -= c; continue; }
-        int pos = 0;
-        for (int k = 0; k < need; ++k) { pos = __builtin_ctzll(m); m &= m - 1; }
-        tcut = t0 + pos + 1; need = 0;
-      }
-    }
-  }
-  double acc[27];
-#pragma unroll
-  for (int e = 0; e < 27; ++e) acc[e] = 0.0;
-  for (int t = lane; t < F; t += 64) {
-    const long tb = (long)b * f_cap + t;
-    const int sx = stt[t], M = Mv[t];
-    const int oi = d.trk_inv[tb * d.n_cap + s];
-    const int need_bits = t < tcut ? (ST_TRI_VALID | ST_GATE_PASS) : ALL;
-    if (M < 2 || (sx & need_bits) != need_bits || oi < 0) continue;
-    const long h0i = (tb * m_cap + oi) * 12;
-    const S* rw = d.trk_rw + tb * 2 * m_cap + 2 * oi;
-    double h0[6], h1[6];
-#pragma unroll
-    for (int k = 0; k < 6; ++k) { h0[k] = (double)ld_hx(d, h0i + k); h1[k] = (double)ld_hx(d, h0i + 6 + k); }
-    const double r0 = (double)rw[0], r1 = (double)rw[1];
-    int e = 0;
-#pragma unroll
-    for (int a = 0; a < 6; ++a)
-#pragma unroll
-      for (int c = a; c < 6; ++c) acc[e++] += h0[a] * h0[c] + h1[a] * h1[c];
-#pragma unroll
-    for (int a = 0; a < 6; ++a) acc[21 + a] += h0[a] * r0 + h1[a] * r1;
-  }
-  double* out = d.Dg + ((long)b * d.n_cap + s) * DG_STRIDE;
-#pragma unroll
-  for (int e = 0; e < 27; ++e) {
-    const double v = wave_sum(acc[e]);
-    if (lane == 0) out[e] = v;
-  }
-}
 
 void feature_device_setup() {
   (void)hipMemcpyToSymbol(HIP_SYMBOL(c_chi2), kChi2Q05, sizeof(double) * 99);
diff --git a/msckf_mono_amd/csrc/kernels_state.hip b/msckf_mono_amd/csrc/kernels_state.hip
--- a/msckf_mono_amd/csrc/kernels_state.hip
+++ b/msckf_mono_amd/csrc/kernels_state.hip
@@ -1,4 +1,5 @@
 #include "dev_common.h"
+#include "select_diag.h"
 
 namespace msckf {
 
@@ -122,10 +123,11 @@
   augment_body<S>(d, b, tid, reinterpret_cast<S*>(smem_raw));
 }
 
-template <class S, bool AUGMENT, int QM>
-__global__ __launch_bounds__(256) void k_propagate(Dev<S> d, int b0, const S* readings, long rd_stride, int K, const int* cnt) {
-  const int b = b0 + blockIdx.x, tid = threadIdx.x, lane = tid & 63, w = tid >> 6;
-  if (cnt) K = cnt[blockIdx.x];
+template <class S, bool AUGMENT, int QM, bool HEAD = false>
+__global__ __launch_bounds__(256) void k_propagate(Dev<S> d, int b0, const S* readings, long rd_stride, int K, const int* cnt, int nb, int ndiag) {
+  if (HEAD && (int)blockIdx.x <= ndiag) { select_diag_body<S>(d, b0, nb, ndiag, (int)blockIdx.x, (int)blockIdx.y); return; }
+  const int b = b0 + (HEAD ? blockIdx.y : blockIdx.x), tid = threadIdx.x, lane = tid & 63, w = tid >> 6;
+  if (cnt) K = cnt[HEAD ? blockIdx.y : blockIdx.x];
   constexpr bool FULLQ = QM == 2;
   if (QM != 0 && (d.qf[(long)b * QF_STRIDE + QF_FLAG] != S(0)) != FULLQ) return;
   __builtin_amdgcn_s_setprio(3);
@@ -456,7 +458,7 @@
 #ifdef MSCKF_ABLATE
   __syncthreads();
   PR_TICK(4);
-  if (tid == 0 && blockIdx.x == 0) { for (int q = 0; q < 5; ++q) atomicAdd(&g_prop_cycles[q], (unsigned long long)pcyc[q]); atomicAdd(&g_prop_cycles[5], 1ull); }
+  if (tid == 0 && b == b0) { for (int q = 0; q < 5; ++q) atomicAdd(&g_prop_cycles[q], (unsigned long long)pcyc[q]); atomicAdd(&g_prop_cycles[5], 1ull); }
 #endif
   if (AUGMENT) {
     __syncthreads();
@@ -509,8 +511,8 @@
 
 template <class S, int QM>
 static void launch_propagate_q(const Dev<S>& d, int b0, int nb, const S* readings, long rd_stride, int K, hipStream_t st, bool then_augment, const int* cnt) {
-  if (then_augment) hipLaunchKernelGGL((k_propagate<S, true, QM>), dim3(nb), dim3(256), (size_t)6 * d.ld * sizeof(S), st, d, b0, readings, rd_stride, K, cnt);
-  else hipLaunchKernelGGL((k_propagate<S, false, QM>), dim3(nb), dim3(256), 0, st, d, b0, readings, rd_stride, K, cnt);
+  if (then_augment) hipLaunchKernelGGL((k_propagate<S, true, QM>), dim3(nb), dim3(256), (size_t)6 * d.ld * sizeof(S), st, d, b0, readings, rd_stride, K, cnt, 0, 0);
+  else hipLaunchKernelGGL((k_propagate<S, false, QM>), dim3(nb), dim3(256), 0, st, d, b0, readings, rd_stride, K, cnt, 0, 0);
 }
 template <class S>
 void launch_propagate(const Dev<S>& d, int b0, int nb, const S* readings, long rd_stride, int K, hipStream_t st, bool then_augment, int qroute, const int* cnt) {
@@ -521,6 +523,17 @@
   launch_propagate_q<S, 2>(d, b0, nb, readings, rd_stride, K, st, then_augment, cnt);
 }
 template <class S>
+void launch_frame_head(const Dev<S>& d, int b0, int nb, const S* readings, long rd_stride, int K, hipStream_t st, int qroute, const int* cnt) {
+  if (nb <= 0) return;
+  if constexpr (sizeof(S) == 4) {
+    const int ndiag = (d.n_cap + 3) / 4;
+    const dim3 grid(ndiag + 2, nb);
+    const size_t lds = (size_t)6 * d.ld * sizeof(S);
+    if (qroute == 0) hipLaunchKernelGGL((k_propagate<S, true, 0, true>), grid, dim3(256), lds, st, d, b0, readings, rd_stride, K, cnt, nb, ndiag);
+    else hipLaunchKernelGGL((k_propagate<S, true, 2, true>), grid, dim3(256), lds, st, d, b0, readings, rd_stride, K, cnt, nb, ndiag);
+  }
+}
+template <class S>
 void launch_augment(const Dev<S>& d, int b0, int nb, hipStream_t st, const int* cnt) {
   if (nb <= 0) return;
   hipLaunchKernelGGL(k_augment<S>, dim3(nb), dim3(256), (size_t)6 * d.ld * sizeof(S), st, d, b0, cnt);
@@ -536,6 +549,8 @@
 
 template void launch_propagate<float>(const Dev<float>&, int, int, const float*, long, int, hipStream_t, bool, int, const int*);
 template void launch_propagate<double>(const Dev<double>&, int, int, const double*, long, int, hipStream_t, bool, int, const int*);
+template void launch_frame_head<float>(const Dev<float>&, int, int, const float*, long, int, hipStream_t, int, const int*);
+template void launch_frame_head<double>(const Dev<double>&, int, int, const double*, long, int, hipStream_t, int, const int*);
 template void launch_augment<float>(const Dev<float>&, int, int, hipStream_t, const int*);
 template void launch_augment<double>(const Dev<double>&, int, int, hipStream_t, const int*);
 template void launch_prune<float>(const Dev<float>&, int, int, hipStream_t, const int*, int);
diff --git a/msckf_mono_amd/csrc/msckf_hip.hip b/msckf_mono_amd/csrc/msckf_hip.hip
--- a/msckf_mono_amd/csrc/msckf_hip.hip
+++ b/msckf_mono_amd/csrc/msckf_hip.hip
@@ -22,6 +22,7 @@
 
 #include "../../include/msckf_hip.h"
 #include "dev_common.h"
+#include "frame_order.h"
 #include "host_lists.h"
 #include "input_layouts.h"
 #include "replay_plan.h"
@@ -134,6 +135,8 @@
   std::vector<int> h_ncam;
   hipStream_t sty[MAXS] = {nullptr}; hipEvent_t ev_fa[MAXS] = {nullptr}, ev_fb[MAXS] = {nullptr};
   Settings settings;
+  msckf_settings::FrameSettings frame_settings;
+  std::atomic<long long> n_feature_first{0};
   int small_limit = 0;
   bool info_form = false;
   std::vector<double> h_uv;
@@ -941,6 +944,11 @@
   }
   int store(int Settings::* field, int v) { settings.*field = v; apply_settings(); return 0; }
   int set_feature_overlap(int on) { return store(&Settings::overlap_feature, on ? 1 : 0); }
+  int set_frame_order(int order) {
+    if (order != 0 && order != 1) return fail(-EINVAL, "order: 0 propagate first on every frame, 1 feature first where the frame allows it");
+    frame_settings.order = order;
+    return 0;
+  }
   int set_compression(int route) {
     if (route < -1 || route > 3) return fail(-EINVAL, "route: -1 default, 0 Householder TSQR, 1..3 information form (blocked matrix-core Cholesky; 1 and 2 named retired factorizations)");
     if (route >= 1 && !info_form) return fail(-ENOTSUP, "information form not available for this window size (6 n_cap + 1 > 384 or f_cap > 1024)");
@@ -1367,13 +1375,13 @@
     if (flips & 1) std::swap(d.P, P_spare);
   }
   int update_compress() const { return routes::effective_compress(d.compress, settings.compress_route, n_lit); }
-  void launch_update(const Dev<S>& vin, int b0, int nb, hipStream_t q, bool feature_done = false, int ncam_ahead = 0, const int* cell_k = nullptr) {
+  void launch_update(const Dev<S>& vin, int b0, int nb, hipStream_t q, bool feature_done = false, int ncam_ahead = 0, const int* cell_k = nullptr, bool select_done = false) {
     invalidate_imu(b0, nb);
     Dev<S> v = vin;
     v.compress = update_compress();
     if (!feature_done) { stage_begin(2, q); launch_feature<S>(v, b0, nb, q); stage_end(2, q); }
     const routes::CompressRoute cr = routes::compress_route(v.compress, d.ldR, d.Mp != nullptr, d.lam_part > 0, d.gram_parts);
-    stage_begin(7, q); if (cr.select_diag) launch_select_diag<S>(v, b0, nb, q); else launch_select<S>(v, b0, nb, q); stage_end(7, q);
+    if (!select_done) { stage_begin(7, q); if (cr.select_diag) launch_select_diag<S>(v, b0, nb, q); else launch_select<S>(v, b0, nb, q); stage_end(7, q); }
     const routes::SmallRoute sr = routes::small_route(nb, [&](int i) { return routes::window_cols(h_ncam[b0 + i], ncam_ahead, cell_k && cell_k[i] == IMU_SKIP, n_cap); },
                                                       small_limit, v.compress, n_lit, d.joseph, f_cap, sizeof(S), update_small_granted());
     if (sr.kind != routes::CHAIN_ONLY) {
@@ -1568,7 +1576,7 @@
     HIPCHK(cp(d.ncam, o->d.ncam, Bz * sizeof(int))); HIPCHK(cp(d.n_resid, o->d.n_resid, Bz * sizeof(long long)));
     HIPCHK(cp(d.stats, o->d.stats, Bz * STAT_STRIDE * sizeof(int))); HIPCHK(cp(d.ncam_upd, o->d.ncam_upd, Bz * sizeof(int)));
     traj = o->traj; h_ncam = o->h_ncam; h_uv = o->h_uv; h_imu = o->h_imu; h_imu_ok = o->h_imu_ok; h_qfull = o->h_qfull;
-    settings.take_over(o->settings);
+    settings.take_over(o->settings); frame_settings.take_over(o->frame_settings);
     prn_list.forget(h_ncam);
     HIPCHK(hipStreamSynchronize(st));
     std::fill(h_lit.begin(), h_lit.end(), 0); n_lit = 0;
@@ -1716,10 +1724,19 @@
     const bool fuse = fuse_frame(f, f1);
     v.trk_n = in.n; v.trk_M = in.M; v.trk_off = in.off; v.trk_slots = in.slots; v.trk_obs = in.obs;
     v.wl_stride_n = 1; v.wl_stride_f = f_cap; v.wl_stride_o = 0;
-    bool early = may_overlap && settings.overlap_feature && !prof && f > f0;
-    for (int b = b0; b < b0 + nb && early; ++b) {
-      const int n_after = std::min(h_ncam[b] + 1, n_cap);
-      early = h_ncam[b] < n_cap && cells.maxslot[b] <= n_after - 2 && cell_k[b] != IMU_SKIP;
+    const int q_route = qroute(b0, nb);
+    const bool select_diag = routes::compress_route(update_compress(), d.ldR, d.Mp != nullptr, d.lam_part > 0, d.gram_parts).select_diag;
+    const bool feature_first = routes::frame_order(frame_settings.order, settings.overlap_feature, sizeof(S), select_diag, q_route, nb, h_ncam.data() + b0,
+                                                   cells.maxslot + b0, cell_k + b0, IMU_SKIP, n_cap, f == f0, prof) == routes::FO_TAKEN;
+    const bool early = may_overlap && settings.overlap_feature &&
+                       routes::feature_ahead(nb, h_ncam.data() + b0, cells.maxslot + b0, cell_k + b0, IMU_SKIP, n_cap, f == f0, prof) == routes::FO_TAKEN;
+    if (feature_first) {
+      StageRange r("msckf_marginalize(features)+imu_prop+msckf_augment_state");
+      Dev<S> v2 = v; v2.ncam_bias = 1;
+      v2.compress = update_compress();
+      launch_feature<S>(v2, b0, nb, q);
+      launch_frame_head<S>(v2, b0, nb, in.rd, (long)K * RD_STRIDE, K, q, q_route, in.k);
+      n_feature_first.fetch_add(1, std::memory_order_relaxed);
     }
     if (early) {
       (void)hipEventRecord(ev_fa[hh], q);
@@ -1729,15 +1746,15 @@
       launch_feature<S>(v2, b0, nb, sty[hh]);
       (void)hipEventRecord(ev_fb[hh], sty[hh]);
     }
-    {
+    if (!feature_first) {
       StageRange r("imu_prop+msckf_augment_state");
-      stage_begin(0, q); launch_propagate<S>(v, b0, nb, in.rd, (long)K * RD_STRIDE, K, q, !prof, qroute(b0, nb), in.k); stage_end(0, q);
+      stage_begin(0, q); launch_propagate<S>(v, b0, nb, in.rd, (long)K * RD_STRIDE, K, q, !prof, q_route, in.k); stage_end(0, q);
       if (prof) { stage_begin(1, q); launch_augment<S>(v, b0, nb, q, in.k); stage_end(1, q); }
     }
     if (early) (void)hipStreamWaitEvent(q, ev_fb[hh], 0);
     v.ncam_defer = 0;
     if (fuse) { v.Pout = s.flipped ? d.P : P_spare; v.fuse_drop = in.drop; }
-    { StageRange r(fuse ? "msckf_marginalize+msckf_prune_empty_states" : "msckf_marginalize"); launch_update(v, b0, nb, q, early, 1, cell_k + b0); }
+    { StageRange r(fuse ? "msckf_marginalize+msckf_prune_empty_states" : "msckf_marginalize"); launch_update(v, b0, nb, q, early || feature_first, 1, cell_k + b0, feature_first); }
     if (fuse) s.flipped = !s.flipped;
     else {
       if (prn.buf) launch_pruned_log<S>(v, b0, nb, q, in.drop, prn.ordinal(f, f0), prn.cap, static_cast<S*>(prn.buf), prn.found);
@@ -2343,6 +2360,12 @@
 int msckf_hip_scenario_pin(msckf_hip_handle h, int f0, int f1) { if (!h) return fail(-EINVAL, "null handle"); return H(h)->scen_pin(f0, f1); }
 int msckf_hip_set_upload_ring(msckf_hip_handle h, int depth, int mode) { if (!h) return fail(-EINVAL, "null handle"); return H(h)->set_upload_ring(depth, mode); }
 int msckf_hip_set_feature_overlap(msckf_hip_handle h, int on) { if (!h) return fail(-EINVAL, "null handle"); return H(h)->set_feature_overlap(on); }
+int msckf_hip_set_frame_order(msckf_hip_handle h, int order) { if (!h) return fail(-EINVAL, "null handle"); return H(h)->set_frame_order(order); }
+int msckf_hip_get_frame_order_count(msckf_hip_handle h, long long* count) {
+  if (!h || !count) return fail(-EINVAL, "null handle or null count");
+  *count = H(h)->n_feature_first.load(std::memory_order_relaxed);
+  return 0;
+}
 int msckf_hip_set_covariance_update(msckf_hip_handle h, int form) { if (!h) return fail(-EINVAL, "null handle"); return H(h)->set_cov_update(form); }
 int msckf_hip_set_compression(msckf_hip_handle h, int route) { if (!h) return fail(-EINVAL, "null handle"); return H(h)->set_compression(route); }
 int msckf_hip_set_gate_early_accept(msckf_hip_handle h, int on) { if (!h) return fail(-EINVAL, "null handle"); return H(h)->set_gate_early(on); }
diff --git a/msckf_mono_amd/csrc/select_diag.h b/msckf_mono_amd/csrc/select_diag.h
--- /dev/null
+++ b/msckf_mono_amd/csrc/select_diag.h
@@ -0,0 +1,249 @@
+#ifndef MSCKF_SELECT_DIAG_H
+#define MSCKF_SELECT_DIAG_H
+
+#include "dev_common.h"
+
+namespace msckf {
+
+template <class S>
+__device__ __forceinline__ int update_ncam(const Dev<S>& d, int b) { return d.ncam_bias ? d.ncam_upd[b] : d.ncam[b]; }
+
+template <class S>
+__device__ __forceinline__ void select_body(const Dev<S>& d, const int b0, const int nb, const int i, const int lane) {
+  if (i >= nb) return;
+  const int b = b0 + i;
+  const int F = d.trk_n[(long)i * d.wl_stride_n];
+  long long nres = d.n_resid[b];
+  int* st = d.stats + (long)b * STAT_STRIDE;
+  int mrej = 0, trej = 0, grej = 0, pass = 0;
+  int* rs = d.row_start + (long)b * (d.f_cap + 1);
+  int* order = d.trk_order + (long)b * d.f_cap;
+  __shared__ int sCnt[64], sBase[64], sRows[64];
+  sCnt[lane] = 0; sRows[lane] = 0;
+  __syncthreads();
+  if (!(nres <= 3 && d.mode == 0) && F <= 256) {
+    __shared__ short sMrow[256];
+    __shared__ short sOrd[256];
+    int sv[4], Mv[4], fv[4];
+    bool inc[4];
+#pragma unroll
+    for (int c = 0; c < 4; ++c) {
+      const int t = 64 * c + lane, tc = min(t, max(F - 1, 0));
+      const long tb = (long)b * d.f_cap + tc;
+      sv[c] = d.trk_status[tb]; Mv[c] = d.trk_M[(long)i * d.wl_stride_f + tc]; fv[c] = d.trk_first[tb] & 63;
+    }
+#pragma unroll
+    for (int c = 0; c < 4; ++c) {
+      const int t = 64 * c + lane;
+      const bool in = t < F;
+      int sx = in ? sv[c] : 0;
+      const int M = in ? Mv[c] : 0;
+      bool m_rej = false, t_rej = false, g_rej = false, valid = false, incl = false;
+      if (in) {
+        if (M < 2 || !(sx & ST_MOTION_OK)) { m_rej = true; sx = (M < 2) ? 0 : (sx & ~(ST_TRI_VALID | ST_GATE_PASS)); }
+        else if (sx & ST_TRI_VALID) valid = true;
+        else { t_rej = true; sx &= ~ST_GATE_PASS; }
+        if (valid) { if (sx & ST_GATE_PASS) { incl = true; sx |= ST_INCLUDED; } else g_rej = true; }
+        d.trk_status[(long)b * d.f_cap + t] = sx;
+        sMrow[t] = (short)(2 * M - 3);
+      }
+      inc[c] = incl;
+      if (incl) { atomicAdd(&sCnt[fv[c]], 1); atomicAdd(&sRows[fv[c]], 2 * M - 3); }
+      mrej += __popcll(__ballot(m_rej)); trej += __popcll(__ballot(t_rej)); grej += __popcll(__ballot(g_rej));
+      pass += __popcll(__ballot(incl)); if (d.mode == 0) nres += __popcll(__ballot(valid));
+    }
+    __syncthreads();
+    {
+      const int c0 = sCnt[lane];
+      int scan = c0;
+#pragma unroll
+      for (int o = 1; o < 64; o <<= 1) { const int up = __shfl_up(scan, o, 64); if (lane >= o) scan += up; }
+      sBase[lane] = scan - c0;
+    }
+    __syncthreads();
+    const int nbin = min(d.n_cap, 64);
+#pragma unroll
+    for (int c = 0; c < 4; ++c) {
+      const int bin = inc[c] ? fv[c] : -1;
+      int rank = 0, cnt = 0;
+      for (int sbin = 0; sbin < nbin; ++sbin) {
+        const unsigned long long m = __ballot(bin == sbin);
+        if (bin == sbin) { rank = __popcll(m & ((1ull << lane) - 1ull)); cnt = __popcll(m); }
+      }
+      int pos = 0;
+      if (inc[c]) { pos = sBase[bin] + rank; sOrd[pos] = (short)(64 * c + lane); order[pos] = 64 * c + lane; }
+      __syncthreads();
+      if (inc[c] && rank == 0) sBase[bin] += cnt;
+      __syncthreads();
+    }
+    int rows = 0;
+    for (int p0 = 0; p0 < pass; p0 += 64) {
+      const int p = p0 + lane;
+      const int r = p < pass ? (int)sMrow[sOrd[p]] : 0;
+      int scan = r;
+#pragma unroll
+      for (int o = 1; o < 64; o <<= 1) { const int up = __shfl_up(scan, o, 64); if (lane >= o) scan += up; }
+      if (p < pass) rs[p] = rows + scan - r;
+      rows += __shfl(scan, 63, 64);
+    }
+    if (lane == 0) {
+      rs[pass] = rows;
+      d.n_resid[b] = nres;
+      st[STAT_NTRACKS] = F; st[STAT_MOTION_REJ] = mrej; st[STAT_TRI_REJ] = trej; st[STAT_GATE_REJ] = grej;
+      st[STAT_PASSED] = pass; st[STAT_MROWS] = rows; st[STAT_RROWS] = rows > 0 ? 6 * update_ncam(d, b) : 0;
+    }
+    return;
+  }
+  if (nres <= 3 && d.mode == 0) {
+    if (lane == 0) {
+      for (int t = 0; t < F; ++t) {
+        const long tb = (long)b * d.f_cap + t;
+        int s = d.trk_status[tb];
+        const int M = d.trk_M[(long)i * d.wl_stride_f + t];
+        bool valid = false;
+        if (M < 2) { if (nres > 3) mrej++; else trej++; s = 0; }
+        else if (nres > 3 && !(s & ST_MOTION_OK)) { mrej++; s &= ~(ST_TRI_VALID | ST_GATE_PASS); }
+        else {
+          if (nres <= 3) s |= ST_MOTION_SKIPPED;
+          if (s & ST_TRI_VALID) { valid = true; nres++; } else { trej++; s &= ~ST_GATE_PASS; }
+        }
+        if (valid) {
+          if (s & ST_GATE_PASS) { s |= ST_INCLUDED; pass++; const int f0 = d.trk_first[tb] & 63; sCnt[f0]++; sRows[f0] += 2 * M - 3; }
+          else grej++;
+        }
+        d.trk_status[tb] = s;
+      }
+    }
+    mrej = __shfl(mrej, 0, 64); trej = __shfl(trej, 0, 64); grej = __shfl(grej, 0, 64); pass = __shfl(pass, 0, 64);
+    nres = __shfl((int)nres, 0, 64);
+  } else {
+    for (int t0 = 0; t0 < F; t0 += 64) {
+      const int t = t0 + lane;
+      const bool in = t < F;
+      const long tb = (long)b * d.f_cap + t;
+      int s = in ? d.trk_status[tb] : 0;
+      const int M = in ? d.trk_M[(long)i * d.wl_stride_f + t] : 0;
+      bool m_rej = false, t_rej = false, g_rej = false, valid = false, incl = false;
+      if (in) {
+        if (M < 2 || !(s & ST_MOTION_OK)) { m_rej = true; s = (M < 2) ? 0 : (s & ~(ST_TRI_VALID | ST_GATE_PASS)); }
+        else if (s & ST_TRI_VALID) valid = true;
+        else { t_rej = true; s &= ~ST_GATE_PASS; }
+        if (valid) { if (s & ST_GATE_PASS) { incl = true; s |= ST_INCLUDED; } else g_rej = true; }
+        d.trk_status[tb] = s;
+      }
+      if (incl) { const int f0 = d.trk_first[tb] & 63; atomicAdd(&sCnt[f0], 1); atomicAdd(&sRows[f0], 2 * M - 3); }
+      mrej += __popcll(__ballot(m_rej)); trej += __popcll(__ballot(t_rej)); grej += __popcll(__ballot(g_rej));
+      pass += __popcll(__ballot(incl)); if (d.mode == 0) nres += __popcll(__ballot(valid));
+    }
+  }
+  __syncthreads();
+  {
+    const int c = sCnt[lane];
+    int scan = c;
+#pragma unroll
+    for (int o = 1; o < 64; o <<= 1) { const int up = __shfl_up(scan, o, 64); if (lane >= o) scan += up; }
+    sBase[lane] = scan - c;
+  }
+  __syncthreads();
+  for (int t0 = 0; t0 < F; t0 += 64) {
+    const int t = t0 + lane;
+    const long tb = (long)b * d.f_cap + t;
+    const bool incl = (t < F) && (d.trk_status[tb] & ST_INCLUDED);
+    const int bin = incl ? (d.trk_first[tb] & 63) : -1;
+    int pos = -1;
+    for (int sbin = 0; sbin < d.n_cap && sbin < 64; ++sbin) {
+      const unsigned long long m = __ballot(bin == sbin);
+      if (bin == sbin) pos = sBase[sbin] + __popcll(m & ((1ull << lane) - 1ull));
+      __syncthreads();
+      if (lane == 0) sBase[sbin] += __popcll(m);
+      __syncthreads();
+    }
+    if (incl) order[pos] = t;
+  }
+  __syncthreads();
+  int rows = 0;
+  for (int p0 = 0; p0 < pass; p0 += 64) {
+    const int p = p0 + lane;
+    int r = 0;
+    if (p < pass) { const int t = order[p]; r = 2 * d.trk_M[(long)i * d.wl_stride_f + t] - 3; }
+    int scan = r;
+#pragma unroll
+    for (int o = 1; o < 64; o <<= 1) { const int up = __shfl_up(scan, o, 64); if (lane >= o) scan += up; }
+    if (p < pass) rs[p] = rows + scan - r;
+    rows += __shfl(scan, 63, 64);
+  }
+  if (lane == 0) {
+    rs[pass] = rows;
+    d.n_resid[b] = nres;
+    st[STAT_NTRACKS] = F; st[STAT_MOTION_REJ] = mrej; st[STAT_TRI_REJ] = trej; st[STAT_GATE_REJ] = grej;
+    st[STAT_PASSED] = pass; st[STAT_MROWS] = rows; st[STAT_RROWS] = rows > 0 ? 6 * update_ncam(d, b) : 0;
+  }
+}
+
+template <class S>
+__device__ __forceinline__ void select_diag_body(const Dev<S>& d, const int b0, const int nb, const int ndiag, const int x, const int i) {
+  const int tid = threadIdx.x, lane = tid & 63, w = tid >> 6;
+  if (x == ndiag) { if (tid < 64) select_body<S>(d, b0, nb, i, tid); return; }
+  const int b = b0 + i;
+  const int N = update_ncam(d, b), F = d.trk_n[(long)i * d.wl_stride_n];
+  const int s = 4 * x + w;
+  if (s >= N) return;
+  const int f_cap = d.f_cap, m_cap = d.m_cap;
+  const int* stt = d.trk_status + (long)b * f_cap;
+  const int* Mv = d.trk_M + (long)i * d.wl_stride_f;
+  constexpr int ALL = ST_MOTION_OK | ST_TRI_VALID | ST_GATE_PASS;
+  int tcut = 0;
+  if (d.mode == 0 && F > 0) {
+    int need = 4 - d.nres_upd[b];
+    if (need > 0) {
+      tcut = F;
+      for (int t0 = 0; t0 < F && need > 0; t0 += 64) {
+        const int t = t0 + lane;
+        const bool v = t < F && Mv[t] >= 2 && (stt[t] & ST_TRI_VALID);
+        unsigned long long m = __ballot(v);
+        const int c = __popcll(m);
+        if (c < need) { need -= c; continue; }
+        int pos = 0;
+        for (int k = 0; k < need; ++k) { pos = __builtin_ctzll(m); m &= m - 1; }
+        tcut = t0 + pos + 1; need = 0;
+      }
+    }
+  }
+  double acc[27];
+#pragma unroll
+  for (int e = 0; e < 27; ++e) acc[e] = 0.0;
+  for (int t = lane; t < F; t += 64) {
+    const long tb = (long)b * f_cap + t;
+    const int sx = stt[t], M = Mv[t];
+    const int oi = d.trk_inv[tb * d.n_cap + s];
+    const int need_bits = t < tcut ? (ST_TRI_VALID | ST_GATE_PASS) : ALL;
+    if (M < 2 || (sx & need_bits) != need_bits || oi < 0) continue;
+    const long h0i = (tb * m_cap + oi) * 12;
+    const S* rw = d.trk_rw + tb * 2 * m_cap + 2 * oi;
+    double h0[6], h1[6];
+#pragma unroll
+    for (int k = 0; k < 6; ++k) { h0[k] = (double)ld_hx(d, h0i + k); h1[k] = (double)ld_hx(d, h0i + 6 + k); }
+    const double r0 = (double)rw[0], r1 = (double)rw[1];
+    int e = 0;
+#pragma unroll
+    for (int a = 0; a < 6; ++a)
+#pragma unroll
+      for (int c = a; c < 6; ++c) acc[e++] += h0[a] * h0[c] + h1[a] * h1[c];
+#pragma unroll
+    for (int a = 0; a < 6; ++a) acc[21 + a] += h0[a] * r0 + h1[a] * r1;
+  }
+  double* out = d.Dg + ((long)b * d.n_cap + s) * DG_STRIDE;
+#pragma unroll
+  for (int e = 0; e < 27; ++e) {
+    const double v = wave_sum(acc[e]);
+    if (lane == 0) out[e] = v;
+  }
+}
+
+template <class S>
+__global__ __launch_bounds__(256) void k_select_diag(Dev<S> d, int b0, int nb, int ndiag) {
+  select_diag_body<S>(d, b0, nb, ndiag, (int)blockIdx.x, (int)blockIdx.y);
+}
+
+}
+#endif
diff --git a/msckf_mono_amd/csrc/settings.h b/msckf_mono_amd/csrc/settings.h
--- a/msckf_mono_amd/csrc/settings.h
+++ b/msckf_mono_amd/csrc/settings.h
@@ -69,6 +69,11 @@
   }
 }
 
+struct FrameSettings {
+  int order = 1;
+  void take_over(const FrameSettings& o) { order = o.order; }
+};
+
 inline bool settings_from_env(Settings& s, std::string& err) {
   for (const SettingRow& r : SETTINGS_TABLE) {
     const char* e = (r.env && r.field) ? getenv(r.env) : nullptr;
```

Result: faster. 228,100 updates/s (median of 6 runs) (+4.5%).
